# purvakulkarni15/PathTracerAP

Measured on NVIDIA B200. Metric: Mrays/s (all bounces), higher is better.
Workload: dtype f32

## Files before the change

### pathtracerap_b200/csrc/api.cu

```cuda
#include <dlfcn.h>

#include <algorithm>
#include <array>
#include <cmath>
#include <chrono>
#include <cstdarg>
#include <cstdio>
#include <cstdlib>
#include <cstring>
#include <atomic>
#include <string>
#include <thread>
#include <vector>

#include "bvh_build.h"
#include "host_math.h"
#include "kernels.cuh"

using namespace ptap;

namespace {

struct Arena {
    char* base = nullptr;
    size_t cap = 0, used = 0;
    cudaError_t reserve(size_t bytes)
    {
        used = 0;
        if (bytes <= cap) return cudaSuccess;
        if (base) cudaFree(base);
        base = nullptr; cap = 0;
        cudaError_t e = cudaMalloc(&base, bytes);
        if (e == cudaSuccess) cap = bytes;
        return e;
    }
    template <typename T> T* alloc(size_t count)
    {
        size_t bytes = (count * sizeof(T) + 255) & ~size_t(255);
        if (used + bytes > cap) return nullptr;
        T* p = reinterpret_cast<T*>(base + used);
        used += bytes;
        return p;
    }
    static size_t need(size_t count, size_t elem) { return (count * elem + 255) & ~size_t(255); }
    void release() { if (base) cudaFree(base); base = nullptr; cap = used = 0; }
};

}

struct ptap_ctx {
    int device = 0;
    int sms = 148;
    cudaStream_t stream = nullptr;
    cudaEvent_t ev0 = nullptr, ev1 = nullptr, tm0 = nullptr, tm1 = nullptr;
    std::vector<cudaEvent_t> prof_events;
    std::vector<int> prof_kind;
    size_t prof_used = 0;
    Arena scene_arena, frame_arena, scratch;
    SceneDev sc{};
    WaveDev wv{};
    int lanes = 1;
    int lanes_env = 0;
    WaveDev wvx[kMaxLanes]{};
    cudaStream_t streams[kMaxLanes] = {};
    cudaEvent_t e_fork = nullptr, e_cache = nullptr, e_join[kMaxLanes] = {}, e_gather[kMaxLanes] = {};
    std::vector<TriRec> h_tris;
    int ntris = 0;
    std::vector<PtapMesh> h_meshes;
    std::vector<PtapModel> h_models;
    std::vector<InstanceTrace> h_inst;
    InstanceTrace* d_inst = nullptr; TriRec* d_tris = nullptr; BvhNode* d_nodes = nullptr; size_t nodes_cap = 0; LeafTri* d_btris = nullptr; int* d_btid = nullptr;
    bool have_scene = false, have_grid = false, have_bvh = false, have_frame = false;
    int bvh_kind = -1;
    int accel = PTAP_ACCEL_GRID_COMPAT;
    uint32_t flags = 0;
    bool cache_valid = false;
    int grid_trace = 0, grid_shade = 0, grid_gen = 0;
    int trace_ctas = 0;
    PtapStats stats{};
    PtapCamera camera{{0.0f, 0.0f, 920.0f}, {-10.0f, -4.0f, 900.0f}, {20.0f, 16.0f}, 0, 0u};
    std::vector<cudaEvent_t> iter_events;
    int iter_events_used = 0;
    std::vector<float> iter_ms;
    int emu_replay_ctas = 6, emu_walk_ctas = 2;
    Arena emu_arena; int emu_lanes = 0;
    int2* d_tri_box = nullptr; size_t tri_box_cap = 0; bool emu_ok = false;
    std::vector<int> h_grid_first, h_model_grid;
    int2* gd_cells = nullptr; int* gd_refs = nullptr; size_t gd_ncells = 0, gd_nrefs = 0;
    void* nccl_comm = nullptr;
    cudaEvent_t e_peer = nullptr;
    unsigned long long* d_stamps = nullptr;
    int stamps_used = 0;
    bool render_pending = false;
    Arena query_arena;
    cudaEvent_t e_qin = nullptr, e_qout = nullptr;
    bool query_anyhit = true;
    std::string err;
};

namespace {

int fail(ptap_ctx* c, int code, const char* fmt, ...)
{
    char buf[512];
    va_list ap; va_start(ap, fmt); vsnprintf(buf, sizeof buf, fmt, ap); va_end(ap);
    if (c) c->err = buf;
    return code;
}

#define CK(call)                                                                                       \
    do {                                                                                               \
        cudaError_t e_ = (call);                                                                       \
        if (e_ != cudaSuccess) return fail(ctx, (int)e_, "%s: %s", #call, cudaGetErrorString(e_));   \
    } while (0)

template <typename F> void parallelFor(int n, F fn)
{
    const int workers = n < (1 << 16) ? 1 : (int)std::min(8u, std::max(1u, std::thread::hardware_concurrency()));
    if (workers <= 1) { fn(0, n); return; }
    std::vector<std::thread> pool;
    const int chunk = (n + workers - 1) / workers;
    for (int w = 1; w < workers; ++w) pool.emplace_back([=]() { fn(std::min(n, w * chunk), std::min(n, (w + 1) * chunk)); });
    fn(0, std::min(n, chunk));
    for (std::thread& t : pool) t.join();
}

float4 row(const float* m, int r) { return make_float4(m[0 + r], m[4 + r], m[8 + r], m[12 + r]); }

constexpr int kMaxStamps = 8192;

void launchTrace(ptap_ctx* c, FrameState* st, const float4* O, const float4* D, float4* hit, float2* uv, int4* counts, int round, int n_fixed,
                 const EmuBuf& emu, bool count_totals = false, cudaStream_t stream = nullptr, unsigned long long* stamp = nullptr)
{
    if (!stream) stream = c->stream;
    if (c->accel == PTAP_ACCEL_GRID_EMULATED) {
        launchTraceEmu(c->sc, O, D, hit, uv, counts, count_totals, st, round, n_fixed, c->grid_trace, c->sms * c->emu_replay_ctas, c->sms, stream, stamp, emu);
        launchTraceGrid(c->sc, O, D, hit, uv, nullptr, false, st, round, n_fixed, c->sms, stream, nullptr, emu.list2);
    }
    else if (c->accel != PTAP_ACCEL_GRID_COMPAT) launchTraceBvh(c->sc, O, D, hit, uv, counts, count_totals, st, round, n_fixed, c->grid_trace, stream, stamp);
    else launchTraceGrid(c->sc, O, D, hit, uv, counts, count_totals, st, round, n_fixed, c->grid_trace, stream, stamp);
}

size_t emuFullThreads(const ptap_ctx* c) { return (size_t)c->sms * kTraceBlock; }

size_t emuArenaNeed(const ptap_ctx* c, size_t n)
{
    return Arena::need(n, sizeof(int)) * 3 + Arena::need(n * kEmuHits, sizeof(int)) + Arena::need(n * kEmuHits, sizeof(float)) + Arena::need(n * 5, sizeof(uint4)) +
           Arena::need(emuFullThreads(c) * kBigHits, sizeof(uint4));
}

EmuBuf emuFromArena(const ptap_ctx* c, Arena& A, size_t n)
{
    EmuBuf e;
    e.n = A.alloc<int>(n); e.list = A.alloc<int>(n); e.list2 = A.alloc<int>(n); e.id = A.alloc<int>(n * kEmuHits); e.t = A.alloc<float>(n * kEmuHits); e.stride = (int)n;
    e.cont = A.alloc<uint4>(n * 5); e.cont_cap = (int)n;
    e.big = A.alloc<uint4>(emuFullThreads(c) * kBigHits);
    return e;
}

int ensureEmuBuffers(ptap_ctx* ctx)
{
    if (ctx->accel != PTAP_ACCEL_GRID_EMULATED) return PTAP_OK;
    const size_t N = (size_t)ctx->wv.N, per_lane = emuArenaNeed(ctx, N), need = per_lane * (size_t)ctx->lanes + 4096;
    bool moved = false;
    if (ctx->emu_arena.cap < need) { CK(ctx->emu_arena.reserve(need)); moved = true; }
    if (!moved && ctx->wv.emu.n && ctx->wv.emu.stride == (int)N && ctx->emu_lanes == ctx->lanes) return PTAP_OK;
    ctx->emu_arena.used = 0;
    ctx->wv.emu = emuFromArena(ctx, ctx->emu_arena, N);
    for (int l = 1; l < ctx->lanes; ++l) ctx->wvx[l].emu = emuFromArena(ctx, ctx->emu_arena, N);
    ctx->emu_lanes = ctx->lanes;
    return PTAP_OK;
}

void profMark(ptap_ctx* c, int kind)
{
    if (!(c->flags & PTAP_FLAG_PROFILE)) return;
    if (c->prof_used == c->prof_events.size()) {
        cudaEvent_t e; cudaEventCreate(&e); c->prof_events.push_back(e); c->prof_kind.push_back(0);
    }
    c->prof_kind[c->prof_used] = kind;
    cudaEventRecord(c->prof_events[c->prof_used++], c->stream);
}

void resetStats(ptap_ctx* c)
{
    const PtapStats old = c->stats;
    c->stats = PtapStats{};
    c->stats.scene_bytes = old.scene_bytes; c->stats.ms_build = old.ms_build; c->stats.bvh_nodes = old.bvh_nodes; c->stats.bvh_depth = old.bvh_depth;
    c->stats.lanes = c->lanes;
}

void applyCamera(const ptap_ctx* c, WaveDev& wv)
{
    wv.step_x = (float)((double)c->camera.span[0] / (double)wv.W);
    wv.step_y = (float)((double)c->camera.span[1] / (double)wv.H);
    for (int k = 0; k < 3; ++k) { wv.cam_o[k] = c->camera.origin[k]; wv.cam_p[k] = c->camera.plane_min[k]; }
    wv.jitter = c->camera.jitter; wv.jitter_seed = c->camera.jitter_seed;
}

int traceGridSize(ptap_ctx* c)
{
    int occ = c->accel == PTAP_ACCEL_GRID_EMULATED ? traceEmuOccupancy() : c->accel != PTAP_ACCEL_GRID_COMPAT ? traceBvhOccupancy() : traceGridOccupancy();
    if (c->trace_ctas > 0) occ = std::min(occ, c->trace_ctas);
    return c->sms * std::max(occ, 1);
}

int collect(ptap_ctx* ctx)
{
    if (!ctx->render_pending) return PTAP_OK;
    CK(cudaStreamSynchronize(ctx->stream));
    ctx->render_pending = false;
    CK(cudaEventElapsedTime(&ctx->stats.ms_render, ctx->ev0, ctx->ev1));
    FrameState fs;
    CK(cudaMemcpy(&fs, ctx->wv.st, sizeof fs, cudaMemcpyDeviceToHost));
    for (int l = 1; l < ctx->lanes; ++l) {
        if (!ctx->wvx[l].st) continue;
        FrameState f2;
        CK(cudaMemcpy(&f2, ctx->wvx[l].st, sizeof f2, cudaMemcpyDeviceToHost));
        const bool later = f2.iter_cur > fs.iter_cur && f2.paths > 0;
        f2.rays_traced += fs.rays_traced; f2.rays_walked += fs.rays_walked; f2.rays_reemulated += fs.rays_reemulated; f2.paths += fs.paths;
        f2.count_nodes += fs.count_nodes; f2.count_tris += fs.count_tris; f2.count_cells += fs.count_cells; f2.count_refs += fs.count_refs;
        if (later) fs = f2;
        else { fs.rays_traced = f2.rays_traced; fs.rays_walked = f2.rays_walked; fs.rays_reemulated = f2.rays_reemulated; fs.paths = f2.paths; fs.count_nodes = f2.count_nodes; fs.count_tris = f2.count_tris; fs.count_cells = f2.count_cells; fs.count_refs = f2.count_refs; }
    }
    ctx->stats.rays_traced = (int64_t)fs.rays_traced;
    ctx->stats.rays_walked = (int64_t)fs.rays_walked;
    ctx->stats.rays_reemulated = (int64_t)fs.rays_reemulated;
    ctx->stats.paths = (int64_t)fs.paths;
    for (int i = 0; i < 16; ++i) ctx->stats.active_per_round[i] = i <= kMaxDepth ? fs.n_active[i] : 0;
    const double rt = fs.rays_traced ? (double)fs.rays_traced : 1.0;
    ctx->stats.avg_nodes = (float)(fs.count_nodes / rt); ctx->stats.avg_tris = (float)(fs.count_tris / rt);
    ctx->stats.avg_cells = (float)(fs.count_cells / rt); ctx->stats.avg_refs = (float)(fs.count_refs / rt);
    ctx->stats.ms_generate = ctx->stats.ms_trace = ctx->stats.ms_shade = 0.f;
    for (size_t i = 0; i + 1 < ctx->prof_used; ++i) {
        float ms = 0.f;
        if (ctx->prof_kind[i] < 0) continue;
        cudaEventElapsedTime(&ms, ctx->prof_events[i], ctx->prof_events[i + 1]);
        if (ctx->prof_kind[i] == 0) ctx->stats.ms_generate += ms;
        else if (ctx->prof_kind[i] == 1) ctx->stats.ms_trace += ms;
        else ctx->stats.ms_shade += ms;
    }
    ctx->prof_used = 0;
    ctx->iter_ms.assign(ctx->iter_events_used, 0.f);
    for (int k = 0; k < ctx->iter_events_used; ++k) cudaEventElapsedTime(&ctx->iter_ms[k], ctx->ev0, ctx->iter_events[k]);
    ctx->iter_events_used = 0;
    ctx->stats.ms_trace_inflight = ctx->stats.ms_trace_sum = 0.f;
    if (ctx->stamps_used > 0 && ctx->d_stamps) {
        std::vector<unsigned long long> h((size_t)ctx->stamps_used * 2);
        CK(cudaMemcpy(h.data(), ctx->d_stamps, h.size() * sizeof(unsigned long long), cudaMemcpyDeviceToHost));
        std::vector<std::pair<unsigned long long, unsigned long long>> iv;
        double sum = 0.0;
        for (int k = 0; k < ctx->stamps_used; ++k)
            if (h[2 * k + 1] >= h[2 * k]) { iv.push_back({h[2 * k], h[2 * k + 1]}); sum += (double)(h[2 * k + 1] - h[2 * k]); }
        std::sort(iv.begin(), iv.end());
        double uni = 0.0; unsigned long long cur_b = 0, cur_e = 0; bool open = false;
        for (auto& x : iv) {
            if (!open) { cur_b = x.first; cur_e = x.second; open = true; }
            else if (x.first <= cur_e) cur_e = std::max(cur_e, x.second);
            else { uni += (double)(cur_e - cur_b); cur_b = x.first; cur_e = x.second; }
        }
        if (open) uni += (double)(cur_e - cur_b);
        ctx->stats.ms_trace_inflight = (float)(uni * 1e-6); ctx->stats.ms_trace_sum = (float)(sum * 1e-6);
        ctx->stamps_used = 0;
    }
    return PTAP_OK;
}

bool invert3(const double m[9], double out[9])
{
    const double c0 = m[4] * m[8] - m[5] * m[7], c1 = m[5] * m[6] - m[3] * m[8], c2 = m[3] * m[7] - m[4] * m[6];
    const double det = m[0] * c0 + m[1] * c1 + m[2] * c2;
    if (!(std::fabs(det) > 1e-300)) return false;
    const double id = 1.0 / det;
    out[0] = c0 * id; out[1] = (m[2] * m[7] - m[1] * m[8]) * id; out[2] = (m[1] * m[5] - m[2] * m[4]) * id;
    out[3] = c1 * id; out[4] = (m[0] * m[8] - m[2] * m[6]) * id; out[5] = (m[2] * m[3] - m[0] * m[5]) * id;
    out[6] = c2 * id; out[7] = (m[1] * m[6] - m[0] * m[7]) * id; out[8] = (m[0] * m[4] - m[1] * m[3]) * id;
    return true;
}

struct TlasItem { float lo[3], hi[3]; int inst; };

float boxArea(const float* lo, const float* hi)
{
    const float dx = hi[0] - lo[0], dy = hi[1] - lo[1], dz = hi[2] - lo[2];
    return 2.f * (dx * dy + dy * dz + dz * dx);
}

int buildTlas(std::vector<TlasItem>& items, int b, int e, std::vector<Bvh2Node>& nodes, float* lo, float* hi)
{
    for (int k = 0; k < 3; ++k) { lo[k] = 3e38f; hi[k] = -3e38f; }
    for (int i = b; i < e; ++i)
        for (int k = 0; k < 3; ++k) { lo[k] = std::min(lo[k], items[i].lo[k]); hi[k] = std::max(hi[k], items[i].hi[k]); }
    if (e - b == 1) return ~(0x20000000 | items[b].inst);
    int axis = 0; float best = -1.f;
    for (int k = 0; k < 3; ++k) {
        float cmin = 3e38f, cmax = -3e38f;
        for (int i = b; i < e; ++i) { const float c = items[i].lo[k] + items[i].hi[k]; cmin = std::min(cmin, c); cmax = std::max(cmax, c); }
        if (cmax - cmin > best) { best = cmax - cmin; axis = k; }
    }
    const int mid = (b + e) / 2;
    std::nth_element(items.begin() + b, items.begin() + mid, items.begin() + e,
                     [axis](const TlasItem& x, const TlasItem& y) { return x.lo[axis] + x.hi[axis] < y.lo[axis] + y.hi[axis]; });
    const int me = (int)nodes.size();
    nodes.emplace_back();
    float l0[3], h0[3], l1[3], h1[3];
    int c0 = buildTlas(items, b, mid, nodes, l0, h0);
    int c1 = buildTlas(items, mid, e, nodes, l1, h1);
    if (boxArea(l1, h1) < boxArea(l0, h0)) {
        std::swap(c0, c1);
        for (int k = 0; k < 3; ++k) { std::swap(l0[k], l1[k]); std::swap(h0[k], h1[k]); }
    }
    Bvh2Node& nd = nodes[me];
    nd.xy0 = make_float4(l0[0], h0[0], l0[1], h0[1]);
    nd.xy1 = make_float4(l1[0], h1[0], l1[1], h1[1]);
    nd.z01 = make_float4(l0[2], h0[2], l1[2], h1[2]);
    nd.link = make_int4(c0, c1, 0, 0);
    return me;
}

void dropBvh(ptap_ctx* ctx)
{
    ctx->have_bvh = false; ctx->bvh_kind = -1; ctx->sc.tlas_root = -1;
}

bool bvhMissing(const ptap_ctx* ctx) { return ctx->accel != PTAP_ACCEL_GRID_COMPAT && !ctx->have_bvh; }

int finishBvh(ptap_ctx* ctx, const BvhNode* roots, const int* mesh_root, int nnodes, int blas_depth, size_t* tlas_bytes)
{
    const int nm = (int)ctx->h_models.size();
    std::vector<TlasItem> items;
    double max_scale = 0.0, max_pad = 0.0, max_trans = 1.0;
    bool consistent = true;
    for (int i = 0; i < nm; ++i) {
        const PtapModel& m = ctx->h_models[i];
        const int root = mesh_root[m.mesh_index];
        ctx->h_inst[i].grid.z = __builtin_bit_cast(float, root);
        if (root < 0) continue;
        const float* W = m.world_to_model; const float* M = m.model_to_world;
        const double w3[9] = {W[0], W[4], W[8], W[1], W[5], W[9], W[2], W[6], W[10]};
        double wi[9];
        if (!invert3(w3, wi)) return fail(ctx, PTAP_E_INVALID, "model %d: world_to_model is singular", i);
        for (int r = 0; r < 3 && consistent; ++r)
            for (int c = 0; c < 4; ++c) {
                const double scale = c == 3 ? std::max(1.0, std::fabs((double)M[12 + r])) : 1.0;
                if (c == 3) max_trans = std::max(max_trans, scale);
                const double v = (double)M[0 + r] * W[4 * c + 0] + (double)M[4 + r] * W[4 * c + 1] + (double)M[8 + r] * W[4 * c + 2] + (c == 3 ? (double)M[12 + r] : 0.0);
                if (!(std::fabs(v - (r == c ? 1.0 : 0.0)) <= 2e-5 * scale)) { consistent = false; break; }
            }
        const BvhNode& r = roots[m.mesh_index];
        float mlo[3] = {3e38f, 3e38f, 3e38f}, mhi[3] = {-3e38f, -3e38f, -3e38f};
        for (int k = 0; k < 4; ++k) {
            if (!slotUsed(r, k)) continue;
            double lo[3], hi[3];
            decodeChild(r, k, lo, hi);
            for (int a = 0; a < 3; ++a) { mlo[a] = std::min(mlo[a], std::nextafter((float)lo[a], -3e38f)); mhi[a] = std::max(mhi[a], std::nextafter((float)hi[a], 3e38f)); }
        }
        TlasItem it; it.inst = i;
        for (int k = 0; k < 3; ++k) { it.lo[k] = 3e38f; it.hi[k] = -3e38f; }
        double ext = 0.0;
        for (int c = 0; c < 8; ++c) {
            const double p[3] = {((c & 1) ? mhi[0] : mlo[0]) - (double)W[12], ((c & 2) ? mhi[1] : mlo[1]) - (double)W[13], ((c & 4) ? mhi[2] : mlo[2]) - (double)W[14]};
            for (int rr = 0; rr < 3; ++rr) {
                const double w = wi[3 * rr] * p[0] + wi[3 * rr + 1] * p[1] + wi[3 * rr + 2] * p[2];
                it.lo[rr] = std::min(it.lo[rr], (float)w); it.hi[rr] = std::max(it.hi[rr], (float)w);
                ext = std::max(ext, std::fabs(w));
            }
        }
        const float pad = (float)(ext * 1e-4 + 1e-3);
        for (int k = 0; k < 3; ++k) { it.lo[k] -= pad; it.hi[k] += pad; }
        items.push_back(it);
        double fro = 0.0;
        for (double v : wi) fro += v * v;
        max_scale = std::max(max_scale, std::sqrt(fro));
        max_pad = std::max(max_pad, (double)pad);
    }
    std::vector<BvhNode> tlas;
    int tlas_root = -1, tlas_depth = 0;
    if (!items.empty()) {
        float lo[3], hi[3];
        std::vector<Bvh2Node> t2;
        const int link = buildTlas(items, 0, (int)items.size(), t2, lo, hi);
        if (link < 0) {
            Bvh2Node nd;
            nd.xy0 = make_float4(lo[0], hi[0], lo[1], hi[1]); nd.xy1 = nd.xy0;
            nd.z01 = make_float4(lo[2], hi[2], lo[2], hi[2]);
            nd.link = make_int4(link, link, 0, 0);
            t2.push_back(nd);
        }
        tlas_root = collapseBvh2(t2.data(), link < 0 ? (int)t2.size() - 1 : link, tlas, nnodes, 1, tlas_depth);
    }
    if (3 * (blas_depth + tlas_depth) + 8 > kBvhStack) return fail(ctx, PTAP_E_INVALID, "BVH too deep for the traversal stack (%d + %d levels, %d entries)", blas_depth, tlas_depth, kBvhStack);
    if (nnodes + tlas.size() > ctx->nodes_cap) return fail(ctx, PTAP_E_NOMEM, "BVH node storage exhausted");
    CK(cudaMemcpyAsync(ctx->d_inst, ctx->h_inst.data(), nm * sizeof(InstanceTrace), cudaMemcpyHostToDevice, ctx->stream));
    if (!tlas.empty()) CK(cudaMemcpyAsync(ctx->d_nodes + nnodes, tlas.data(), tlas.size() * sizeof(BvhNode), cudaMemcpyHostToDevice, ctx->stream));
    CK(cudaStreamSynchronize(ctx->stream));
    if (tlas_bytes) *tlas_bytes = nm * sizeof(InstanceTrace) + tlas.size() * sizeof(BvhNode);
    ctx->sc.tlas_root = tlas_root;
    ctx->sc.tmin_world = -(float)((kEpsilon + 2e-4) * max_scale * 1.001 + max_pad + 1e-3);
    ctx->sc.prune = consistent ? 1.0003f : INFINITY;
    ctx->sc.tie = consistent ? 1.5e-4f : INFINITY;
    ctx->sc.c_pad = (float)(4e-5 * max_trans + 1e-3);
    ctx->have_bvh = true;
    return PTAP_OK;
}

int uploadBvh(ptap_ctx* ctx, const BvhNode* nodes, int nnodes, const int* tri_id, const int* mesh_root, int known_depth, size_t* bytes)
{
    const int nt = ctx->ntris, nm = (int)ctx->h_models.size();
    dropBvh(ctx);
    if ((size_t)nnodes > ctx->nodes_cap) return fail(ctx, PTAP_E_NOMEM, "BVH has more nodes than reserved (2 per triangle)");
    {
        std::atomic<int> bad_node{-1}, bad_leaf{-1}, bad_entry{-1};
        parallelFor(nnodes, [&](int b, int e) {
            for (int i = b; i < e; ++i)
                for (int k = 0; k < 4; ++k) {
                    const int l = nodes[i].link[k];
                    if (l >= nnodes) bad_node = i;
                    if (l < 0) { const int code = ~l, first = code >> 3, cnt = (code & 7) + 1; if (code >= 0x20000000 || first < 0 || first + cnt > nt) bad_leaf = i; }
                }
        });
        parallelFor(nt, [&](int b, int e) { for (int k = b; k < e; ++k) if (tri_id[k] < 0 || tri_id[k] >= nt) bad_entry = k; });
        if (bad_node >= 0) return fail(ctx, PTAP_E_INVALID, "BVH node %d: child index out of range", bad_node.load());
        if (bad_leaf >= 0) return fail(ctx, PTAP_E_INVALID, "BVH node %d: leaf range out of bounds", bad_leaf.load());
        if (bad_entry >= 0) return fail(ctx, PTAP_E_INVALID, "BVH leaf order entry %d out of range", bad_entry.load());
    }
    for (size_t m = 0; m < ctx->h_meshes.size(); ++m)
        if (mesh_root[m] >= nnodes) return fail(ctx, PTAP_E_INVALID, "mesh %d: BVH root out of range", (int)m);
    int blas_depth = 0;
    (void)known_depth;
    {
        std::vector<int> level(nnodes, 0);
        bool ordered = true;
        for (size_t m = 0; m < ctx->h_meshes.size(); ++m) {
            if (mesh_root[m] < 0) continue;
            if (level[mesh_root[m]]) return fail(ctx, PTAP_E_INVALID, "BVH node %d is the root of two meshes", mesh_root[m]);
            level[mesh_root[m]] = 1;
        }
        for (int i = 0; i < nnodes && ordered; ++i) {
            if (!level[i]) continue;
            blas_depth = std::max(blas_depth, level[i]);
            for (int k = 0; k < 4; ++k) {
                const int l = nodes[i].link[k];
                if (l < 0 || !slotUsed(nodes[i], k)) continue;
                if (l <= i) { ordered = false; break; }
                if (level[l]) return fail(ctx, PTAP_E_INVALID, "BVH node %d is reachable twice", l);
                level[l] = level[i] + 1;
            }
        }
        if (!ordered) {
            blas_depth = 0;
            std::vector<std::pair<int, int>> todo;
            std::vector<char> seen(nnodes, 0);
            for (size_t m = 0; m < ctx->h_meshes.size(); ++m) if (mesh_root[m] >= 0) todo.push_back({mesh_root[m], 1});
            while (!todo.empty()) {
                const auto [node, d] = todo.back(); todo.pop_back();
                if (seen[node]) return fail(ctx, PTAP_E_INVALID, "BVH node %d is reachable twice", node);
                seen[node] = 1;
                blas_depth = std::max(blas_depth, d);
                for (int k = 0; k < 4; ++k)
                    if (nodes[node].link[k] >= 0 && slotUsed(nodes[node], k)) todo.push_back({nodes[node].link[k], d + 1});
            }
        }
    }
    std::vector<BvhNode> roots(ctx->h_meshes.size());
    for (size_t m = 0; m < roots.size(); ++m)
        if (mesh_root[m] >= 0) roots[m] = nodes[mesh_root[m]];
    CK(cudaMemcpyAsync(ctx->d_nodes, nodes, (size_t)nnodes * sizeof(BvhNode), cudaMemcpyHostToDevice, ctx->stream));
    CK(cudaMemcpyAsync(ctx->d_btid, tri_id, (size_t)nt * sizeof(int), cudaMemcpyHostToDevice, ctx->stream));
    launchGatherTris(ctx->d_tris, ctx->d_btid, nt, ctx->d_btris, ctx->stream);
    size_t tb = 0;
    const int rc = finishBvh(ctx, roots.data(), mesh_root, nnodes, blas_depth, &tb);
    if (rc) return rc;
    if (bytes) *bytes = tb + (size_t)nnodes * sizeof(BvhNode) + (size_t)nt * sizeof(int);
    ctx->bvh_kind = PTAP_ACCEL_BVH;
    return PTAP_OK;
}

int buildBvhOnDevice(ptap_ctx* ctx)
{
    const int nt = ctx->ntris, nmesh = (int)ctx->h_meshes.size();
    dropBvh(ctx);
    int max_tris = 0;
    for (const PtapMesh& m : ctx->h_meshes) max_tris = std::max(max_tris, m.t_end - m.t_start);
    const size_t need = deviceBvhScratchBytes(max_tris);
    if (need > ctx->scratch.cap) CK(ctx->scratch.reserve(need)); else ctx->scratch.used = 0;
    std::vector<int> mesh_root(nmesh, -1);
    int nnodes = 0, leaf_base = 0, blas_depth = 0;
    for (int mi = 0; mi < nmesh; ++mi) {
        const PtapMesh& m = ctx->h_meshes[mi];
        const int n = m.t_end - m.t_start;
        if (n <= 0 || m.t_start < 0 || m.t_end > nt) continue;
        if ((size_t)nnodes + (size_t)n > ctx->nodes_cap || leaf_base + n > nt) return fail(ctx, PTAP_E_NOMEM, "device BVH build: node / leaf storage exhausted");
        int made = 0, depth = 0;
        std::string why;
        const int e = buildMeshBvhDevice(ctx->d_tris, m.t_start, m.t_end, m.bb_min, m.bb_max, nnodes, ctx->d_nodes + nnodes, leaf_base, ctx->d_btris, ctx->d_btid,
                                         ctx->scratch.base, ctx->scratch.cap, ctx->stream, &made, &depth, &why);
        if (e != 0) return fail(ctx, e, "device BVH build of mesh %d (%d triangles): %s", mi, n, why.empty() ? cudaGetErrorString((cudaError_t)e) : why.c_str());
        mesh_root[mi] = nnodes;
        nnodes += made; leaf_base += n; blas_depth = std::max(blas_depth, depth);
    }
    std::vector<BvhNode> roots(nmesh);
    for (int mi = 0; mi < nmesh; ++mi)
        if (mesh_root[mi] >= 0) CK(cudaMemcpyAsync(&roots[mi], ctx->d_nodes + mesh_root[mi], sizeof(BvhNode), cudaMemcpyDeviceToHost, ctx->stream));
    CK(cudaStreamSynchronize(ctx->stream));
    const int rc = finishBvh(ctx, roots.data(), mesh_root.data(), nnodes, blas_depth, nullptr);
    if (rc) return rc;
    ctx->bvh_kind = PTAP_ACCEL_BVH_DEVICE;
    ctx->stats.bvh_nodes = nnodes; ctx->stats.bvh_depth = blas_depth;
    return PTAP_OK;
}

}

extern "C" {

int ptap_create(int device, size_t arena_bytes, ptap_ctx** out)
{
    if (!out) return PTAP_E_INVALID;
    *out = nullptr;
    int ndev = 0;
    if (cudaGetDeviceCount(&ndev) != cudaSuccess || ndev == 0 || device < 0 || device >= ndev) return PTAP_E_NO_DEVICE;
    cudaDeviceProp prop;
    if (cudaGetDeviceProperties(&prop, device) != cudaSuccess) return PTAP_E_NO_DEVICE;
    if (prop.major < 10) return PTAP_E_NO_DEVICE;
    ptap_ctx* ctx = new ptap_ctx();
    ctx->device = device;
    ctx->sms = prop.multiProcessorCount;
    if (cudaSetDevice(device) != cudaSuccess || cudaStreamCreateWithFlags(&ctx->stream, cudaStreamNonBlocking) != cudaSuccess) {
        delete ctx; return PTAP_E_NO_DEVICE;
    }
    cudaEventCreate(&ctx->ev0); cudaEventCreate(&ctx->ev1);
    auto envInt = [](const char* name, int dflt) { const char* v = getenv(name); return v && *v ? atoi(v) : dflt; };
    ctx->sc.vote_tri = std::min(32, std::max(1, envInt("PTAP_VOTE_TRI", kVoteTri)));
    ctx->sc.vote_inst = std::min(32, std::max(1, envInt("PTAP_VOTE_INST", kVoteInst)));
    ctx->sc.vote_refill = std::min(32, std::max(1, envInt("PTAP_VOTE_REFILL", kVoteRefill)));
    ctx->sc.batch = std::max(1, envInt("PTAP_BATCH", kTraceBatch));
    ctx->sc.vote_grid = std::min(32, std::max(1, envInt("PTAP_VOTE_GRID", kVoteGrid)));
    ctx->sc.shade_sort = envInt("PTAP_SHADE_SORT", 0) != 0;
    ctx->lanes_env = std::min(kMaxLanes, std::max(0, envInt("PTAP_LANES", 0)));
    ctx->lanes = ctx->lanes_env ? ctx->lanes_env : kDefaultLanes;
    ctx->streams[0] = ctx->stream;
    const int max_lanes = ctx->lanes_env ? ctx->lanes_env : kMaxLanes;
    if (max_lanes > 1) {
        bool ok = cudaEventCreateWithFlags(&ctx->e_fork, cudaEventDisableTiming) == cudaSuccess && cudaEventCreateWithFlags(&ctx->e_cache, cudaEventDisableTiming) == cudaSuccess;
        for (int l = 0; l < max_lanes; ++l) {
            if (l > 0) ok = ok && cudaStreamCreateWithFlags(&ctx->streams[l], cudaStreamNonBlocking) == cudaSuccess;
            ok = ok && cudaEventCreateWithFlags(&ctx->e_join[l], cudaEventDisableTiming) == cudaSuccess && cudaEventCreateWithFlags(&ctx->e_gather[l], cudaEventDisableTiming) == cudaSuccess;
        }
        if (!ok) { ptap_destroy(ctx); return PTAP_E_NOMEM; }
    }
    ctx->trace_ctas = std::max(0, envInt("PTAP_TRACE_CTAS", 0));
    ctx->emu_replay_ctas = std::max(1, envInt("PTAP_EMU_REPLAY_CTAS", 6));
    ctx->emu_walk_ctas = std::max(1, envInt("PTAP_EMU_WALK_CTAS", 2));
    ctx->sc.emu_refill = std::min(32, std::max(1, envInt("PTAP_EMU_REFILL", 8)));
    ctx->query_anyhit = envInt("PTAP_QUERY_ANYHIT", 1) != 0;
    if (cudaEventCreateWithFlags(&ctx->e_qin, cudaEventDisableTiming) != cudaSuccess || cudaEventCreateWithFlags(&ctx->e_qout, cudaEventDisableTiming) != cudaSuccess) {
        ptap_destroy(ctx); return PTAP_E_NOMEM;
    }
    if (arena_bytes) {
        if (ctx->scene_arena.reserve(arena_bytes / 4) != cudaSuccess || ctx->frame_arena.reserve(arena_bytes - arena_bytes / 4) != cudaSuccess) {
            ptap_destroy(ctx); return PTAP_E_NOMEM;
        }
    }
    *out = ctx;
    return PTAP_OK;
}

void ptap_destroy(ptap_ctx* ctx)
{
    if (!ctx) return;
    cudaSetDevice(ctx->device);
    if (ctx->stream) cudaStreamSynchronize(ctx->stream);
    for (int l = 1; l < kMaxLanes; ++l) if (ctx->streams[l]) { cudaStreamSynchronize(ctx->streams[l]); cudaStreamDestroy(ctx->streams[l]); }
    for (cudaEvent_t e : {ctx->e_fork, ctx->e_cache}) if (e) cudaEventDestroy(e);
    for (int l = 0; l < kMaxLanes; ++l) { if (ctx->e_join[l]) cudaEventDestroy(ctx->e_join[l]); if (ctx->e_gather[l]) cudaEventDestroy(ctx->e_gather[l]); }
    ctx->scene_arena.release(); ctx->frame_arena.release(); ctx->scratch.release(); ctx->emu_arena.release(); ctx->query_arena.release();
    for (cudaEvent_t e : {ctx->e_qin, ctx->e_qout}) if (e) cudaEventDestroy(e);
    if (ctx->gd_cells) cudaFree(ctx->gd_cells);
    if (ctx->d_tri_box) cudaFree(ctx->d_tri_box);
    if (ctx->gd_refs) cudaFree(ctx->gd_refs);
    for (cudaEvent_t e : ctx->prof_events) cudaEventDestroy(e);
    for (cudaEvent_t e : ctx->iter_events) cudaEventDestroy(e);
    if (ctx->e_peer) cudaEventDestroy(ctx->e_peer);
    if (ctx->nccl_comm) ptap_nccl_finalize(ctx);
    if (ctx->ev0) cudaEventDestroy(ctx->ev0);
    if (ctx->tm0) { cudaEventDestroy(ctx->tm0); cudaEventDestroy(ctx->tm1); }
    if (ctx->ev1) cudaEventDestroy(ctx->ev1);
    if (ctx->stream) cudaStreamDestroy(ctx->stream);
    delete ctx;
}

const char* ptap_last_error(const ptap_ctx* ctx) { return ctx ? ctx->err.c_str() : "no context"; }
void* ptap_stream(ptap_ctx* ctx) { return ctx ? (void*)ctx->stream : nullptr; }

int ptap_upload_scene(ptap_ctx* ctx, const PtapSceneView* v)
{
    if (!ctx || !v || !v->models || !v->meshes || !v->vertices || !v->triangles || v->nmodels <= 0) return fail(ctx, PTAP_E_INVALID, "upload_scene: missing arrays");
    CK(cudaSetDevice(ctx->device));
    if (ctx->render_pending) { int rc = collect(ctx); if (rc) return rc; }
    const bool timing = getenv("PTAP_UPLOAD_TIMING") != nullptr;
    const auto t_begin = std::chrono::steady_clock::now();
    auto t_last = t_begin;
    auto lap = [&](const char* what) {
        if (!timing) return;
        const auto now = std::chrono::steady_clock::now();
        fprintf(stderr, "ptap_upload_scene: %-28s %8.3f ms\n", what, std::chrono::duration<double, std::milli>(now - t_last).count());
        t_last = now;
    };
    const int nm = v->nmodels, nt = v->ntriangles;
    const bool grid = v->grids && v->voxels && v->refs && v->ngrids > 0;
    ctx->have_scene = false; ctx->have_grid = false; ctx->have_bvh = false; ctx->bvh_kind = -1; ctx->cache_valid = false; ctx->emu_ok = false;
    ctx->sc.tlas_root = -1; ctx->sc.nmodels = 0;
    for (int i = 0; i < nm; ++i) {
        const PtapModel& m = v->models[i];
        if (m.mesh_index < 0 || m.mesh_index >= v->nmeshes) return fail(ctx, PTAP_E_INVALID, "model %d: mesh_index %d out of range", i, m.mesh_index);
        if (grid && (m.grid_index < 0 || m.grid_index >= v->ngrids)) return fail(ctx, PTAP_E_INVALID, "model %d: grid_index %d out of range", i, m.grid_index);
    }
    const bool prepacked = v->tri_recs && v->n_tri_recs == nt;
    if (!prepacked)
        for (int t = 0; t < nt; ++t)
            for (int k = 0; k < 3; ++k)
                if (v->triangles[t].v[k] < 0 || v->triangles[t].v[k] >= v->nvertices) return fail(ctx, PTAP_E_INVALID, "triangle %d: vertex index out of range", t);

    std::vector<InstanceTrace> inst(nm);
    std::vector<InstanceShade> shade(nm);
    for (int i = 0; i < nm; ++i) {
        const PtapModel& m = v->models[i];
        InstanceTrace& it = inst[i];
        for (int r = 0; r < 3; ++r) { it.w2m[r] = row(m.world_to_model, r); it.m2w[r] = row(m.model_to_world, r); }
        it.bb_min = make_float4(0, 0, 0, 1); it.bb_max = make_float4(0, 0, 0, 1); it.grid = make_float4(1, 0, 0, 0);
        if (grid) {
            const PtapGrid& g = v->grids[m.grid_index];
            int owner = g.entity_index;
            if (owner < 0 || owner >= nm) return fail(ctx, PTAP_E_INVALID, "grid %d: entity_index %d out of range", m.grid_index, owner);
            const PtapMesh& mesh = v->meshes[v->models[owner].mesh_index];
            it.bb_min = make_float4(mesh.bb_min[0], mesh.bb_min[1], mesh.bb_min[2], g.width[0]);
            it.bb_max = make_float4(mesh.bb_max[0], mesh.bb_max[1], mesh.bb_max[2], g.width[1]);
            it.grid.x = g.width[2];
            it.grid.y = __builtin_bit_cast(float, (int)g.v_start);
        }
        float nmx[9];
        hm::normal_matrix(m.model_to_world, nmx);
        shade[i].nm0 = make_float4(nmx[0], nmx[1], nmx[2], m.mat.color[0]);
        shade[i].nm1 = make_float4(nmx[3], nmx[4], nmx[5], m.mat.color[1]);
        shade[i].nm2 = make_float4(nmx[6], nmx[7], nmx[8], m.mat.color[2]);
        shade[i].mat = make_int4(m.mat.type, 0, 0, 0);
    }
    const TriRec* recs = static_cast<const TriRec*>(v->tri_recs);
    if (!prepacked) {
        ctx->h_tris.resize(nt);
        makeTriRecs(v->vertices, v->triangles, nt, ctx->h_tris.data());
        recs = ctx->h_tris.data();
    } else ctx->h_tris.clear();
    ctx->ntris = nt;
    ctx->h_meshes.assign(v->meshes, v->meshes + v->nmeshes);
    ctx->h_models.assign(v->models, v->models + nm);
    ctx->h_grid_first.clear(); ctx->h_model_grid.clear();
    if (grid) {
        for (int g = 0; g < v->ngrids; ++g) ctx->h_grid_first.push_back(v->grids[g].v_start);
        for (int i = 0; i < nm; ++i) ctx->h_model_grid.push_back(v->models[i].grid_index);
    }

    std::vector<int2> cells;
    if (grid) {
        cells.resize(v->nvoxels);
        for (int i = 0; i < v->nvoxels; ++i) {
            const bool tri = v->voxels[i].entity_type == 2;
            cells[i] = tri ? make_int2(v->voxels[i].start, v->voxels[i].end) : make_int2(0, 0);
            if (tri && (v->voxels[i].start < 0 || v->voxels[i].end > v->nrefs)) return fail(ctx, PTAP_E_INVALID, "voxel %d: ref range out of bounds", i);
        }
        for (int i = 0; i < v->nrefs; ++i)
            if (v->refs[i] < 0 || v->refs[i] >= nt) return fail(ctx, PTAP_E_INVALID, "ref %d: triangle index out of range", i);
        if (v->grid_dim[0] <= 0 || v->grid_dim[1] <= 0 || v->grid_dim[2] <= 0) return fail(ctx, PTAP_E_INVALID, "grid_dim must be positive");
        const long long ncell = (long long)v->grid_dim[0] * v->grid_dim[1] * v->grid_dim[2];
        for (int g = 0; g < v->ngrids; ++g)
            if (v->grids[g].v_start < 0 || v->grids[g].v_start + ncell > v->nvoxels) return fail(ctx, PTAP_E_INVALID, "grid %d: voxel range out of bounds", g);
    }

    lap("validate + repack (host)");
    const size_t nodes_cap = (size_t)std::max(nt, 1) * 2 + (size_t)nm * 2 + 2;
    size_t need = Arena::need(nm, sizeof(InstanceTrace)) + Arena::need(nm, sizeof(InstanceShade)) +
                  Arena::need(nt, sizeof(TriRec)) + Arena::need(nt, sizeof(LeafTri)) + Arena::need(nt, sizeof(float4)) + Arena::need(nt, sizeof(int)) + Arena::need(nodes_cap, sizeof(BvhNode)) +
                  (grid ? Arena::need(v->nvoxels, sizeof(int2)) + Arena::need(v->nrefs, sizeof(int)) : 0) + 4096;
    if (need > ctx->scene_arena.cap) CK(ctx->scene_arena.reserve(need)); else ctx->scene_arena.used = 0;
    Arena& A = ctx->scene_arena;
    InstanceTrace* d_inst = A.alloc<InstanceTrace>(nm);
    InstanceShade* d_shade = A.alloc<InstanceShade>(nm);
    TriRec* d_tris = A.alloc<TriRec>(nt);
    LeafTri* d_btris = A.alloc<LeafTri>(nt);
    float4* d_normals = A.alloc<float4>(nt);
    int* d_btid = A.alloc<int>(nt);
    BvhNode* d_nodes = A.alloc<BvhNode>(nodes_cap);
    int2* d_cells = grid ? A.alloc<int2>(v->nvoxels) : nullptr;
    int* d_refs = grid ? A.alloc<int>(v->nrefs) : nullptr;
    if (!d_inst || !d_shade || !d_tris || !d_normals || !d_btris || !d_btid || !d_nodes || (grid && (!d_cells || !d_refs))) return fail(ctx, PTAP_E_NOMEM, "scene arena exhausted");
    CK(cudaMemcpyAsync(d_inst, inst.data(), nm * sizeof(InstanceTrace), cudaMemcpyHostToDevice, ctx->stream));
    CK(cudaMemcpyAsync(d_shade, shade.data(), nm * sizeof(InstanceShade), cudaMemcpyHostToDevice, ctx->stream));
    CK(cudaMemcpyAsync(d_tris, recs, (size_t)nt * sizeof(TriRec), cudaMemcpyHostToDevice, ctx->stream));
    launchExtractNormals(d_tris, nt, d_normals, ctx->stream);
    ctx->d_tris = d_tris;
    if (grid) {
        CK(cudaMemcpyAsync(d_cells, cells.data(), cells.size() * sizeof(int2), cudaMemcpyHostToDevice, ctx->stream));
        CK(cudaMemcpyAsync(d_refs, v->refs, v->nrefs * sizeof(int), cudaMemcpyHostToDevice, ctx->stream));
    }
    size_t bytes = nm * (sizeof(InstanceTrace) + sizeof(InstanceShade)) + (size_t)nt * sizeof(TriRec) +
                   (grid ? cells.size() * sizeof(int2) + (size_t)v->nrefs * sizeof(int) : 0);
    ctx->h_inst = inst;
    ctx->d_inst = d_inst; ctx->d_nodes = d_nodes; ctx->nodes_cap = nodes_cap; ctx->d_btris = d_btris; ctx->d_btid = d_btid;
    ctx->have_bvh = false; ctx->bvh_kind = -1;
    lap("enqueue scene copies");
    if (v->bvh_nodes && v->n_bvh_nodes > 0 && v->bvh_tri_id && v->bvh_mesh_root) {
        if (v->n_bvh_tris != nt || v->n_bvh_roots != v->nmeshes) return fail(ctx, PTAP_E_INVALID, "upload_scene: prebuilt BVH does not match the triangle / mesh counts");
        size_t bb = 0;
        int rc = uploadBvh(ctx, reinterpret_cast<const BvhNode*>(v->bvh_nodes), v->n_bvh_nodes, v->bvh_tri_id, v->bvh_mesh_root, v->bvh_depth, &bb);
        if (rc) return rc;
        bytes += bb;
    }
    lap("BVH checks + TLAS (host)");
    CK(cudaStreamSynchronize(ctx->stream));
    lap("wait for the device");
    ctx->stats.scene_bytes = (int64_t)bytes;
    ctx->sc.inst = d_inst; ctx->sc.shade = d_shade; ctx->sc.tris = d_tris; ctx->sc.normals = d_normals;
    ctx->sc.cells = d_cells; ctx->sc.refs = d_refs; ctx->sc.nodes = d_nodes; ctx->sc.bvh_tris = d_btris; ctx->sc.bvh_tri_id = d_btid;
    ctx->sc.nmodels = nm; ctx->sc.gx = v->grid_dim[0]; ctx->sc.gy = v->grid_dim[1]; ctx->sc.gz = v->grid_dim[2];
    ctx->have_scene = true; ctx->have_grid = grid; ctx->cache_valid = false;
    ctx->accel = grid ? PTAP_ACCEL_GRID_COMPAT : PTAP_ACCEL_BVH;
    ctx->grid_trace = 0;
    return PTAP_OK;
}

int ptap_build_accel(ptap_ctx* ctx, int kind)
{
    if (!ctx || !ctx->have_scene) return fail(ctx, PTAP_E_STATE, "build_accel: no scene uploaded");
    CK(cudaSetDevice(ctx->device));
    if (ctx->render_pending) { int rc = collect(ctx); if (rc) return rc; }
    if (kind == PTAP_ACCEL_GRID_COMPAT) {
        if (!ctx->have_grid) return fail(ctx, PTAP_E_STATE, "build_accel: the uploaded scene carries no grids (call ptap_scene_build_grids first)");
    } else if (kind == PTAP_ACCEL_BVH) {
        if (!ctx->have_bvh || ctx->bvh_kind != PTAP_ACCEL_BVH) {
            BvhBuildResult res;
            if ((int)ctx->h_tris.size() != ctx->ntris) {
                ctx->h_tris.resize(ctx->ntris);
                CK(cudaMemcpyAsync(ctx->h_tris.data(), ctx->d_tris, (size_t)ctx->ntris * sizeof(TriRec), cudaMemcpyDeviceToHost, ctx->stream));
                CK(cudaStreamSynchronize(ctx->stream));
            }
            buildSceneBvh(ctx->h_tris.data(), (int)ctx->h_tris.size(), ctx->h_meshes.data(), (int)ctx->h_meshes.size(), res);
            int rc = uploadBvh(ctx, res.nodes.data(), (int)res.nodes.size(), res.tri_id.data(), res.mesh_root.data(), res.max_depth + 1, nullptr);
            if (rc) return rc;
            CK(cudaStreamSynchronize(ctx->stream));
        }
    } else if (kind == PTAP_ACCEL_BVH_DEVICE) {
        if (ctx->bvh_kind != PTAP_ACCEL_BVH_DEVICE) {
            cudaEvent_t b0, b1;
            CK(cudaEventCreate(&b0)); CK(cudaEventCreate(&b1));
            CK(cudaEventRecord(b0, ctx->stream));
            const int rc = buildBvhOnDevice(ctx);
            if (rc) { cudaEventDestroy(b0); cudaEventDestroy(b1); return rc; }
            CK(cudaEventRecord(b1, ctx->stream)); CK(cudaEventSynchronize(b1));
            cudaEventElapsedTime(&ctx->stats.ms_build, b0, b1);
            cudaEventDestroy(b0); cudaEventDestroy(b1);
        }
    } else if (kind == PTAP_ACCEL_GRID_EMULATED) {
        if (!ctx->have_grid) return fail(ctx, PTAP_E_STATE, "build_accel: the uploaded scene carries no grids (call ptap_scene_build_grids first)");
        if (!ctx->have_bvh) { const int rc = buildBvhOnDevice(ctx); if (rc) return rc; }
        if (!ctx->emu_ok) {
            const int nt = ctx->ntris, ng = (int)ctx->h_grid_first.size();
            if ((size_t)nt > ctx->tri_box_cap) {
                if (ctx->d_tri_box) { cudaFree(ctx->d_tri_box); ctx->d_tri_box = nullptr; ctx->tri_box_cap = 0; }
                CK(cudaMalloc(&ctx->d_tri_box, (size_t)std::max(nt, 1) * sizeof(int2)));
                ctx->tri_box_cap = (size_t)nt;
            }
            std::vector<int> range(2 * (size_t)std::max(ng, 1), 0);
            int ok = 0;
            const int e = gridTriBoxes(ctx->sc.cells, ctx->sc.refs, ng, ctx->h_grid_first.data(), ctx->sc.gx, ctx->sc.gy, ctx->sc.gz, nt, ctx->d_tri_box, range.data(), &ok, ctx->stream);
            if (e != 0) return fail(ctx, e, "build_accel: voxel boxes: %s", cudaGetErrorString((cudaError_t)e));
            if (!ok) return fail(ctx, PTAP_E_UNSUPPORTED, "build_accel: the voxel lists are not box-shaped ascending registrations of one grid per triangle; use PTAP_ACCEL_GRID_COMPAT");
            for (size_t i = 0; i < ctx->h_models.size(); ++i) {
                const int g = ctx->h_model_grid[i];
                const PtapMesh& mesh = ctx->h_meshes[ctx->h_models[i].mesh_index];
                if (range[2 * g] <= range[2 * g + 1] && (range[2 * g] < mesh.t_start || range[2 * g + 1] >= mesh.t_end))
                    return fail(ctx, PTAP_E_UNSUPPORTED, "build_accel: grid %d lists triangles outside the mesh of model %d; use PTAP_ACCEL_GRID_COMPAT", g, (int)i);
            }
            ctx->sc.tri_box = ctx->d_tri_box;
            ctx->emu_ok = true;
        }
    } else return fail(ctx, PTAP_E_INVALID, "build_accel: unknown kind %d", kind);
    ctx->accel = kind;
    ctx->cache_valid = false;
    ctx->grid_trace = traceGridSize(ctx);
    return PTAP_OK;
}

int ptap_set_render_params(ptap_ctx* ctx, int32_t W, int32_t H, int32_t depth, uint32_t flags)
{
    if (!ctx || W <= 0 || H <= 0 || depth <= 0 || depth > kMaxDepth) return fail(ctx, PTAP_E_INVALID, "set_render_params: W,H > 0 and 1 <= depth <= %d required", kMaxDepth);
    if ((long long)W * H > (1ll << 30)) return fail(ctx, PTAP_E_INVALID, "set_render_params: too many pixels");
    CK(cudaSetDevice(ctx->device));
    if (ctx->render_pending) { int rc = collect(ctx); if (rc) return rc; }
    const int N = W * H;
    ctx->lanes = ctx->lanes_env ? ctx->lanes_env : (N <= (1 << 20) ? kSmallFrameLanes : kDefaultLanes);
    const int ntiles = (N + kShadeTile - 1) / kShadeTile, nscan = (N + kScanSlots - 1) / kScanSlots;
    size_t need = Arena::need(N, sizeof(float4)) * 8 + Arena::need(N, sizeof(float2)) + Arena::need((size_t)N * 3, sizeof(float)) +
                  Arena::need((size_t)nscan * kMaxDepth, sizeof(unsigned long long)) + Arena::need(ntiles, sizeof(int)) * 2 +
                  Arena::need((size_t)nscan * kScanSlots, 1) + Arena::need(1, sizeof(FrameState)) + Arena::need(2 * kMaxStamps, sizeof(unsigned long long)) + 4096;
    if (ctx->lanes > 1)
        need += (size_t)(ctx->lanes - 1) * (Arena::need(N, sizeof(float4)) * 7 + Arena::need((size_t)nscan * kMaxDepth, sizeof(unsigned long long)) +
                                            Arena::need(ntiles, sizeof(int)) * 2 + Arena::need((size_t)nscan * kScanSlots, 1) + Arena::need(1, sizeof(FrameState)) + 4096) +
                (size_t)ctx->lanes * Arena::need((size_t)N * 3, sizeof(float));
    if (need > ctx->frame_arena.cap) CK(ctx->frame_arena.reserve(need)); else ctx->frame_arena.used = 0;
    Arena& A = ctx->frame_arena;
    WaveDev& wv = ctx->wv;
    for (int k = 0; k < 2; ++k) { wv.O[k] = A.alloc<float4>(N); wv.D[k] = A.alloc<float4>(N); wv.C[k] = A.alloc<float4>(N); }
    wv.hit = A.alloc<float4>(N); wv.hit_cache = A.alloc<float4>(N); wv.uv = A.alloc<float2>(N);
    wv.film = A.alloc<float>((size_t)N * 3);
    wv.tile_status = A.alloc<unsigned long long>((size_t)nscan * kMaxDepth);
    wv.tile_offset = A.alloc<int>(ntiles);
    wv.tile_ballot = A.alloc<unsigned>(ntiles);
    wv.perm = A.alloc<unsigned char>((size_t)nscan * kScanSlots);
    wv.st = A.alloc<FrameState>(1);
    wv.emu = EmuBuf{};
    ctx->d_stamps = A.alloc<unsigned long long>(2 * kMaxStamps); ctx->stamps_used = 0;
    if (!ctx->d_stamps || !wv.st || !wv.tile_status || !wv.tile_offset || !wv.tile_ballot || !wv.perm || !wv.film) return fail(ctx, PTAP_E_NOMEM, "frame arena exhausted");
    wv.W = W; wv.H = H; wv.N = N; wv.depth = depth; wv.ntiles = ntiles; wv.nscan = nscan;
    applyCamera(ctx, wv);
    wv.iter_stride = 1; wv.contrib = nullptr;
    if (ctx->lanes > 1) wv.contrib = A.alloc<float>((size_t)N * 3);
    for (int l = 1; l < ctx->lanes; ++l) {
        WaveDev& w2 = ctx->wvx[l];
        w2 = wv;
        for (int k = 0; k < 2; ++k) { w2.O[k] = A.alloc<float4>(N); w2.D[k] = A.alloc<float4>(N); w2.C[k] = A.alloc<float4>(N); }
        w2.hit = A.alloc<float4>(N);
        w2.tile_status = A.alloc<unsigned long long>((size_t)nscan * kMaxDepth);
        w2.tile_offset = A.alloc<int>(ntiles); w2.tile_ballot = A.alloc<unsigned>(ntiles);
        w2.perm = A.alloc<unsigned char>((size_t)nscan * kScanSlots);
        w2.st = A.alloc<FrameState>(1);
        w2.contrib = A.alloc<float>((size_t)N * 3);
        if (!w2.st || !w2.contrib || !wv.contrib || !w2.perm || !w2.hit) return fail(ctx, PTAP_E_NOMEM, "frame arena exhausted (lane %d)", l);
        CK(cudaMemsetAsync(w2.st, 0, sizeof(FrameState), ctx->stream));
    }
    CK(cudaMemsetAsync(wv.film, 0, (size_t)N * 3 * sizeof(float), ctx->stream));
    CK(cudaMemsetAsync(wv.st, 0, sizeof(FrameState), ctx->stream));
    CK(cudaStreamSynchronize(ctx->stream));
    ctx->flags = flags; ctx->cache_valid = false; ctx->have_frame = true;
    ctx->grid_shade = ctx->sms * std::max(shadeOccupancy(), 1);
    ctx->grid_gen = ctx->sms * 8;
    if (!ctx->grid_trace) ctx->grid_trace = traceGridSize(ctx);
    resetStats(ctx);
    return PTAP_OK;
}

int ptap_set_camera(ptap_ctx* ctx, const PtapCamera* cam)
{
    if (!ctx) return PTAP_E_INVALID;
    CK(cudaSetDevice(ctx->device));
    if (ctx->render_pending) { int rc = collect(ctx); if (rc) return rc; }
    const PtapCamera ref{{0.0f, 0.0f, 920.0f}, {-10.0f, -4.0f, 900.0f}, {20.0f, 16.0f}, 0, 0u};
    const PtapCamera c = cam ? *cam : ref;
    if (!(c.span[0] > 0.0f) || !(c.span[1] > 0.0f)) return fail(ctx, PTAP_E_INVALID, "set_camera: the image plane needs a positive extent");
    ctx->camera = c;
    ctx->cache_valid = false;
    if (ctx->have_frame) {
        applyCamera(ctx, ctx->wv);
        for (int l = 1; l < kMaxLanes; ++l) if (ctx->wvx[l].st) { WaveDev& w = ctx->wvx[l]; w.step_x = ctx->wv.step_x; w.step_y = ctx->wv.step_y; for (int k = 0; k < 3; ++k) { w.cam_o[k] = ctx->wv.cam_o[k]; w.cam_p[k] = ctx->wv.cam_p[k]; } w.jitter = ctx->wv.jitter; w.jitter_seed = ctx->wv.jitter_seed; }
    }
    return PTAP_OK;
}

int ptap_render(ptap_ctx* ctx, int32_t iter_begin, int32_t iter_end)
{
    if (!ctx || !ctx->have_scene || !ctx->have_frame) return fail(ctx, PTAP_E_STATE, "render: scene and render parameters required");
    if ((ctx->accel == PTAP_ACCEL_GRID_COMPAT || ctx->accel == PTAP_ACCEL_GRID_EMULATED) && !ctx->have_grid) return fail(ctx, PTAP_E_STATE, "render: no grid in the uploaded scene; build the BVH");
    if (bvhMissing(ctx)) return fail(ctx, PTAP_E_STATE, "render: no BVH on the device (build_accel failed or was not called)");
    if (iter_end < iter_begin) return fail(ctx, PTAP_E_INVALID, "render: empty iteration range");
    CK(cudaSetDevice(ctx->device));
    if (ctx->render_pending) { int rc = collect(ctx); if (rc) return rc; }
    { const int rc = ensureEmuBuffers(ctx); if (rc) return rc; }
    const bool cache = (ctx->flags & PTAP_FLAG_FIRST_HIT_CACHE) && !ctx->camera.jitter;
    const int L = (ctx->flags & (PTAP_FLAG_PROFILE | PTAP_FLAG_COUNT)) ? 1 : std::max(1, std::min(ctx->lanes, iter_end - iter_begin));
    WaveDev lane[kMaxLanes];
    lane[0] = ctx->wv;
    for (int l = 1; l < L; ++l) lane[l] = ctx->wvx[l];
    for (int l = 0; l < L; ++l) { lane[l].iter_stride = L; if (L == 1) lane[l].contrib = nullptr; }
    const bool stamping = (ctx->flags & PTAP_FLAG_STAMP) != 0;
    if (stamping) {
        CK(cudaMemset2DAsync(ctx->d_stamps, 16, 0xff, 8, kMaxStamps, ctx->stream));
        CK(cudaMemset2DAsync(ctx->d_stamps + 1, 16, 0x00, 8, kMaxStamps, ctx->stream));
    }
    ctx->stamps_used = 0; ctx->iter_events_used = 0;
    CK(cudaEventRecord(ctx->ev0, ctx->stream));
    if (L > 1) CK(cudaEventRecord(ctx->e_fork, ctx->stream));
    for (int l = 0; l < L; ++l) {
        if (l > 0) CK(cudaStreamWaitEvent(ctx->streams[l], ctx->e_fork, 0));
        launchSetIter(lane[l].st, iter_begin + l, ctx->streams[l]);
    }
    int64_t launches = L, trace_launches = 0;
    int cache_lane = -1;
    unsigned cache_waited = 0;
    for (int it = iter_begin; it < iter_end; ++it) {
        const int l = (it - iter_begin) % L;
        const WaveDev& wv = lane[l];
        cudaStream_t S = ctx->streams[l];
        profMark(ctx, 0);
        launchGenerate(wv, it, ctx->grid_gen, S); ++launches;
        int in = 0;
        for (int round = 0; round < wv.depth; ++round) {
            float4* hitbuf = (round == 0 && cache) ? wv.hit_cache : wv.hit;
            if (!(round == 0 && cache && ctx->cache_valid)) {
                profMark(ctx, 1);
                unsigned long long* stamp = stamping && ctx->stamps_used < kMaxStamps ? ctx->d_stamps + 2 * (size_t)ctx->stamps_used++ : nullptr;
                launchTrace(ctx, wv.st, wv.O[in], wv.D[in], hitbuf, nullptr, nullptr, round, -1, wv.emu, (ctx->flags & PTAP_FLAG_COUNT) != 0, S, stamp); launches += ctx->accel == PTAP_ACCEL_GRID_EMULATED ? 5 : 1; ++trace_launches;
                if (L > 1 && round == 0 && cache) { CK(cudaEventRecord(ctx->e_cache, S)); cache_lane = l; cache_waited = 1u << l; }
            } else if (L > 1 && cache_lane >= 0 && !(cache_waited >> l & 1u)) {
                CK(cudaStreamWaitEvent(S, ctx->e_cache, 0)); cache_waited |= 1u << l;
            }
            profMark(ctx, 2);
            launchScan(ctx->sc, wv, round, hitbuf, wv.depth - round, -1, S); ++launches;
            launchShade(ctx->sc, wv, round, in, hitbuf, wv.depth - round, -1, 0, nullptr, ctx->grid_shade, S); ++launches;
            in ^= 1;
        }
        if (L > 1) {
            if (it > iter_begin) CK(cudaStreamWaitEvent(S, ctx->e_gather[(l + L - 1) % L], 0));
            launchFilmAdd(wv.film, wv.contrib, (size_t)wv.N * 3, S); ++launches;
            CK(cudaEventRecord(ctx->e_gather[l], S));
        }
        if (cache) ctx->cache_valid = true;
        if (ctx->flags & PTAP_FLAG_ITER_TIMES) {
            if (ctx->iter_events_used == (int)ctx->iter_events.size()) { cudaEvent_t e; CK(cudaEventCreate(&e)); ctx->iter_events.push_back(e); }
            CK(cudaEventRecord(ctx->iter_events[ctx->iter_events_used++], S));
        }
    }
    for (int l = 1; l < L; ++l) {
        CK(cudaEventRecord(ctx->e_join[l], ctx->streams[l]));
        CK(cudaStreamWaitEvent(ctx->stream, ctx->e_join[l], 0));
    }
    profMark(ctx, -1);
    CK(cudaEventRecord(ctx->ev1, ctx->stream));
    CK(cudaGetLastError());
    ctx->stats.kernel_launches += launches;
    ctx->stats.trace_launches = trace_launches;
    ctx->render_pending = true;
    return PTAP_OK;
}

int ptap_sync(ptap_ctx* ctx)
{
    if (!ctx) return PTAP_E_INVALID;
    CK(cudaSetDevice(ctx->device));
    int rc = collect(ctx); if (rc) return rc;
    CK(cudaStreamSynchronize(ctx->stream));
    return PTAP_OK;
}

int ptap_frame_begin(ptap_ctx* ctx)
{
    if (!ctx || !ctx->have_frame) return fail(ctx, PTAP_E_STATE, "frame_begin: no render parameters");
    CK(cudaSetDevice(ctx->device));
    if (ctx->render_pending) { int rc = collect(ctx); if (rc) return rc; }
    CK(cudaMemsetAsync(ctx->wv.film, 0, (size_t)ctx->wv.N * 3 * sizeof(float), ctx->stream));
    CK(cudaMemsetAsync(ctx->wv.st, 0, sizeof(FrameState), ctx->stream));
    for (int l = 1; l < ctx->lanes; ++l) if (ctx->wvx[l].st) CK(cudaMemsetAsync(ctx->wvx[l].st, 0, sizeof(FrameState), ctx->stream));
    ctx->cache_valid = false;
    resetStats(ctx);
    return PTAP_OK;
}

int ptap_timer_start(ptap_ctx* ctx)
{
    if (!ctx) return PTAP_E_INVALID;
    CK(cudaSetDevice(ctx->device));
    if (!ctx->tm0) { CK(cudaEventCreate(&ctx->tm0)); CK(cudaEventCreate(&ctx->tm1)); }
    CK(cudaEventRecord(ctx->tm0, ctx->stream));
    return PTAP_OK;
}

int ptap_timer_stop(ptap_ctx* ctx, float* ms)
{
    if (!ctx || !ms || !ctx->tm0) return PTAP_E_INVALID;
    CK(cudaSetDevice(ctx->device));
    CK(cudaEventRecord(ctx->tm1, ctx->stream));
    CK(cudaEventSynchronize(ctx->tm1));
    CK(cudaEventElapsedTime(ms, ctx->tm0, ctx->tm1));
    return PTAP_OK;
}

int ptap_film_reset(ptap_ctx* ctx)
{
    if (!ctx || !ctx->have_frame) return fail(ctx, PTAP_E_STATE, "film_reset: no render parameters");
    CK(cudaSetDevice(ctx->device));
    CK(cudaMemsetAsync(ctx->wv.film, 0, (size_t)ctx->wv.N * 3 * sizeof(float), ctx->stream));
    return PTAP_OK;
}

int ptap_read_film(ptap_ctx* ctx, float* rgb)
{
    if (!ctx || !ctx->have_frame || !rgb) return fail(ctx, PTAP_E_STATE, "read_film: no render parameters");
    CK(cudaSetDevice(ctx->device));
    CK(cudaMemcpyAsync(rgb, ctx->wv.film, (size_t)ctx->wv.N * 3 * sizeof(float), cudaMemcpyDeviceToHost, ctx->stream));
    return ptap_sync(ctx);
}

int ptap_film_device_ptr(ptap_ctx* ctx, void** dev_ptr, size_t* nfloats)
{
    if (!ctx || !ctx->have_frame || !dev_ptr) return fail(ctx, PTAP_E_STATE, "film_device_ptr: no render parameters");
    *dev_ptr = ctx->wv.film;
    if (nfloats) *nfloats = (size_t)ctx->wv.N * 3;
    return PTAP_OK;
}

int ptap_film_add(ptap_ctx* ctx, const float* rgb)
{
    if (!ctx || !ctx->have_frame || !rgb) return fail(ctx, PTAP_E_STATE, "film_add: no render parameters");
    CK(cudaSetDevice(ctx->device));
    const size_t n = (size_t)ctx->wv.N * 3;
    if (Arena::need(n, sizeof(float)) > ctx->scratch.cap) CK(ctx->scratch.reserve(Arena::need(n, sizeof(float)))); else ctx->scratch.used = 0;
    float* tmp = ctx->scratch.alloc<float>(n);
    CK(cudaMemcpyAsync(tmp, rgb, n * sizeof(float), cudaMemcpyHostToDevice, ctx->stream));
    launchFilmAdd(ctx->wv.film, tmp, n, ctx->stream);
    CK(cudaStreamSynchronize(ctx->stream));
    return PTAP_OK;
}

int ptap_get_stats(ptap_ctx* ctx, PtapStats* out)
{
    if (!ctx || !out) return PTAP_E_INVALID;
    CK(cudaSetDevice(ctx->device));
    int rc = collect(ctx); if (rc) return rc;
// ... 575 lines not shown
```

### pathtracerap_b200/csrc/bvh_device.cu

```cuda
#include <algorithm>
#include <cmath>
#include <cstdlib>
#include <string>
#include <utility>
#include <vector>

#include <cub/device/device_radix_sort.cuh>
#include <cub/device/device_scan.cuh>

#include "kernels.cuh"

namespace ptap {

namespace {

constexpr float kBandEpsF = 0.0056f;
#ifndef PTAP_LBVH_CLUSTER
#define PTAP_LBVH_CLUSTER 1
#endif
constexpr int kCluster = PTAP_LBVH_CLUSTER;

__device__ __forceinline__ unsigned expandBits(unsigned v)
{
    v = (v * 0x00010001u) & 0xFF0000FFu;
    v = (v * 0x00000101u) & 0x0F00F00Fu;
    v = (v * 0x00000011u) & 0xC30C30C3u;
    v = (v * 0x00000005u) & 0x49249249u;
    return v;
}

struct Box6 { float lo[3], hi[3]; };

__device__ __forceinline__ Box6 fatBox(const TriRec& r, float slack)
{
    Box6 b;
    const float uv[3][2] = {{-kBandEpsF, -kBandEpsF}, {1.0f + 2.0f * kBandEpsF, -kBandEpsF}, {-kBandEpsF, 1.0f + 2.0f * kBandEpsF}};
    const float v0[3] = {r.v0.x, r.v0.y, r.v0.z}, e1[3] = {r.e1.x, r.e1.y, r.e1.z}, e2[3] = {r.e2.x, r.e2.y, r.e2.z};
#pragma unroll
    for (int k = 0; k < 3; ++k) {
        float lo = 3e38f, hi = -3e38f;
#pragma unroll
        for (int c = 0; c < 3; ++c) {
            const float p = v0[k] + uv[c][0] * e1[k] + uv[c][1] * e2[k];
            lo = fminf(lo, p); hi = fmaxf(hi, p);
        }
        const float pad = slack + 2e-6f * fmaxf(fabsf(lo), fabsf(hi));
        b.lo[k] = lo - pad; b.hi[k] = hi + pad;
    }
    return b;
}

__global__ void k_lbvh_keys(const TriRec* __restrict__ tris, int t0, int n, float3 mlo, float3 minv, unsigned* __restrict__ keys, int* __restrict__ ids)
{
    const int i = blockIdx.x * blockDim.x + threadIdx.x;
    if (i >= n) return;
    const TriRec r = tris[t0 + i];
    const float cx = r.v0.x + (r.e1.x + r.e2.x) * (1.0f / 3.0f), cy = r.v0.y + (r.e1.y + r.e2.y) * (1.0f / 3.0f), cz = r.v0.z + (r.e1.z + r.e2.z) * (1.0f / 3.0f);
    const unsigned qx = (unsigned)fminf(fmaxf((cx - mlo.x) * minv.x, 0.0f), 1023.0f);
    const unsigned qy = (unsigned)fminf(fmaxf((cy - mlo.y) * minv.y, 0.0f), 1023.0f);
    const unsigned qz = (unsigned)fminf(fmaxf((cz - mlo.z) * minv.z, 0.0f), 1023.0f);
    keys[i] = (expandBits(qx) << 2) | (expandBits(qy) << 1) | expandBits(qz);
    ids[i] = t0 + i;
}

__global__ void k_lbvh_leaves(const TriRec* __restrict__ tris, const unsigned* __restrict__ keys, const int* __restrict__ ids, int n, int nleaves,
                              float slack, int leaf_base, LeafTri* __restrict__ btris, int* __restrict__ btid, Box6* __restrict__ leaf_box,
                              unsigned long long* __restrict__ leaf_key)
{
    const int c = blockIdx.x * blockDim.x + threadIdx.x;
    if (c >= nleaves) return;
    Box6 box;
#pragma unroll
    for (int k = 0; k < 3; ++k) { box.lo[k] = 3e38f; box.hi[k] = -3e38f; }
    const int first = kCluster * c, last = min(first + kCluster, n);
    for (int s = first; s < last; ++s) {
        const int id = ids[s];
        const TriRec r = tris[id];
        const Box6 b = fatBox(r, slack);
#pragma unroll
        for (int k = 0; k < 3; ++k) { box.lo[k] = fminf(box.lo[k], b.lo[k]); box.hi[k] = fmaxf(box.hi[k], b.hi[k]); }
        float4* o = reinterpret_cast<float4*>(&btris[leaf_base + s]);
        o[0] = make_float4(r.v0.x, r.v0.y, r.v0.z, r.e1.x);
        o[1] = make_float4(r.e1.y, r.e1.z, r.e2.x, r.e2.y);
        o[2] = make_float4(r.e2.z, __int_as_float(id), 0.0f, 0.0f);
        o[3] = make_float4(0.0f, 0.0f, 0.0f, 0.0f);
        btid[leaf_base + s] = id;
    }
    leaf_box[c] = box;
    leaf_key[c] = ((unsigned long long)keys[first] << 32) | (unsigned)c;
}

__device__ __forceinline__ int delta(const unsigned long long* __restrict__ k, int n, int i, int j)
{
    return (j < 0 || j >= n) ? -1 : __clzll(k[i] ^ k[j]);
}

__global__ void k_lbvh_topology(const unsigned long long* __restrict__ key, int nleaves, int2* __restrict__ child, int* __restrict__ parent_internal,
                                int* __restrict__ parent_leaf)
{
    const int i = blockIdx.x * blockDim.x + threadIdx.x;
    if (i >= nleaves - 1) return;
    const int d = delta(key, nleaves, i, i + 1) - delta(key, nleaves, i, i - 1) >= 0 ? 1 : -1;
    const int dmin = delta(key, nleaves, i, i - d);
    int lmax = 2;
    while (delta(key, nleaves, i, i + lmax * d) > dmin) lmax <<= 1;
    int l = 0;
    for (int t = lmax >> 1; t >= 1; t >>= 1)
        if (delta(key, nleaves, i, i + (l + t) * d) > dmin) l += t;
    const int j = i + l * d;
    const int dnode = delta(key, nleaves, i, j);
    int s = 0;
    for (int t = (l + 1) >> 1;; t = (t + 1) >> 1) {
        if (delta(key, nleaves, i, i + (s + t) * d) > dnode) s += t;
        if (t <= 1) break;
    }
    const int gamma = i + s * d + min(d, 0);
    const int lo = min(i, j), hi = max(i, j);
    const int left = lo == gamma ? ~gamma : gamma, right = hi == gamma + 1 ? ~(gamma + 1) : gamma + 1;
    child[i] = make_int2(left, right);
    if (left >= 0) parent_internal[left] = i; else parent_leaf[~left] = i;
    if (right >= 0) parent_internal[right] = i; else parent_leaf[~right] = i;
    if (i == 0) parent_internal[0] = -1;
}

__device__ __forceinline__ Box6 loadBoxL2(const Box6* p)
{
    Box6 b;
    const float* f = reinterpret_cast<const float*>(p);
#pragma unroll
    for (int k = 0; k < 3; ++k) { b.lo[k] = __ldcg(f + k); b.hi[k] = __ldcg(f + 3 + k); }
    return b;
}

__global__ void k_lbvh_refit(const int2* __restrict__ child, const int* __restrict__ parent_internal, const int* __restrict__ parent_leaf,
                             const Box6* __restrict__ leaf_box, int nleaves, Box6* __restrict__ node_box, int* __restrict__ arrived)
{
    const int c = blockIdx.x * blockDim.x + threadIdx.x;
    if (c >= nleaves) return;
    int node = parent_leaf[c];
    while (node >= 0) {
        if (atomicAdd(&arrived[node], 1) == 0) return;
        __threadfence();
        const int2 ch = child[node];
        const Box6 a = ch.x >= 0 ? loadBoxL2(&node_box[ch.x]) : leaf_box[~ch.x], b = ch.y >= 0 ? loadBoxL2(&node_box[ch.y]) : leaf_box[~ch.y];
        Box6 u;
#pragma unroll
        for (int k = 0; k < 3; ++k) { u.lo[k] = fminf(a.lo[k], b.lo[k]); u.hi[k] = fmaxf(a.hi[k], b.hi[k]); }
        node_box[node] = u;
        __threadfence();
        node = parent_internal[node];
    }
}

__device__ __forceinline__ int leafLink(int c, int n, int leaf_base)
{
    const int first = kCluster * c, count = min(kCluster, n - first);
    return ~(((leaf_base + first) << 3) | (count - 1));
}

__device__ void encodeNodeDevice(BvhNode& nd, const Box6* boxes, int ne)
{
    float lo[3] = {3e38f, 3e38f, 3e38f}, mag = 0.0f;
    for (int c = 0; c < ne; ++c)
        for (int k = 0; k < 3; ++k) {
            lo[k] = fminf(lo[k], boxes[c].lo[k]);
            mag = fmaxf(mag, fmaxf(fabsf(boxes[c].lo[k]), fabsf(boxes[c].hi[k])));
        }
    const float margin = __fmul_ru(mag, 9.5367431640625e-7f) + 1e-30f;
    float p[3];
    for (int k = 0; k < 3; ++k) p[k] = nextafterf(__fsub_rd(lo[k], margin), -3e38f);
    nd.px = p[0]; nd.py = p[1]; nd.pz = p[2]; nd.pad = 0;
    for (int c = 0; c < 4; ++c)
        for (int k = 0; k < 3; ++k) {
            if (c < ne) {
                nd.planes[k][0][c] = nextafterf(__fsub_rd(__fsub_rd(boxes[c].lo[k], margin), p[k]), -3e38f);
                nd.planes[k][1][c] = nextafterf(__fsub_ru(__fadd_ru(boxes[c].hi[k], margin), p[k]), 3e38f);
            } else { nd.planes[k][0][c] = 1e15f; nd.planes[k][1][c] = -1e15f; }
        }
}

__global__ void k_lbvh_collapse(const int2* __restrict__ child, const Box6* __restrict__ node_box, const Box6* __restrict__ leaf_box, int n, int leaf_base,
                                const int2* __restrict__ frontier, int nfrontier, int2* __restrict__ next, int* __restrict__ counters ,
                                int node_base, BvhNode* __restrict__ out)
{
    const int f = blockIdx.x * blockDim.x + threadIdx.x;
    if (f >= nfrontier) return;
    const int2 item = frontier[f];
    int ent[4]; Box6 ebox[4]; int ne = 2;
    { const int2 ch = child[item.x]; ent[0] = ch.x; ent[1] = ch.y; }
    for (int k = 0; k < 2; ++k) ebox[k] = ent[k] >= 0 ? node_box[ent[k]] : leaf_box[~ent[k]];
    while (ne < 4) {
        int best = -1; float best_area = -1.0f;
        for (int k = 0; k < ne; ++k) {
            if (ent[k] < 0) continue;
            const float dx = ebox[k].hi[0] - ebox[k].lo[0], dy = ebox[k].hi[1] - ebox[k].lo[1], dz = ebox[k].hi[2] - ebox[k].lo[2];
            const float a = dx * dy + dy * dz + dz * dx;
            if (a > best_area) { best_area = a; best = k; }
        }
        if (best < 0) break;
        const int2 g = child[ent[best]];
        ent[best] = g.x; ebox[best] = g.x >= 0 ? node_box[g.x] : leaf_box[~g.x];
        ent[ne] = g.y; ebox[ne] = g.y >= 0 ? node_box[g.y] : leaf_box[~g.y];
        ++ne;
    }
    BvhNode nd;
    Box6 boxes[4];
    for (int k = 0; k < 4; ++k) {
        if (k < ne) {
            const int e = ent[k];
            boxes[k] = ebox[k];
            if (e >= 0) {
                const int idx = atomicAdd(&counters[0], 1);
                next[atomicAdd(&counters[1], 1)] = make_int2(e, idx);
                nd.link[k] = node_base + idx;
            } else nd.link[k] = leafLink(~e, n, leaf_base);
        } else nd.link[k] = nd.link[0];
    }
    encodeNodeDevice(nd, boxes, ne);
    out[item.y] = nd;
}

__global__ void k_lbvh_single(const Box6* __restrict__ leaf_box, int n, int leaf_base, BvhNode* __restrict__ out)
{
    BvhNode nd;
    const Box6 b = leaf_box[0];
    for (int k = 0; k < 4; ++k) nd.link[k] = leafLink(0, n, leaf_base);
    encodeNodeDevice(nd, &b, 1);
    out[0] = nd;
}


#ifndef PTAP_PLOC_RADIUS
#define PTAP_PLOC_RADIUS 16
#endif
constexpr int kPlocRadius = PTAP_PLOC_RADIUS;
#ifndef PTAP_PLOC_TOP
#define PTAP_PLOC_TOP 4096
#endif
constexpr int kPlocTop = PTAP_PLOC_TOP;

__device__ __forceinline__ float unionArea(const Box6& a, const Box6& b)
{
    const float dx = fmaxf(a.hi[0], b.hi[0]) - fminf(a.lo[0], b.lo[0]), dy = fmaxf(a.hi[1], b.hi[1]) - fminf(a.lo[1], b.lo[1]), dz = fmaxf(a.hi[2], b.hi[2]) - fminf(a.lo[2], b.lo[2]);
    return dx * dy + dy * dz + dz * dx;
}

__global__ void k_ploc_init(const Box6* __restrict__ leaf_box, int n, Box6* __restrict__ cbox, int* __restrict__ cnode)
{
    const int i = blockIdx.x * blockDim.x + threadIdx.x;
    if (i < n) { cbox[i] = leaf_box[i]; cnode[i] = ~i; }
}

__device__ __forceinline__ unsigned long long plocTieKey(int i, int j)
{
    return ((unsigned long long)((i >> 1) != (j >> 1)) << 63) | ((unsigned long long)abs(i - j) << 32) | (unsigned)min(i, j);
}

__global__ void k_ploc_nearest(const Box6* __restrict__ cbox, int n, int* __restrict__ nearest)
{
    const int i = blockIdx.x * blockDim.x + threadIdx.x;
    if (i >= n) return;
    const Box6 me = cbox[i];
    float best = 3e38f; int bj = -1; unsigned long long bkey = ~0ull;
    const int j0 = max(0, i - kPlocRadius), j1 = min(n - 1, i + kPlocRadius);
    for (int j = j0; j <= j1; ++j) {
        if (j == i) continue;
        const float a = unionArea(me, cbox[j]);
        const unsigned long long key = plocTieKey(i, j);
        if (a < best || (a == best && key < bkey)) { best = a; bj = j; bkey = key; }
    }
    nearest[i] = bj;
}

__global__ void k_ploc_merge(Box6* __restrict__ cbox, int* __restrict__ cnode, const int* __restrict__ nearest, int n, int2* __restrict__ child,
                             Box6* __restrict__ node_box, int* __restrict__ counter, int* __restrict__ keep)
{
    const int i = blockIdx.x * blockDim.x + threadIdx.x;
    if (i >= n) return;
    const int j = nearest[i];
    if (j >= 0 && nearest[j] == i) {
        if (i < j) {
            const Box6 a = cbox[i], b = cbox[j];
            Box6 u;
#pragma unroll
            for (int k = 0; k < 3; ++k) { u.lo[k] = fminf(a.lo[k], b.lo[k]); u.hi[k] = fmaxf(a.hi[k], b.hi[k]); }
            const int id = atomicAdd(counter, 1);
            child[id] = make_int2(cnode[i], cnode[j]);
            node_box[id] = u;
            cbox[i] = u; cnode[i] = id;
            keep[i] = 1;
        } else keep[i] = 0;
    } else keep[i] = 1;
}

__global__ void k_ploc_compact(const Box6* __restrict__ cbox, const int* __restrict__ cnode, const int* __restrict__ keep, const int* __restrict__ pos, int n,
                               Box6* __restrict__ obox, int* __restrict__ onode)
{
    const int i = blockIdx.x * blockDim.x + threadIdx.x;
    if (i < n && keep[i]) { obox[pos[i]] = cbox[i]; onode[pos[i]] = cnode[i]; }
}

struct TopItem { Box6 box; float c[3]; int link; };

int buildTopSah(std::vector<TopItem>& it, int begin, int end, int base, std::vector<int2>& out_child, std::vector<Box6>& out_box, Box6& bounds)
{
    auto grow = [](Box6& a, const Box6& b) { for (int k = 0; k < 3; ++k) { a.lo[k] = std::min(a.lo[k], b.lo[k]); a.hi[k] = std::max(a.hi[k], b.hi[k]); } };
    auto area = [](const Box6& b) { const float dx = b.hi[0] - b.lo[0], dy = b.hi[1] - b.lo[1], dz = b.hi[2] - b.lo[2]; return dx < 0 ? 0.0f : dx * dy + dy * dz + dz * dx; };
    auto empty = []() { Box6 b; for (int k = 0; k < 3; ++k) { b.lo[k] = 3e38f; b.hi[k] = -3e38f; } return b; };
    bounds = empty();
    float clo[3] = {3e38f, 3e38f, 3e38f}, chi[3] = {-3e38f, -3e38f, -3e38f};
    for (int i = begin; i < end; ++i) { grow(bounds, it[i].box); for (int k = 0; k < 3; ++k) { clo[k] = std::min(clo[k], it[i].c[k]); chi[k] = std::max(chi[k], it[i].c[k]); } }
    if (end - begin == 1) return it[begin].link;
    constexpr int kBins = 16;
    int best_axis = -1, best_bin = -1; float best_cost = 3e38f;
    for (int axis = 0; axis < 3; ++axis) {
        const float ext = chi[axis] - clo[axis];
        if (!(ext > 0.0f)) continue;
        Box6 bb[kBins]; int cnt[kBins];
        for (int b = 0; b < kBins; ++b) { bb[b] = empty(); cnt[b] = 0; }
        const float scale = kBins / ext;
        for (int i = begin; i < end; ++i) { const int b = std::min(kBins - 1, std::max(0, (int)((it[i].c[axis] - clo[axis]) * scale))); grow(bb[b], it[i].box); cnt[b]++; }
        float right_area[kBins]; int right_cnt[kBins];
        Box6 acc = empty(); int c = 0;
        for (int b = kBins - 1; b > 0; --b) { grow(acc, bb[b]); c += cnt[b]; right_area[b] = area(acc); right_cnt[b] = c; }
        acc = empty(); c = 0;
        for (int b = 0; b < kBins - 1; ++b) {
            grow(acc, bb[b]); c += cnt[b];
            if (c == 0 || right_cnt[b + 1] == 0) continue;
            const float cost = area(acc) * c + right_area[b + 1] * right_cnt[b + 1];
            if (cost < best_cost) { best_cost = cost; best_axis = axis; best_bin = b; }
        }
    }
    int mid = begin + (end - begin) / 2;
    if (best_axis >= 0) {
        const float lo = clo[best_axis], scale = kBins / (chi[best_axis] - clo[best_axis]);
        auto m = std::partition(it.begin() + begin, it.begin() + end, [&](const TopItem& t) { return std::min(kBins - 1, std::max(0, (int)((t.c[best_axis] - lo) * scale))) <= best_bin; });
        const int k = (int)(m - it.begin());
        if (k > begin && k < end) mid = k;
    }
    const int me = (int)out_child.size();
    out_child.push_back(make_int2(0, 0)); out_box.push_back(bounds);
    Box6 b0, b1;
    const int l0 = buildTopSah(it, begin, mid, base, out_child, out_box, b0);
    const int l1 = buildTopSah(it, mid, end, base, out_child, out_box, b1);
    out_child[me] = make_int2(l0, l1);
    return base + me;
}

template <typename T> T* carve(char*& p, size_t count)
{
    T* r = reinterpret_cast<T*>(p);
    p += (count * sizeof(T) + 255) & ~size_t(255);
    return r;
}

}

size_t deviceBvhScratchBytes(int ntris)
{
    const size_t n = (size_t)std::max(ntris, 1), L = (n + kCluster - 1) / kCluster;
    size_t cub_bytes = 0;
    cub::DeviceRadixSort::SortPairs(nullptr, cub_bytes, (const unsigned*)nullptr, (unsigned*)nullptr, (const int*)nullptr, (int*)nullptr, (int)n, 0, 30);
    size_t scan_bytes = 0;
    cub::DeviceScan::ExclusiveSum(nullptr, scan_bytes, (const int*)nullptr, (int*)nullptr, (int)n);
    cub_bytes = std::max(cub_bytes, scan_bytes);
    return 4 * ((n * 4 + 255) & ~size_t(255)) + cub_bytes + 256 + 4 * ((L * sizeof(Box6) + 255) & ~size_t(255)) + ((L * 8 + 255) & ~size_t(255)) * 4 +
           ((L * 4 + 255) & ~size_t(255)) * 3 + 4096;
}

int buildMeshBvhDevice(const TriRec* d_tris, int t0, int t1, const float* bb_min, const float* bb_max, int node_base, BvhNode* out_nodes, int leaf_base,
                       LeafTri* btris, int* btid, char* scratch, size_t scratch_bytes, cudaStream_t stream, int* nnodes, int* depth, std::string* why)
{
    const int n = t1 - t0, L = (n + kCluster - 1) / kCluster;
    *nnodes = 0; *depth = 0;
    if (n <= 0) return cudaSuccess;
    if (deviceBvhScratchBytes(n) > scratch_bytes) return cudaErrorMemoryAllocation;
    char* p = scratch;
    unsigned* keys = carve<unsigned>(p, n); unsigned* keys2 = carve<unsigned>(p, n);
    int* ids = carve<int>(p, n); int* ids2 = carve<int>(p, n);
    size_t cub_bytes = 0;
    cub::DeviceRadixSort::SortPairs(nullptr, cub_bytes, (const unsigned*)keys, keys2, (const int*)ids, ids2, n, 0, 30);
    { size_t scan_bytes = 0; cub::DeviceScan::ExclusiveSum(nullptr, scan_bytes, (const int*)nullptr, (int*)nullptr, n); cub_bytes = std::max(cub_bytes, scan_bytes); }
    void* cub_tmp = carve<char>(p, cub_bytes + 1);
    Box6* leaf_box = carve<Box6>(p, L); Box6* node_box = carve<Box6>(p, L);
    Box6* cbox_a = carve<Box6>(p, L); Box6* cbox_b = carve<Box6>(p, L);
    unsigned long long* leaf_key = carve<unsigned long long>(p, L);
    int2* child = carve<int2>(p, L); int2* fr_a = carve<int2>(p, L); int2* fr_b = carve<int2>(p, L);
    int* parent_internal = carve<int>(p, L); int* parent_leaf = carve<int>(p, L); int* arrived = carve<int>(p, L);
    int* counters = carve<int>(p, 64);

    double ext = 0.0;
    float3 mlo, minv;
    {
        const float lo[3] = {bb_min[0], bb_min[1], bb_min[2]}, hi[3] = {bb_max[0], bb_max[1], bb_max[2]};
        for (int k = 0; k < 3; ++k) ext = std::max(ext, (double)std::max(std::fabs(lo[k]), std::fabs(hi[k])));
        mlo = make_float3(lo[0], lo[1], lo[2]);
        auto inv = [](float a, float b) { return b > a ? 1023.999f / (b - a) : 0.0f; };
        minv = make_float3(inv(lo[0], hi[0]), inv(lo[1], hi[1]), inv(lo[2], hi[2]));
    }
    const float slack = (float)(ext * 4e-6 + 1e-6);
    const int B = 256;
    k_lbvh_keys<<<(n + B - 1) / B, B, 0, stream>>>(d_tris, t0, n, mlo, minv, keys, ids);
    cudaError_t e = cub::DeviceRadixSort::SortPairs(cub_tmp, cub_bytes, (const unsigned*)keys, keys2, (const int*)ids, ids2, n, 0, 30, stream);
    if (e != cudaSuccess) return e;
    k_lbvh_leaves<<<(L + B - 1) / B, B, 0, stream>>>(d_tris, keys2, ids2, n, L, slack, leaf_base, btris, btid, leaf_box, leaf_key);
    if (L == 1) {
        k_lbvh_single<<<1, 1, 0, stream>>>(leaf_box, n, leaf_base, out_nodes);
        *nnodes = 1; *depth = 1;
        return cudaGetLastError();
    }
    int root_node = 0;
    const char* which = getenv("PTAP_DEVICE_BUILDER");
    if (which && std::string(which) == "lbvh") {
        k_lbvh_topology<<<(L - 1 + B - 1) / B, B, 0, stream>>>(leaf_key, L, child, parent_internal, parent_leaf);
        e = cudaMemsetAsync(arrived, 0, (size_t)L * sizeof(int), stream);
        if (e != cudaSuccess) return e;
        k_lbvh_refit<<<(L + B - 1) / B, B, 0, stream>>>(child, parent_internal, parent_leaf, leaf_box, L, node_box, arrived);
    } else {
        Box6 *cb = cbox_a, *cb2 = cbox_b;
        int *cn = parent_internal, *cn2 = parent_leaf, *nearest = arrived, *keep = reinterpret_cast<int*>(keys), *pos = ids;
        e = cudaMemsetAsync(counters + 8, 0, sizeof(int), stream);
        if (e != cudaSuccess) return e;
        k_ploc_init<<<(L + B - 1) / B, B, 0, stream>>>(leaf_box, L, cb, cn);
        int m = L, rounds = 0;
        const char* top_env = getenv("PTAP_PLOC_TOP");
        const int top = top_env ? atoi(top_env) : kPlocTop;
        while (m > 1 && !(top > 1 && m <= top)) {
            const int g = (m + B - 1) / B;
            k_ploc_nearest<<<g, B, 0, stream>>>(cb, m, nearest);
            k_ploc_merge<<<g, B, 0, stream>>>(cb, cn, nearest, m, child, node_box, counters + 8, keep);
            e = cub::DeviceScan::ExclusiveSum(cub_tmp, cub_bytes, keep, pos, m, stream);
            if (e != cudaSuccess) return e;
            k_ploc_compact<<<g, B, 0, stream>>>(cb, cn, keep, pos, m, cb2, cn2);
            int last[2];
            e = cudaMemcpyAsync(&last[0], pos + m - 1, sizeof(int), cudaMemcpyDeviceToHost, stream);
            if (e == cudaSuccess) e = cudaMemcpyAsync(&last[1], keep + m - 1, sizeof(int), cudaMemcpyDeviceToHost, stream);
            if (e == cudaSuccess) e = cudaStreamSynchronize(stream);
            if (e != cudaSuccess) return e;
            const int m2 = last[0] + last[1];
            if (m2 >= m || ++rounds > 4096) {
                if (why) *why = "PLOC merging stalled at " + std::to_string(m2) + " of " + std::to_string(L) + " clusters after " + std::to_string(rounds) + " rounds";
                return cudaErrorUnknown;
            }
            m = m2;
            std::swap(cb, cb2); std::swap(cn, cn2);
        }
        if (m > 1) {
            std::vector<Box6> hb(m); std::vector<int> hl(m);
            int made = 0;
            e = cudaMemcpyAsync(hb.data(), cb, (size_t)m * sizeof(Box6), cudaMemcpyDeviceToHost, stream);
            if (e == cudaSuccess) e = cudaMemcpyAsync(hl.data(), cn, (size_t)m * sizeof(int), cudaMemcpyDeviceToHost, stream);
            if (e == cudaSuccess) e = cudaMemcpyAsync(&made, counters + 8, sizeof(int), cudaMemcpyDeviceToHost, stream);
            if (e == cudaSuccess) e = cudaStreamSynchronize(stream);
            if (e != cudaSuccess) return e;
            if (made + m - 1 > L) return cudaErrorUnknown;
            std::vector<TopItem> items(m);
            for (int k = 0; k < m; ++k) { items[k].box = hb[k]; items[k].link = hl[k]; for (int a = 0; a < 3; ++a) items[k].c[a] = 0.5f * (hb[k].lo[a] + hb[k].hi[a]); }
            std::vector<int2> tc; std::vector<Box6> tb;
            tc.reserve(m); tb.reserve(m);
            Box6 bounds;
            root_node = buildTopSah(items, 0, m, made, tc, tb, bounds);
            e = cudaMemcpyAsync(child + made, tc.data(), tc.size() * sizeof(int2), cudaMemcpyHostToDevice, stream);
            if (e == cudaSuccess) e = cudaMemcpyAsync(node_box + made, tb.data(), tb.size() * sizeof(Box6), cudaMemcpyHostToDevice, stream);
            if (e == cudaSuccess) e = cudaStreamSynchronize(stream);
            if (e != cudaSuccess) return e;
        } else {
            e = cudaMemcpyAsync(&root_node, cn, sizeof(int), cudaMemcpyDeviceToHost, stream);
            if (e == cudaSuccess) e = cudaStreamSynchronize(stream);
            if (e != cudaSuccess) return e;
        }
        if (root_node < 0) return cudaErrorUnknown;
    }
    const int2 root = make_int2(root_node, 0);
    const int init[2] = {1, 0};
    e = cudaMemcpyAsync(fr_a, &root, sizeof root, cudaMemcpyHostToDevice, stream);
    if (e == cudaSuccess) e = cudaMemcpyAsync(counters, init, sizeof init, cudaMemcpyHostToDevice, stream);
    if (e != cudaSuccess) return e;
    int nfrontier = 1, levels = 0;
    int2 *cur = fr_a, *nxt = fr_b;
    while (nfrontier > 0) {
        ++levels;
        k_lbvh_collapse<<<(nfrontier + B - 1) / B, B, 0, stream>>>(child, node_box, leaf_box, n, leaf_base, cur, nfrontier, nxt, counters, node_base, out_nodes);
        int host_counters[2];
        e = cudaMemcpyAsync(host_counters, counters, sizeof host_counters, cudaMemcpyDeviceToHost, stream);
        if (e == cudaSuccess) e = cudaStreamSynchronize(stream);
        if (e != cudaSuccess) return e;
        nfrontier = host_counters[1];
        *nnodes = host_counters[0];
        const int zero = 0;
        e = cudaMemcpyAsync(counters + 1, &zero, sizeof zero, cudaMemcpyHostToDevice, stream);
        if (e != cudaSuccess) return e;
        std::swap(cur, nxt);
        if (levels > 200) { if (why) *why = "the 4-wide collapse exceeded 200 levels"; return cudaErrorUnknown; }
    }
    *depth = levels;
    return cudaGetLastError();
}

}
```

### pathtracerap_b200/csrc/bvh_traverse.cuh

```cuda
#pragma once
#include "kernels.cuh"

namespace ptap {
namespace bvh {

constexpr unsigned kFull = 0xffffffffu;
constexpr int kDone = (int)0x80000000u;
constexpr unsigned kEnterBit = 0x20000000u, kExitBit = 0x40000000u, kIndexMask = 0x1fffffffu;
__device__ __forceinline__ float2 fma2(float2 a, float2 b, float2 c)
{
    unsigned long long ra = *reinterpret_cast<unsigned long long*>(&a), rb = *reinterpret_cast<unsigned long long*>(&b), rc = *reinterpret_cast<unsigned long long*>(&c), rd;
    asm("fma.rn.f32x2 %0, %1, %2, %3;" : "=l"(rd) : "l"(ra), "l"(rb), "l"(rc));
    return *reinterpret_cast<float2*>(&rd);
}

__device__ __forceinline__ uint4 ldg4u(const void* p)
{
    uint4 r;
    asm("ld.global.nc.v4.u32 {%0,%1,%2,%3}, [%4];" : "=r"(r.x), "=r"(r.y), "=r"(r.z), "=r"(r.w) : "l"(p));
    return r;
}

__device__ __forceinline__ int childKey(float nx, float ny, float nz, float fx, float fy, float fz, float tmin, float tmax)
{
    const float tn = fmaxf(fmaxf(fmaxf(nx, ny), nz), tmin);
    const float tf = fminf(fminf(fminf(fx, fy), fz), tmax);
    const bool h = tn <= tf + __fmaf_rn(fabsf(tf), 2e-6f, 1e-6f);
    return h ? __float_as_int(fmaxf(tn, 0.0f)) : 0x7f800000;
}

__device__ __forceinline__ unsigned nearOffsets(const V3& d)
{
    const unsigned sx = __float_as_uint(d.x) >> 31, sy = __float_as_uint(d.y) >> 31, sz = __float_as_uint(d.z) >> 31;
    return (32u + (sx << 4)) | ((64u + (sy << 4)) << 8) | ((96u + (sz << 4)) << 16);
}

__device__ __forceinline__ float safeInv(float d)
{
    const float ooeps = 1e-30f;
    return __fdividef(1.0f, fabsf(d) > ooeps ? d : copysignf(ooeps, d));
}

__device__ __forceinline__ float worldBound(float g_dist, float prune, float cb)
{
    return g_dist < kFloatMax ? g_dist * prune + cb + 1e-3f : 3.0e38f;
}

__device__ __forceinline__ void nodeChildren(const char* __restrict__ np, const V3& ro, const V3& rinv, unsigned near_off, float tmin, float tmax, int key[4], int lnk[4])
{
    const F8 hd = ldg8(np);
    const unsigned nox = near_off & 0xffu, noy = (near_off >> 8) & 0xffu, noz = near_off >> 16;
    const uint4 NX = ldg4u(np + nox), FX = ldg4u(np + (nox ^ 16u));
    const uint4 NY = ldg4u(np + noy), FY = ldg4u(np + (noy ^ 16u));
    const uint4 NZ = ldg4u(np + noz), FZ = ldg4u(np + (noz ^ 16u));
    const float cx = (hd.v[0] - ro.x) * rinv.x, cy = (hd.v[1] - ro.y) * rinv.y, cz = (hd.v[2] - ro.z) * rinv.z;
    const float2 ix = make_float2(rinv.x, rinv.x), iy = make_float2(rinv.y, rinv.y), iz = make_float2(rinv.z, rinv.z);
    const float2 ccx = make_float2(cx, cx), ccy = make_float2(cy, cy), ccz = make_float2(cz, cz);
    const float2 nxa = fma2(make_float2(__uint_as_float(NX.x), __uint_as_float(NX.y)), ix, ccx), nxb = fma2(make_float2(__uint_as_float(NX.z), __uint_as_float(NX.w)), ix, ccx);
    const float2 nya = fma2(make_float2(__uint_as_float(NY.x), __uint_as_float(NY.y)), iy, ccy), nyb = fma2(make_float2(__uint_as_float(NY.z), __uint_as_float(NY.w)), iy, ccy);
    const float2 nza = fma2(make_float2(__uint_as_float(NZ.x), __uint_as_float(NZ.y)), iz, ccz), nzb = fma2(make_float2(__uint_as_float(NZ.z), __uint_as_float(NZ.w)), iz, ccz);
    const float2 fxa = fma2(make_float2(__uint_as_float(FX.x), __uint_as_float(FX.y)), ix, ccx), fxb = fma2(make_float2(__uint_as_float(FX.z), __uint_as_float(FX.w)), ix, ccx);
    const float2 fya = fma2(make_float2(__uint_as_float(FY.x), __uint_as_float(FY.y)), iy, ccy), fyb = fma2(make_float2(__uint_as_float(FY.z), __uint_as_float(FY.w)), iy, ccy);
    const float2 fza = fma2(make_float2(__uint_as_float(FZ.x), __uint_as_float(FZ.y)), iz, ccz), fzb = fma2(make_float2(__uint_as_float(FZ.z), __uint_as_float(FZ.w)), iz, ccz);
    key[0] = childKey(nxa.x, nya.x, nza.x, fxa.x, fya.x, fza.x, tmin, tmax);
    key[1] = childKey(nxa.y, nya.y, nza.y, fxa.y, fya.y, fza.y, tmin, tmax);
    key[2] = childKey(nxb.x, nyb.x, nzb.x, fxb.x, fyb.x, fzb.x, tmin, tmax);
    key[3] = childKey(nxb.y, nyb.y, nzb.y, fxb.y, fyb.y, fzb.y, tmin, tmax);
#pragma unroll
    for (int c = 0; c < 4; ++c) lnk[c] = __float_as_int(hd.v[4 + c]);
#define PTAP_CSWAP(a, b) { const bool sw = key[b] < key[a]; const int ka = sw ? key[b] : key[a], kb = sw ? key[a] : key[b]; \
                           const int la = sw ? lnk[b] : lnk[a], lb = sw ? lnk[a] : lnk[b]; key[a] = ka; key[b] = kb; lnk[a] = la; lnk[b] = lb; }
    PTAP_CSWAP(0, 1) PTAP_CSWAP(2, 3) PTAP_CSWAP(0, 2) PTAP_CSWAP(1, 3) PTAP_CSWAP(1, 2)
#undef PTAP_CSWAP
}

}
}
```

### pathtracerap_b200/csrc/device_types.h

```cpp
#pragma once
#include <cuda_runtime.h>
#include <stdint.h>

namespace ptap {

constexpr float kEpsilon = 0.005f;
constexpr float kFloatMax = 9999999.0f;
constexpr float kFloatMin = -9999990.0f;
constexpr int kAnyOccluded = -2;
constexpr int kMaxDepth = 16;
constexpr int kBigHits = 108;
constexpr int kEmuHits = 8;
constexpr int kBvhStack = 160;

struct InstanceTrace {
    float4 w2m[3];
    float4 m2w[3];
    float4 bb_min;
    float4 bb_max;
    float4 grid;
};

struct InstanceShade {
    float4 nm0;
    float4 nm1;
    float4 nm2;
    int4 mat;
};

struct TriRec {
    float4 v0;
    float4 e1;
    float4 e2;
};

struct __align__(32) LeafTri {
    float v0[3], e1[3], e2[3];
    int id;
    int pad[6];
};

struct Bvh2Node {
    float4 xy0;
    float4 xy1;
    float4 z01;
    int4 link;
};

struct __align__(32) BvhNode {
    float px, py, pz;
    int pad;
    int link[4];
    float planes[3][2][4];
};
static_assert(sizeof(BvhNode) == 128, "BvhNode must be one 128-byte line");

struct FrameState {
    int n_active[kMaxDepth + 2];
    unsigned int ticket[kMaxDepth + 2];
    unsigned int fetch[kMaxDepth + 2];
    unsigned int n_replay[kMaxDepth + 2];
    unsigned int fetch_replay[kMaxDepth + 2];
    unsigned int n_walk[kMaxDepth + 2];
    unsigned int fetch_walk[kMaxDepth + 2];
    unsigned int fetch_emu[kMaxDepth + 2];
    unsigned int n_cont[kMaxDepth + 2];
    int iter_cur, iter_next;
    int cache_valid;
    int pad;
    unsigned long long rays_traced;
    unsigned long long rays_walked;
    unsigned long long rays_reemulated;
    unsigned long long paths;
    unsigned long long count_nodes, count_tris, count_cells, count_refs;
};

struct SceneDev {
    const InstanceTrace* inst;
    const InstanceShade* shade;
    const TriRec* tris;
    const float4* normals;
    const int2* cells;
    const int* refs;
    const int2* tri_box;
    const BvhNode* nodes;
    const LeafTri* bvh_tris;
    const int* bvh_tri_id;
    int nmodels;
    int gx, gy, gz;
    int tlas_root;
    float tmin_world;
    int batch;
    int shade_sort;
    int vote_grid;
    int emu_refill;
    int vote_tri, vote_inst, vote_refill;
    float c_pad;
    float tie;
    float prune;
};

struct EmuBuf {
    int* n;
    int* id;
    float* t;
    int* list;
    int* list2;
    uint4* cont;
    uint4* big;
    int stride;
    int cont_cap;
};

struct WaveDev {
    float4* O[2];
    float4* D[2];
    float4* C[2];
    float4* hit;
    float4* hit_cache;
    float2* uv;
    EmuBuf emu;
    float* film;
    float* contrib;
    unsigned long long* tile_status;
    int* tile_offset;
    unsigned* tile_ballot;
    unsigned char* perm;
    FrameState* st;
    int W, H, N, depth, ntiles, nscan;
    float step_x, step_y;
    float cam_o[3], cam_p[3];
    int jitter; unsigned jitter_seed;
    int iter_stride;
};

}
```

### pathtracerap_b200/csrc/kernels.cuh

```cuda
#pragma once
#include <string>

#include "device_types.h"
#include "exact_math.cuh"
#include "../../include/ptap.h"

namespace ptap {

#ifndef PTAP_TRACE_BLOCK
#define PTAP_TRACE_BLOCK 128
#endif
constexpr int kTraceBlock = PTAP_TRACE_BLOCK;
constexpr int kShadeBlock = 256;
constexpr int kShadeTile = 32;
constexpr int kScanBlock = 256, kScanSlots = 2048, kScanTiles = kScanSlots / kShadeTile;
constexpr int kGenBlock = 256;
constexpr int kMaxLanes = 8, kDefaultLanes = 4, kSmallFrameLanes = 8;
constexpr int kTraceBatch = 32;
constexpr int kVoteTri = 8, kVoteInst = 6, kVoteRefill = 8;
constexpr int kVoteGrid = 5;

__device__ __forceinline__ unsigned long long globalTimerNs()
{
    unsigned long long t;
    asm volatile("mov.u64 %0, %%globaltimer;" : "=l"(t));
    return t;
}

__device__ __forceinline__ float exactHitDistance(const SceneDev& sc, V3 bo, V3 bd, int im, float t)
{
    const InstanceTrace* __restrict__ inst = &sc.inst[im];
    const float4 w0 = ldg4(&inst->w2m[0]), w1 = ldg4(&inst->w2m[1]), w2 = ldg4(&inst->w2m[2]);
    const V3 ro = xmat4(w0, w1, w2, bo, 1.0f);
    const V3 rd = xnormalize(xmat4(w0, w1, w2, bd, 0.0f));
    const V3 nd = xnormalize(rd);
    const V3 pm = xadd(ro, xscale(nd, t));
    const V3 pw = xmat4(ldg4(&inst->m2w[0]), ldg4(&inst->m2w[1]), ldg4(&inst->m2w[2]), pm, 1.0f);
    return xlength(xsub(pw, bo));
}

void launchTraceGrid(const SceneDev& sc, const float4* O, const float4* D, float4* hit, float2* uv, int4* counts, bool count_totals,
                     FrameState* st, int round, int n_fixed, int grid, cudaStream_t stream, unsigned long long* stamp = nullptr, const int* list = nullptr);
void launchTraceEmu(const SceneDev& sc, const float4* O, const float4* D, float4* hit, float2* uv, int4* counts, bool count_totals,
                    FrameState* st, int round, int n_fixed, int grid, int grid_replay, int grid_full, cudaStream_t stream, unsigned long long* stamp, const EmuBuf& emu);
int traceEmuOccupancy();
int gridTriBoxes(const int2* cells, const int* refs, int ngrids, const int* grid_first_cell, int gx, int gy, int gz, int ntris, int2* tri_box,
                 int* grid_tri_range_host, int* ok, cudaStream_t stream);
int traceGridOccupancy();
void launchTraceBvh(const SceneDev& sc, const float4* O, const float4* D, float4* hit, float2* uv, int4* counts, bool count_totals,
                    FrameState* st, int round, int n_fixed, int grid, cudaStream_t stream, unsigned long long* stamp = nullptr);
int traceBvhOccupancy();
void launchTraceBvhAny(const SceneDev& sc, const float4* O, const float4* D, float4* hit, FrameState* st, int n, int grid, cudaStream_t stream);

size_t deviceBvhScratchBytes(int ntris);
int buildMeshBvhDevice(const TriRec* d_tris, int t0, int t1, const float* bb_min, const float* bb_max, int node_base, BvhNode* out_nodes, int leaf_base,
                       LeafTri* btris, int* btid, char* scratch, size_t scratch_bytes, cudaStream_t stream, int* nnodes, int* depth,
                       std::string* why);

int gridDeviceCount(const float* d_pos, int t0, int n, const float bb_min[3], const float width[3], const int gd[3], int* d_count, int* d_offset,
                    void* d_tmp, size_t tmp_bytes, cudaStream_t stream, long long* npairs);
int gridDeviceFill(const float* d_pos, int t0, int n, const float bb_min[3], const float width[3], const int gd[3], const int* d_offset, int npairs,
                   int* d_keys, int* d_vals, int* d_keys2, void* d_tmp, size_t tmp_bytes, int ref_base, int* d_refs, int2* d_cells, cudaStream_t stream);
size_t gridDeviceTempBytes(int ntris, long long npairs);

void launchGenerate(const WaveDev& wv, int iter , int grid, cudaStream_t stream);
void launchScan(const SceneDev& sc, const WaveDev& wv, int round, const float4* hit, int remaining, int n_fixed, cudaStream_t stream);
void launchShade(const SceneDev& sc, const WaveDev& wv, int round, int in_buf, const float4* hit, int remaining, int n_fixed,
                 int iter_fixed, int* slot_pos, int grid, cudaStream_t stream);
int shadeOccupancy();
void launchResolveHits(const SceneDev& sc, const float4* O, const float4* D, const float4* hit, const float2* uv, int n, PtapHit* out, cudaStream_t stream);
void launchResolveOccluded(const SceneDev& sc, const float4* O, const float4* D, const float4* hit, int n, uint8_t* occluded, cudaStream_t stream);
void launchSetIter(FrameState* st, int iter, cudaStream_t stream);
void launchFilmAdd(float* film, const float* add, size_t n, cudaStream_t stream);
void launchResolveBmp(const float* film, size_t nvalues, float div, unsigned char* out, cudaStream_t stream);
void launchResolveBox(const float* film, int W, int H, int sx, int sy, float* out, cudaStream_t stream);
void launchExtractNormals(const TriRec* tris, int n, float4* normals, cudaStream_t stream);
void launchGatherTris(const TriRec* tris, const int* tri_id, int n, LeafTri* out, cudaStream_t stream);

}
```

### pathtracerap_b200/csrc/trace_bvh.cu

```cuda
#include "bvh_traverse.cuh"

namespace ptap {

using namespace bvh;

namespace {

#ifndef PTAP_TRACE_MIN_CTAS
#define PTAP_TRACE_MIN_CTAS 8
#endif
#ifndef PTAP_NODE_LDG256
#define PTAP_NODE_LDG256 0
#endif
#ifndef PTAP_COLD_SMEM
#define PTAP_COLD_SMEM 0
#endif
#ifndef PTAP_SMEM_STACK
#define PTAP_SMEM_STACK 12
#endif
constexpr int kSmemStack = PTAP_SMEM_STACK;
#ifndef PTAP_NODE_STEPS
#define PTAP_NODE_STEPS 1
#endif
constexpr int kNodeSteps = PTAP_NODE_STEPS;

template <bool UV, bool COUNT>
__device__ __forceinline__ void leafTriangle(const SceneDev& sc, const V3& o, const V3& d, float& tmax, int& best_tri, float& best_u, float& best_v,
                                             int k, int4& cnt)
{
    const F8 ta = ldg8(&sc.bvh_tris[k]), tb = ldg8(reinterpret_cast<const char*>(&sc.bvh_tris[k]) + 32);
    if (COUNT) cnt.z++;
    const V3 v0 = v3(ta.v[0], ta.v[1], ta.v[2]), v0v1 = v3(ta.v[3], ta.v[4], ta.v[5]), v0v2 = v3(ta.v[6], ta.v[7], tb.v[0]);
    const V3 pvec = xcross(d, v0v2);
    const float det = xdot(v0v1, pvec);
    const float invDet = xdiv(1.0f, det);
    const V3 tvec = xsub(o, v0);
    const float u = xmul(xdot(tvec, pvec), invDet);
    const V3 qvec = xcross(tvec, v0v1);
    const float v = xmul(xdot(d, qvec), invDet);
    const float t = xmul(xdot(v0v2, qvec), invDet);
    const bool reject = (xabs(xsub(det, 0.0f)) < kEpsilon) | (u < (0.0f - kEpsilon)) | (u > (1.0f + kEpsilon)) |
                        (v < (0.0f - kEpsilon)) | (xadd(u, v) > (1.0f + kEpsilon)) | (t < (0.0f - kEpsilon)) | (t > tmax);
    if (reject || !(t <= tmax)) return;
    const int id = __float_as_int(tb.v[1]);
    if (t < tmax || (best_tri >= 0 && id < best_tri)) { tmax = t; best_tri = id; if (UV) { best_u = u; best_v = v; } }
}

}

template <bool UV, bool COUNT, bool ANY = false>
__global__ void __launch_bounds__(kTraceBlock, PTAP_TRACE_MIN_CTAS)
k_trace_bvh(SceneDev sc, const float4* __restrict__ O, const float4* __restrict__ D, float4* __restrict__ hit,
            float2* __restrict__ uv, int4* __restrict__ counts, FrameState* st, int round, int n_fixed, unsigned long long* __restrict__ stamp)
{
    const int n = n_fixed >= 0 ? n_fixed : st->n_active[round];
    if (blockIdx.x == 0 && threadIdx.x == 0 && n_fixed < 0) st->rays_traced += (unsigned long long)n;
    if (stamp && threadIdx.x == 0) atomicMin(stamp, globalTimerNs());
    unsigned int* cursor = &st->fetch[round];
    const int lane = threadIdx.x & 31;
    unsigned long long tot_x = 0, tot_z = 0;
    int4 cnt = make_int4(0, 0, 0, 0);

    if (sc.tlas_root < 0) {
        for (int k = blockIdx.x * blockDim.x + threadIdx.x; k < n; k += gridDim.x * blockDim.x) {
            hit[k] = make_float4(kFloatMax, __int_as_float(-1), __int_as_float(-1), 0.0f);
            if (UV && uv) uv[k] = make_float2(0.0f, 0.0f);
            if (COUNT && counts) counts[k] = cnt;
        }
        return;
    }

    int sp = 0;
    __shared__ int s_stack[kSmemStack > 0 ? kSmemStack * kTraceBlock : 1];
    int l_stack[kBvhStack > kSmemStack ? kBvhStack - kSmemStack : 1];
    auto push = [&](int v) {
        if (kSmemStack > 0 && sp < kSmemStack) s_stack[sp * kTraceBlock + threadIdx.x] = v; else l_stack[sp - kSmemStack] = v;
        ++sp;
    };
    auto pop = [&]() {
        --sp;
        return (kSmemStack > 0 && sp < kSmemStack) ? s_stack[sp * kTraceBlock + threadIdx.x] : l_stack[sp - kSmemStack];
    };
    int node = kDone, i = -1;
#if PTAP_COLD_SMEM
    __shared__ float s_cold[16 * kTraceBlock];
    float* const cold = s_cold + threadIdx.x;
#define CF(k) cold[(k) * kTraceBlock]
#else
    float cold_regs[16];
#define CF(k) cold_regs[k]
#endif
#define C_BO v3(CF(0), CF(1), CF(2))
#define C_BD v3(CF(3), CF(4), CF(5))
#define C_WINV v3(CF(6), CF(7), CF(8))
#define C_WNEAR CF(9)
#define g_dist CF(10)
#define g_t CF(11)
#define g_model_f CF(12)
#define g_tri_f CF(13)
#define g_u CF(14)
#define g_v CF(15)
    unsigned near_off = 0u;
    V3 ro = v3(0, 0, 0), rd = v3(0, 0, 1), rinv = v3(0, 0, 0);
    float tmin = 0.0f, tmax = 0.0f;
    int best_tri = -1; float best_u = 0.0f, best_v = 0.0f;
    int w_next = 0, w_end = 0;
    bool exhausted = false;
    const int vote_tri = sc.vote_tri, vote_inst = sc.vote_inst, vote_refill = sc.vote_refill;
    float any_len = 0.0f, any_cb = 0.0f, any_scale = 0.0f;

    for (;;) {
#pragma unroll
        for (int rep = 0; rep < kNodeSteps; ++rep) {
            if (node >= 0) {
                const char* __restrict__ np = reinterpret_cast<const char*>(&sc.nodes[node]);
                const F8 hd = ldg8(np);
#if PTAP_NODE_LDG256
                const F8 px8 = ldg8(np + 32), py8 = ldg8(np + 64), pz8 = ldg8(np + 96);
                if (COUNT) cnt.x++;
                const float cx = (hd.v[0] - ro.x) * rinv.x, cy = (hd.v[1] - ro.y) * rinv.y, cz = (hd.v[2] - ro.z) * rinv.z;
                const float2 ix = make_float2(rinv.x, rinv.x), iy = make_float2(rinv.y, rinv.y), iz = make_float2(rinv.z, rinv.z);
                const float2 ccx = make_float2(cx, cx), ccy = make_float2(cy, cy), ccz = make_float2(cz, cz);
                const float2 lxa = fma2(make_float2(px8.v[0], px8.v[1]), ix, ccx), lxb = fma2(make_float2(px8.v[2], px8.v[3]), ix, ccx), hxa = fma2(make_float2(px8.v[4], px8.v[5]), ix, ccx), hxb = fma2(make_float2(px8.v[6], px8.v[7]), ix, ccx);
                const float2 lya = fma2(make_float2(py8.v[0], py8.v[1]), iy, ccy), lyb = fma2(make_float2(py8.v[2], py8.v[3]), iy, ccy), hya = fma2(make_float2(py8.v[4], py8.v[5]), iy, ccy), hyb = fma2(make_float2(py8.v[6], py8.v[7]), iy, ccy);
                const float2 lza = fma2(make_float2(pz8.v[0], pz8.v[1]), iz, ccz), lzb = fma2(make_float2(pz8.v[2], pz8.v[3]), iz, ccz), hza = fma2(make_float2(pz8.v[4], pz8.v[5]), iz, ccz), hzb = fma2(make_float2(pz8.v[6], pz8.v[7]), iz, ccz);
#define PTAP_MM(l, h, c) fminf(l.c, h.c), fmaxf(l.c, h.c)
                const float2 nxa = make_float2(fminf(lxa.x, hxa.x), fminf(lxa.y, hxa.y)), fxa = make_float2(fmaxf(lxa.x, hxa.x), fmaxf(lxa.y, hxa.y));
                const float2 nxb = make_float2(fminf(lxb.x, hxb.x), fminf(lxb.y, hxb.y)), fxb = make_float2(fmaxf(lxb.x, hxb.x), fmaxf(lxb.y, hxb.y));
                const float2 nya = make_float2(fminf(lya.x, hya.x), fminf(lya.y, hya.y)), fya = make_float2(fmaxf(lya.x, hya.x), fmaxf(lya.y, hya.y));
                const float2 nyb = make_float2(fminf(lyb.x, hyb.x), fminf(lyb.y, hyb.y)), fyb = make_float2(fmaxf(lyb.x, hyb.x), fmaxf(lyb.y, hyb.y));
                const float2 nza = make_float2(fminf(lza.x, hza.x), fminf(lza.y, hza.y)), fza = make_float2(fmaxf(lza.x, hza.x), fmaxf(lza.y, hza.y));
                const float2 nzb = make_float2(fminf(lzb.x, hzb.x), fminf(lzb.y, hzb.y)), fzb = make_float2(fmaxf(lzb.x, hzb.x), fmaxf(lzb.y, hzb.y));
#undef PTAP_MM
#else
                const unsigned nox = near_off & 0xffu, noy = (near_off >> 8) & 0xffu, noz = near_off >> 16;
                const uint4 NX = ldg4u(np + nox), FX = ldg4u(np + (nox ^ 16u));
                const uint4 NY = ldg4u(np + noy), FY = ldg4u(np + (noy ^ 16u));
                const uint4 NZ = ldg4u(np + noz), FZ = ldg4u(np + (noz ^ 16u));
                if (COUNT) cnt.x++;
                const float cx = (hd.v[0] - ro.x) * rinv.x, cy = (hd.v[1] - ro.y) * rinv.y, cz = (hd.v[2] - ro.z) * rinv.z;
                const float2 ix = make_float2(rinv.x, rinv.x), iy = make_float2(rinv.y, rinv.y), iz = make_float2(rinv.z, rinv.z);
                const float2 ccx = make_float2(cx, cx), ccy = make_float2(cy, cy), ccz = make_float2(cz, cz);
                const float2 nxa = fma2(make_float2(__uint_as_float(NX.x), __uint_as_float(NX.y)), ix, ccx), nxb = fma2(make_float2(__uint_as_float(NX.z), __uint_as_float(NX.w)), ix, ccx);
                const float2 nya = fma2(make_float2(__uint_as_float(NY.x), __uint_as_float(NY.y)), iy, ccy), nyb = fma2(make_float2(__uint_as_float(NY.z), __uint_as_float(NY.w)), iy, ccy);
                const float2 nza = fma2(make_float2(__uint_as_float(NZ.x), __uint_as_float(NZ.y)), iz, ccz), nzb = fma2(make_float2(__uint_as_float(NZ.z), __uint_as_float(NZ.w)), iz, ccz);
                const float2 fxa = fma2(make_float2(__uint_as_float(FX.x), __uint_as_float(FX.y)), ix, ccx), fxb = fma2(make_float2(__uint_as_float(FX.z), __uint_as_float(FX.w)), ix, ccx);
                const float2 fya = fma2(make_float2(__uint_as_float(FY.x), __uint_as_float(FY.y)), iy, ccy), fyb = fma2(make_float2(__uint_as_float(FY.z), __uint_as_float(FY.w)), iy, ccy);
                const float2 fza = fma2(make_float2(__uint_as_float(FZ.x), __uint_as_float(FZ.y)), iz, ccz), fzb = fma2(make_float2(__uint_as_float(FZ.z), __uint_as_float(FZ.w)), iz, ccz);
#endif
                int key[4], lnk[4];
                key[0] = childKey(nxa.x, nya.x, nza.x, fxa.x, fya.x, fza.x, tmin, tmax);
                key[1] = childKey(nxa.y, nya.y, nza.y, fxa.y, fya.y, fza.y, tmin, tmax);
                key[2] = childKey(nxb.x, nyb.x, nzb.x, fxb.x, fyb.x, fzb.x, tmin, tmax);
                key[3] = childKey(nxb.y, nyb.y, nzb.y, fxb.y, fyb.y, fzb.y, tmin, tmax);
#pragma unroll
                for (int c = 0; c < 4; ++c) lnk[c] = __float_as_int(hd.v[4 + c]);
                if (!ANY) {
#define PTAP_CSWAP(a, b) { const bool sw = key[b] < key[a]; const int ka = sw ? key[b] : key[a], kb = sw ? key[a] : key[b]; \
                           const int la = sw ? lnk[b] : lnk[a], lb = sw ? lnk[a] : lnk[b]; key[a] = ka; key[b] = kb; lnk[a] = la; lnk[b] = lb; }
                    PTAP_CSWAP(0, 1) PTAP_CSWAP(2, 3) PTAP_CSWAP(0, 2) PTAP_CSWAP(1, 3) PTAP_CSWAP(1, 2)
#undef PTAP_CSWAP
                }
                if (key[3] != 0x7f800000) push(lnk[3]);
                if (key[2] != 0x7f800000) push(lnk[2]);
                if (key[1] != 0x7f800000) push(lnk[1]);
                if (key[0] != 0x7f800000) node = lnk[0]; else node = pop();
            }
        }
        const unsigned code = ~(unsigned)node;
        const unsigned state = min(code >> 29, 4u);
        const bool live = state != 3u || i >= 0 || !exhausted;
        const unsigned sum = __reduce_add_sync(kFull, live ? 1u << (6u * state) : 0u);
        if (sum == 0u) break;
        const int n_tri = sum & 63u, n_enter = (sum >> 6) & 63u, n_exit = (sum >> 12) & 63u, n_done = (sum >> 18) & 63u, n_inner = (sum >> 24) & 63u;
        const bool s_tri = state == 0u, s_enter = state == 1u, s_exit = state == 2u, s_done = state == 3u;

        if (s_tri && n_tri >= min(vote_tri, n_inner)) {
            leafTriangle<UV, COUNT>(sc, ro, rd, tmax, best_tri, best_u, best_v, (int)(code >> 3), cnt);
            if constexpr (ANY) {
                bool occluded = false;
                if (best_tri >= 0) {
                    const float m = fmaxf(fabsf(tmax), kEpsilon) * any_scale;
                    occluded = m + (m * sc.tie + any_cb) < any_len;
                }
                if (occluded) { sp = 0; node = kDone; g_model_f = __int_as_float(kAnyOccluded); }
                else if (code & 7u) node = (int)~(code + 7u); else node = pop();
            } else {
                if (code & 7u) node = (int)~(code + 7u); else node = pop();
            }
        }
        if (s_enter && n_enter >= min(vote_inst, n_inner)) {
            const int im = (int)(code & kIndexMask);
            const InstanceTrace* __restrict__ inst = &sc.inst[im];
            const float4 w0 = ldg4(&inst->w2m[0]), w1 = ldg4(&inst->w2m[1]), w2 = ldg4(&inst->w2m[2]);
            const V3 bo = C_BO, bd = C_BD;
            ro = xmat4(w0, w1, w2, bo, 1.0f);
            const V3 dm = xmat4(w0, w1, w2, bd, 0.0f);
            const float mlen = xsqrt(xdot(dm, dm));
            rd = xscale(dm, xdiv(1.0f, mlen));
            rinv = v3(safeInv(rd.x), safeInv(rd.y), safeInv(rd.z));
            near_off = nearOffsets(rd);
            const float wil = rsqrtf(bd.x * bd.x + bd.y * bd.y + bd.z * bd.z);
            tmin = -(kEpsilon + 1e-4f);
            tmax = kFloatMax; best_tri = -1;
            if (g_dist < kFloatMax) {
                const float tb = (g_dist * sc.prune + sc.c_pad + 1e-4f * (fabsf(bo.x) + fabsf(bo.y) + fabsf(bo.z))) * (mlen * wil) * 1.0001f;
                if (tb < kFloatMax) tmax = tb;
            }
            if constexpr (ANY) any_scale = __fdividef(1.0f, mlen * wil);
            push(__float_as_int(__fdividef(1.0f, mlen * wil)));
            push((int)~(kExitBit | (unsigned)im));
            node = __float_as_int(__ldg(&inst->grid.z));
        }
        if (s_exit && n_exit >= min(vote_inst, n_inner)) {
            const int im = (int)(code & kIndexMask);
            const float ascale = __int_as_float(pop());
            const V3 bo = C_BO, bd = C_BD;
            const int g_model = __float_as_int(g_model_f);
            const float cb = sc.c_pad + 1e-4f * (fabsf(bo.x) + fabsf(bo.y) + fabsf(bo.z));
            if (best_tri >= 0) {
                const float a = fabsf(tmax * ascale);
                const float a_lo = a - (fabsf(a) * sc.tie + cb), a_hi = a + (fabsf(a) * sc.tie + cb);
                const float g_lo = g_dist - (g_dist * sc.tie + cb), g_hi = g_dist + (g_dist * sc.tie + cb);
                bool take;
                float nd = a;
                if (a_hi < g_lo && a_hi < 0.99f * kFloatMax) take = true;
                else if ((ANY || g_model >= 0) && a_lo > g_hi) take = false;
                else {
                    const float dn = exactHitDistance(sc, bo, bd, im, tmax);
                    const float dg = g_model >= 0 ? exactHitDistance(sc, bo, bd, g_model, g_t) : ANY ? g_dist : kFloatMax;
                    take = dg > dn || (dg == dn && g_model >= 0 && im < g_model);
                    nd = dn;
                    if (!take && g_model >= 0) g_dist = dg;
                }
                if (take) {
                    g_dist = nd; g_model_f = __int_as_float(im); g_tri_f = __int_as_float(best_tri); g_t = tmax;
                    if (UV) { g_u = best_u; g_v = best_v; }
                }
            }
            ro = bo; rinv = C_WINV; near_off = __float_as_uint(C_WNEAR);
            tmin = sc.tmin_world; tmax = worldBound(g_dist, sc.prune, cb);
            node = pop();
        }
        if (n_done > 0 && n_done >= min(vote_refill, n_inner)) {
            const unsigned m_done = __ballot_sync(kFull, s_done && live);
            if (s_done && i >= 0) {
                const bool found = g_dist < kFloatMax;
                if constexpr (ANY) {
                    const bool cand = __float_as_int(g_model_f) >= 0;
                    hit[i] = make_float4(cand ? -1.0f : kFloatMax, cand ? g_tri_f : __int_as_float(-1), g_model_f, g_t);
                } else {
                    hit[i] = make_float4(found ? -1.0f : kFloatMax, found ? g_tri_f : __int_as_float(-1), found ? g_model_f : __int_as_float(-1), g_t);
                }
                if (UV && uv) uv[i] = make_float2(g_u, g_v);
                if (COUNT) { if (counts) counts[i] = cnt; tot_x += cnt.x; tot_z += cnt.z; }
                i = -1;
            }
            if (w_next >= w_end && !exhausted) {
                unsigned b = 0;
                if (lane == 0) b = atomicAdd(cursor, (unsigned)sc.batch);
                b = __shfl_sync(kFull, b, 0);
                if (b >= (unsigned)n) { exhausted = true; w_next = w_end = n; }
                else { w_next = (int)b; w_end = min((int)b + sc.batch, n); }
            }
            const int avail = w_end - w_next;
            const int rank = __popc(m_done & ((1u << lane) - 1u));
            if (s_done && live && rank < avail) {
                i = w_next + rank;
                const float4 o4 = O[i], d4 = D[i];
                const V3 bo = v3(o4), bd = v3(d4);
                const float il = rsqrtf(bd.x * bd.x + bd.y * bd.y + bd.z * bd.z);
                const V3 winv = v3(safeInv(bd.x * il), safeInv(bd.y * il), safeInv(bd.z * il));
                const unsigned wnear_off = nearOffsets(bd);
                CF(0) = bo.x; CF(1) = bo.y; CF(2) = bo.z; CF(3) = bd.x; CF(4) = bd.y; CF(5) = bd.z;
                CF(6) = winv.x; CF(7) = winv.y; CF(8) = winv.z; C_WNEAR = __uint_as_float(wnear_off);
                ro = bo; rinv = winv; near_off = wnear_off;
                tmin = sc.tmin_world; tmax = 3.0e38f;
                g_dist = kFloatMax; g_model_f = __int_as_float(-1); g_tri_f = __int_as_float(-1); g_t = 0.0f; g_u = 0.0f; g_v = 0.0f;
                best_tri = -1;
                if (COUNT) cnt = make_int4(0, 0, 0, 0);
                sp = 0; push(kDone);
                node = sc.tlas_root;
                if constexpr (ANY) {
                    any_len = d4.w > kFloatMax ? kFloatMax : d4.w;
                    any_cb = sc.c_pad + 1e-4f * (fabsf(bo.x) + fabsf(bo.y) + fabsf(bo.z));
                    if (any_len < kFloatMax) { g_dist = any_len; tmax = worldBound(any_len, sc.prune, any_cb); }
                    if (!(any_len > 0.0f)) node = pop();
                }
            }
            w_next += min(__popc(m_done), avail);
        }
    }
    if (stamp && (threadIdx.x & 31) == 0) atomicMax(stamp + 1, globalTimerNs());
    if (COUNT) {
#pragma unroll
        for (int d = 16; d > 0; d >>= 1) { tot_x += __shfl_xor_sync(kFull, tot_x, d); tot_z += __shfl_xor_sync(kFull, tot_z, d); }
        if (lane == 0) { atomicAdd(&st->count_nodes, tot_x); atomicAdd(&st->count_tris, tot_z); }
    }
}

#undef CF
#undef C_BO
#undef C_BD
#undef C_WINV
#undef C_WNEAR
#undef g_dist
#undef g_t
#undef g_model_f
#undef g_tri_f
#undef g_u
#undef g_v

void launchTraceBvhAny(const SceneDev& sc, const float4* O, const float4* D, float4* hit, FrameState* st, int n, int grid, cudaStream_t stream)
{
    k_trace_bvh<false, false, true><<<grid, kTraceBlock, 0, stream>>>(sc, O, D, hit, nullptr, nullptr, st, 0, n, nullptr);
}

void launchTraceBvh(const SceneDev& sc, const float4* O, const float4* D, float4* hit, float2* uv, int4* counts, bool count_totals,
                     FrameState* st, int round, int n_fixed, int grid, cudaStream_t stream, unsigned long long* stamp)
{
    if (counts || count_totals) k_trace_bvh<true, true><<<grid, kTraceBlock, 0, stream>>>(sc, O, D, hit, uv, counts, st, round, n_fixed, stamp);
    else if (uv) k_trace_bvh<true, false><<<grid, kTraceBlock, 0, stream>>>(sc, O, D, hit, uv, counts, st, round, n_fixed, stamp);
    else k_trace_bvh<false, false><<<grid, kTraceBlock, 0, stream>>>(sc, O, D, hit, uv, counts, st, round, n_fixed, stamp);
}

int traceBvhOccupancy()
{
    int nb = 0;
    cudaOccupancyMaxActiveBlocksPerMultiprocessor(&nb, k_trace_bvh<false, false>, kTraceBlock, 0);
    return nb;
}

}
```

### pathtracerap_b200/csrc/trace_emu.cu

```cuda
#include "bvh_traverse.cuh"

namespace ptap {

using namespace bvh;

namespace {

#ifndef PTAP_EMU_MIN_CTAS
#define PTAP_EMU_MIN_CTAS 7
#endif
#ifndef PTAP_EMU_FULL_BATCH
#define PTAP_EMU_FULL_BATCH 8
#endif
constexpr int kFullBatch = PTAP_EMU_FULL_BATCH;
constexpr int kFullHits = 20;
constexpr int kEmuStack = 12;
constexpr int kReplayBlock = 128, kReplayBatch = 32;
constexpr int kSetupBlock = 128;
#ifndef PTAP_EMU_SETUP_STEPS
#define PTAP_EMU_SETUP_STEPS 2
#endif
#ifndef PTAP_EMU_BURST
#define PTAP_EMU_BURST 8
#endif
constexpr int kBurst = PTAP_EMU_BURST;
#ifndef PTAP_EMU_SETUP_BURST
#define PTAP_EMU_SETUP_BURST PTAP_EMU_BURST
#endif
constexpr int kSetupBurst = PTAP_EMU_SETUP_BURST;
constexpr int kSetupSteps = PTAP_EMU_SETUP_STEPS;
constexpr unsigned kGuard = 0x20080200u;

}

template <bool COUNT>
__global__ void __launch_bounds__(kTraceBlock, PTAP_EMU_MIN_CTAS)
k_trace_emu(SceneDev sc, const float4* __restrict__ O, const float4* __restrict__ D, float4* __restrict__ hit,
            int4* __restrict__ counts, FrameState* st, int round, int n_fixed, unsigned long long* __restrict__ stamp, EmuBuf emu)
{
    const int n = n_fixed >= 0 ? n_fixed : st->n_active[round];
    if (blockIdx.x == 0 && threadIdx.x == 0 && n_fixed < 0) st->rays_traced += (unsigned long long)n;
    if (stamp && threadIdx.x == 0) atomicMin(stamp, globalTimerNs());
    unsigned int* cursor = &st->fetch[round];
    const int lane = threadIdx.x & 31;
    unsigned long long tot_x = 0, tot_z = 0;
    int4 cnt = make_int4(0, 0, 0, 0);

    if (sc.tlas_root < 0) {
        for (int k = blockIdx.x * blockDim.x + threadIdx.x; k < n; k += gridDim.x * blockDim.x) {
            hit[k] = make_float4(kFloatMax, __int_as_float(-1), __int_as_float(-1), 0.0f);
            emu.n[k] = 0;
            if (COUNT && counts) counts[k] = cnt;
        }
        return;
    }

    int sp = 0;
    __shared__ int s_stack[kEmuStack * kTraceBlock];
    int l_stack[kBvhStack - kEmuStack];
    auto push = [&](int v) { if (sp < kEmuStack) s_stack[sp * kTraceBlock + threadIdx.x] = v; else l_stack[sp - kEmuStack] = v; ++sp; };
    auto pop = [&]() { --sp; return sp < kEmuStack ? s_stack[sp * kTraceBlock + threadIdx.x] : l_stack[sp - kEmuStack]; };
    __shared__ int s_id[2 * kEmuHits * kTraceBlock];
    __shared__ float s_t[2 * kEmuHits * kTraceBlock];
    int cur = 0, nh = 0, nh_best = 0;
    int n_amb = 0; bool best_amb = false;
    float c_t = kFloatMax; int c_tri = -1;

    int node = kDone, i = -1;
    V3 bo = v3(0, 0, 0), bd = v3(0, 0, 0);
    V3 winv = v3(0, 0, 0);
    unsigned near_off = 0u, wnear_off = 0u;
    V3 ro = v3(0, 0, 0), rd = v3(0, 0, 1), rinv = v3(0, 0, 0);
    float tmin = 0.0f, tmax = 0.0f;
    float g_dist = kFloatMax, g_t = 0.0f;
    int g_model = -1, g_tri = -1;
    int w_next = 0, w_end = 0;
    bool exhausted = false;
    const int vote_tri = sc.vote_tri, vote_inst = sc.vote_inst, vote_refill = sc.vote_refill;

    for (;;) {
        if (node >= 0) {
            int key[4], lnk[4];
            nodeChildren(reinterpret_cast<const char*>(&sc.nodes[node]), ro, rinv, near_off, tmin, tmax, key, lnk);
            if (COUNT) cnt.x++;
            if (key[3] != 0x7f800000) push(lnk[3]);
            if (key[2] != 0x7f800000) push(lnk[2]);
            if (key[1] != 0x7f800000) push(lnk[1]);
            if (key[0] != 0x7f800000) node = lnk[0]; else node = pop();
        }
        const unsigned code = ~(unsigned)node;
        const unsigned state = min(code >> 29, 4u);
        const bool live = state != 3u || i >= 0 || !exhausted;
        const unsigned sum = __reduce_add_sync(kFull, live ? 1u << (6u * state) : 0u);
        if (sum == 0u) break;
        const int n_tri = sum & 63u, n_enter = (sum >> 6) & 63u, n_exit = (sum >> 12) & 63u, n_done = (sum >> 18) & 63u, n_inner = (sum >> 24) & 63u;
        const bool s_tri = state == 0u, s_enter = state == 1u, s_exit = state == 2u, s_done = state == 3u;

        if (s_tri && n_tri >= min(vote_tri, n_inner)) {
            const int k = (int)(code >> 3);
            const F8 ta = ldg8(&sc.bvh_tris[k]), tb = ldg8(reinterpret_cast<const char*>(&sc.bvh_tris[k]) + 32);
            if (COUNT) cnt.z++;
            const V3 v0 = v3(ta.v[0], ta.v[1], ta.v[2]), v0v1 = v3(ta.v[3], ta.v[4], ta.v[5]), v0v2 = v3(ta.v[6], ta.v[7], tb.v[0]);
            const V3 pvec = xcross(rd, v0v2);
            const float det = xdot(v0v1, pvec);
            const float invDet = xdiv(1.0f, det);
            const V3 tvec = xsub(ro, v0);
            const float u = xmul(xdot(tvec, pvec), invDet);
            const V3 qvec = xcross(tvec, v0v1);
            const float v = xmul(xdot(rd, qvec), invDet);
            const float t = xmul(xdot(v0v2, qvec), invDet);
            const bool reject = (xabs(xsub(det, 0.0f)) < kEpsilon) | (u < (0.0f - kEpsilon)) | (u > (1.0f + kEpsilon)) |
                                (v < (0.0f - kEpsilon)) | (xadd(u, v) > (1.0f + kEpsilon)) | (t < (0.0f - kEpsilon));
            if (!reject) {
                const int id = __float_as_int(tb.v[1]);
                if (nh < kEmuHits) {
                    const int slot = ((cur * kEmuHits + nh) * kTraceBlock) + threadIdx.x;
                    s_id[slot] = id; s_t[slot] = t;
                }
                ++nh;
                if (t < c_t || (t == c_t && c_tri >= 0 && id < c_tri)) { c_t = t; c_tri = id; }
            }
            if (code & 7u) node = (int)~(code + 7u); else node = pop();
        }
        if (s_enter && n_enter >= min(vote_inst, n_inner)) {
            const int im = (int)(code & kIndexMask);
            const InstanceTrace* __restrict__ inst = &sc.inst[im];
            const float4 w0 = ldg4(&inst->w2m[0]), w1 = ldg4(&inst->w2m[1]), w2 = ldg4(&inst->w2m[2]);
            ro = xmat4(w0, w1, w2, bo, 1.0f);
            const V3 dm = xmat4(w0, w1, w2, bd, 0.0f);
            const float mlen = xsqrt(xdot(dm, dm));
            rd = xscale(dm, xdiv(1.0f, mlen));
            rinv = v3(safeInv(rd.x), safeInv(rd.y), safeInv(rd.z));
            near_off = nearOffsets(rd);
            const float wil = rsqrtf(bd.x * bd.x + bd.y * bd.y + bd.z * bd.z);
            tmin = -(kEpsilon + 1e-4f);
            tmax = 3.0e38f;
            nh = 0; c_t = kFloatMax; c_tri = -1;
            push(__float_as_int(__fdividef(1.0f, mlen * wil)));
            push((int)~(kExitBit | (unsigned)im));
            node = __float_as_int(__ldg(&inst->grid.z));
        }
        if (s_exit && n_exit >= min(vote_inst, n_inner)) {
            const int im = (int)(code & kIndexMask);
            const float ascale = __int_as_float(pop());
            const float cb = sc.c_pad + 1e-4f * (fabsf(bo.x) + fabsf(bo.y) + fabsf(bo.z));
            const bool amb = c_tri >= 0 && c_t < 0.0f && nh >= 2;
            if (amb) ++n_amb;
            if (c_tri >= 0) {
                const float a = fabsf(c_t * ascale);
                const float a_lo = a - (fabsf(a) * sc.tie + cb), a_hi = a + (fabsf(a) * sc.tie + cb);
                const float g_lo = g_dist - (g_dist * sc.tie + cb), g_hi = g_dist + (g_dist * sc.tie + cb);
                bool take;
                float nd = a;
                if (a_hi < g_lo && a_hi < 0.99f * kFloatMax) take = true;
                else if (g_model >= 0 && a_lo > g_hi) take = false;
                else {
                    const float dn = exactHitDistance(sc, bo, bd, im, c_t);
                    const float dg = g_model >= 0 ? exactHitDistance(sc, bo, bd, g_model, g_t) : kFloatMax;
                    take = dg > dn || (dg == dn && g_model >= 0 && im < g_model);
                    nd = dn;
                    if (!take && g_model >= 0) g_dist = dg;
                }
                if (take) {
                    g_dist = nd; g_model = im; g_tri = c_tri; g_t = c_t;
                    nh_best = nh; cur ^= 1;
                    best_amb = amb;
                }
            }
            nh = 0; c_t = kFloatMax; c_tri = -1;
            ro = bo; rinv = winv; near_off = wnear_off;
            tmin = sc.tmin_world; tmax = worldBound(g_dist, sc.prune, cb);
            node = pop();
        }
        if (n_done > 0 && n_done >= min(vote_refill, n_inner)) {
            const unsigned m_done = __ballot_sync(kFull, s_done && live);
            if (s_done && i >= 0) {
                const bool found = g_model >= 0;
                hit[i] = make_float4(found ? -1.0f : kFloatMax, __int_as_float(found ? g_tri : -1), __int_as_float(found ? g_model : -1), g_t);
                emu.n[i] = !found ? 0 : n_amb > (best_amb ? 1 : 0) ? kEmuHits + 1 : nh_best;
                if (found && nh_best > 1) {
                    const int kept = min(nh_best, kEmuHits), base = (cur ^ 1) * kEmuHits;
                    for (int j = 0; j < kept; ++j) {
                        const int slot = (base + j) * kTraceBlock + threadIdx.x;
                        emu.id[(size_t)j * emu.stride + i] = s_id[slot]; emu.t[(size_t)j * emu.stride + i] = s_t[slot];
                    }
                }
                if (COUNT) { if (counts) counts[i] = cnt; tot_x += cnt.x; tot_z += cnt.z; }
                i = -1;
            }
            if (w_next >= w_end && !exhausted) {
                unsigned b = 0;
                if (lane == 0) b = atomicAdd(cursor, (unsigned)sc.batch);
                b = __shfl_sync(kFull, b, 0);
                if (b >= (unsigned)n) { exhausted = true; w_next = w_end = n; }
                else { w_next = (int)b; w_end = min((int)b + sc.batch, n); }
            }
            const int avail = w_end - w_next;
            const int rank = __popc(m_done & ((1u << lane) - 1u));
            if (s_done && live && rank < avail) {
                i = w_next + rank;
                const float4 o4 = O[i], d4 = D[i];
                bo = v3(o4); bd = v3(d4);
                const float il = rsqrtf(bd.x * bd.x + bd.y * bd.y + bd.z * bd.z);
                winv = v3(safeInv(bd.x * il), safeInv(bd.y * il), safeInv(bd.z * il));
                wnear_off = nearOffsets(bd);
                ro = bo; rinv = winv; near_off = wnear_off;
                tmin = sc.tmin_world; tmax = 3.0e38f;
                g_dist = kFloatMax; g_model = -1; g_tri = -1; g_t = 0.0f;
                nh = 0; nh_best = 0; c_t = kFloatMax; c_tri = -1; n_amb = 0; best_amb = false;
                if (COUNT) cnt = make_int4(0, 0, 0, 0);
                sp = 0; push(kDone);
                node = sc.tlas_root;
            }
            w_next += min(__popc(m_done), avail);
        }
    }
    if (stamp && (threadIdx.x & 31) == 0) atomicMax(stamp + 1, globalTimerNs());
    if (COUNT) {
#pragma unroll
        for (int d = 16; d > 0; d >>= 1) { tot_x += __shfl_xor_sync(kFull, tot_x, d); tot_z += __shfl_xor_sync(kFull, tot_z, d); }
        if (lane == 0) { atomicAdd(&st->count_nodes, tot_x); atomicAdd(&st->count_tris, tot_z); }
    }
}

namespace {

struct Replay {
    int i, nh, ix, iy, iz, cx, cy, cz, k, best_k, w_tri, steps;
    unsigned ulo, uhi, gpos, seen;
    float tmx, tmy, tmz, dx, dy, dz, w_t, t_star;
    bool inter, passed;
};

template <int BURST = kBurst>
__device__ __forceinline__ bool replayStep(Replay& r, int GX, int GY, int GZ, const unsigned* s_lo, const unsigned* s_hi, const float* s_ts, const int* s_ids, int stride)
{
    ++r.steps;
    const unsigned gneg = kGuard ^ r.gpos;
    const unsigned v = (unsigned)r.ix | ((unsigned)r.iy << 10) | ((unsigned)r.iz << 20);
    bool any = false, finished = false;
    const unsigned u1 = (v | kGuard) - r.ulo, u2 = (r.uhi | kGuard) - v;
    if ((u1 & u2 & kGuard) == kGuard) {
#pragma unroll 1
        for (int j = 0; j < r.nh; ++j) {
            const int slot = j * stride + threadIdx.x;
            const unsigned d1 = (v | kGuard) - s_lo[slot], d2 = (s_hi[slot] | kGuard) - v;
            if ((d1 & d2 & kGuard) == kGuard) {
                any = true;
                if (!((r.seen >> j) & 1u)) {
                    r.seen |= 1u << j;
                    const float tj = s_ts[slot]; const int idj = s_ids[slot];
                    if (r.w_t > tj || (r.w_t == tj && r.best_k == r.k && idj < r.w_tri)) { r.w_t = tj; r.w_tri = idj; r.best_k = r.k; }
                }
            }
        }
    } else if ((~u2 & r.gpos) | (~u1 & gneg)) r.passed = true;
    if (r.w_t == r.t_star) finished = true;
    else {
        if (any) { r.cx = r.ix; r.cy = r.iy; r.cz = r.iz; r.inter = true; }
        if (r.inter && (abs(r.cx - r.ix) > 2 || abs(r.cy - r.iy) > 2 || abs(r.cz - r.iz) > 2)) finished = true;
        else if (r.passed) finished = true;
        else {
            const bool px = r.gpos & (1u << 9), py = r.gpos & (1u << 19), pz = r.gpos & (1u << 29);
            const bool sx = r.tmx < r.tmy && r.tmx < r.tmz, sy = !sx && r.tmy < r.tmz;
            r.ix += sx ? (px ? 1 : -1) : 0; r.iy += sy ? (py ? 1 : -1) : 0; r.iz += (sx || sy) ? 0 : (pz ? 1 : -1);
            const float tsel = sx ? r.tmx : sy ? r.tmy : r.tmz;
            const int isel = sx ? r.ix : sy ? r.iy : r.iz, lim = sx ? (px ? GX : -1) : sy ? (py ? GY : -1) : (pz ? GZ : -1);
            if (isel == lim || tsel >= kFloatMax) finished = true;
            else { r.tmx = sx ? xadd(r.tmx, r.dx) : r.tmx; r.tmy = sy ? xadd(r.tmy, r.dy) : r.tmy; r.tmz = (sx || sy) ? r.tmz : xadd(r.tmz, r.dz); }
        }
    }
    ++r.k;
#pragma unroll 1
    for (int b = 0; b < BURST && !finished; ++b) {
        const unsigned w = (unsigned)r.ix | ((unsigned)r.iy << 10) | ((unsigned)r.iz << 20);
        const unsigned q1 = (w | kGuard) - r.ulo, q2 = (r.uhi | kGuard) - w;
        if ((q1 & q2 & kGuard) == kGuard) break;
        ++r.steps;
        if ((~q2 & r.gpos) | (~q1 & gneg)) finished = true;
        else if (r.inter && (abs(r.cx - r.ix) > 2 || abs(r.cy - r.iy) > 2 || abs(r.cz - r.iz) > 2)) finished = true;
        else {
            const bool px = r.gpos & (1u << 9), py = r.gpos & (1u << 19), pz = r.gpos & (1u << 29);
            const bool sx = r.tmx < r.tmy && r.tmx < r.tmz, sy = !sx && r.tmy < r.tmz;
            r.ix += sx ? (px ? 1 : -1) : 0; r.iy += sy ? (py ? 1 : -1) : 0; r.iz += (sx || sy) ? 0 : (pz ? 1 : -1);
            const float tsel = sx ? r.tmx : sy ? r.tmy : r.tmz;
            const int isel = sx ? r.ix : sy ? r.iy : r.iz, lim = sx ? (px ? GX : -1) : sy ? (py ? GY : -1) : (pz ? GZ : -1);
            if (isel == lim || tsel >= kFloatMax) finished = true;
            else { r.tmx = sx ? xadd(r.tmx, r.dx) : r.tmx; r.tmy = sy ? xadd(r.tmy, r.dy) : r.tmy; r.tmz = (sx || sy) ? r.tmz : xadd(r.tmz, r.dz); }
        }
        ++r.k;
    }
    return finished;
}

__device__ __forceinline__ bool replayEnter(const InstanceTrace* __restrict__ inst, const V3& ro, const V3& rd, int GX, int GY, int GZ, Replay& r)
{
    const float4 bbmin_wx = ldg4(&inst->bb_min), bbmax_wy = ldg4(&inst->bb_max), gridrec = ldg4(&inst->grid);
    const V3 mn = v3(bbmin_wx), mx = v3(bbmax_wy);
    const V3 inv = v3(xdiv(1.0f, rd.x), xdiv(1.0f, rd.y), xdiv(1.0f, rd.z));
    const float t1 = rd.x == 0.0f ? kFloatMin : xmul(xsub(mn.x, ro.x), inv.x);
    const float t2 = rd.x == 0.0f ? kFloatMax : xmul(xsub(mx.x, ro.x), inv.x);
    const float t3 = rd.y == 0.0f ? kFloatMin : xmul(xsub(mn.y, ro.y), inv.y);
    const float t4 = rd.y == 0.0f ? kFloatMax : xmul(xsub(mx.y, ro.y), inv.y);
    const float t5 = rd.z == 0.0f ? kFloatMin : xmul(xsub(mn.z, ro.z), inv.z);
    const float t6 = rd.z == 0.0f ? kFloatMax : xmul(xsub(mx.z, ro.z), inv.z);
    const float sl_min = max_std(max_std(min_std(t1, t2), min_std(t3, t4)), min_std(t5, t6));
    const float sl_max = min_std(min_std(max_std(t1, t2), max_std(t3, t4)), max_std(t5, t6));
    const V3 p = xadd(ro, xscale(rd, sl_min));
    if ((sl_max < 0 || sl_min > sl_max) || (xsub(p.x, mn.x) < -kEpsilon || xsub(p.y, mn.y) < -kEpsilon || xsub(p.z, mn.z) < -kEpsilon)) return false;
    const float wx = bbmin_wx.w, wy = bbmax_wy.w, wz = gridrec.x;
    r.ix = f2i_x86(xdiv(xabs(xadd(xsub(p.x, mn.x), kEpsilon)), wx));
    r.iy = f2i_x86(xdiv(xabs(xadd(xsub(p.y, mn.y), kEpsilon)), wy));
    r.iz = f2i_x86(xdiv(xabs(xadd(xsub(p.z, mn.z), kEpsilon)), wz));
    r.ix = min(max(r.ix, 0), GX - 1); r.iy = min(max(r.iy, 0), GY - 1); r.iz = min(max(r.iz, 0), GZ - 1);
    r.tmx = kFloatMax; r.tmy = kFloatMax; r.tmz = kFloatMax; r.dx = kFloatMax; r.dy = kFloatMax; r.dz = kFloatMax;
    if (rd.x != 0) { const int nx = rd.x > 0.0f ? r.ix + 1 : r.ix; r.dx = xabs(xmul(wx, inv.x)); r.tmx = xmul(xsub(xadd(mn.x, xmul((float)nx, wx)), p.x), inv.x); }
    if (rd.y != 0) { const int ny = rd.y > 0.0f ? r.iy + 1 : r.iy; r.dy = xabs(xmul(wy, inv.y)); r.tmy = xmul(xsub(xadd(mn.y, xmul((float)ny, wy)), p.y), inv.y); }
    if (rd.z != 0) { const int nz = rd.z > 0.0f ? r.iz + 1 : r.iz; r.dz = xabs(xmul(wz, inv.z)); r.tmz = xmul(xsub(xadd(mn.z, xmul((float)nz, wz)), p.z), inv.z); }
    r.gpos = (rd.x > 0.0f ? 1u << 9 : 0u) | (rd.y > 0.0f ? 1u << 19 : 0u) | (rd.z > 0.0f ? 1u << 29 : 0u);
    r.seen = 0u; r.passed = false; r.cx = 0; r.cy = 0; r.cz = 0; r.best_k = -1; r.k = 0; r.inter = false;
    return true;
}

__device__ __forceinline__ void replayLoadHits(const SceneDev& sc, const EmuBuf& emu, int i, int nh, int first_id, float t_star, unsigned& ulo, unsigned& uhi,
                                               unsigned* s_lo, unsigned* s_hi, float* s_ts, int* s_ids, int stride)
{
    ulo = 0x1ffu | (0x1ffu << 10) | (0x1ffu << 20); uhi = 0u;
#pragma unroll 1
    for (int j = 0; j < nh; ++j) {
        const int slot = j * stride + threadIdx.x;
        const int idj = nh == 1 ? first_id : emu.id[(size_t)j * emu.stride + i];
        s_ids[slot] = idj; s_ts[slot] = nh == 1 ? t_star : emu.t[(size_t)j * emu.stride + i];
        const int2 bx = __ldg(&sc.tri_box[idj]);
        const unsigned lj = (unsigned)bx.x, hj = (unsigned)bx.y;
        s_lo[slot] = lj; s_hi[slot] = hj;
        if ((((hj | kGuard) - lj) & kGuard) == kGuard) {
            ulo = min(ulo & 0x1ffu, lj & 0x1ffu) | min(ulo & (0x1ffu << 10), lj & (0x1ffu << 10)) | min(ulo & (0x1ffu << 20), lj & (0x1ffu << 20));
            uhi = max(uhi & 0x1ffu, hj & 0x1ffu) | max(uhi & (0x1ffu << 10), hj & (0x1ffu << 10)) | max(uhi & (0x1ffu << 20), hj & (0x1ffu << 20));
        }
    }
}

template <bool UV>
__device__ __forceinline__ void replayFinish(const SceneDev& sc, const Replay& r, const float4& h, const float4* __restrict__ O, const float4* __restrict__ D,
                                             float4* __restrict__ hit, float2* __restrict__ uv, FrameState* st, int round, const EmuBuf& emu)
{
    if (r.w_tri >= 0 && r.w_t == r.t_star) {
        if (r.w_tri != __float_as_int(h.y)) hit[r.i] = make_float4(h.x, __int_as_float(r.w_tri), h.z, h.w);
        if (UV && uv) {
            const InstanceTrace* __restrict__ inst = &sc.inst[__float_as_int(h.z)];
            const float4 w0 = ldg4(&inst->w2m[0]), w1 = ldg4(&inst->w2m[1]), w2 = ldg4(&inst->w2m[2]);
            const V3 ro = xmat4(w0, w1, w2, v3(O[r.i]), 1.0f), rd = xnormalize(xmat4(w0, w1, w2, v3(D[r.i]), 0.0f));
            const float4 a = ldg4(&sc.tris[r.w_tri].v0), b = ldg4(&sc.tris[r.w_tri].e1), c = ldg4(&sc.tris[r.w_tri].e2);
            const V3 pvec = xcross(rd, v3(c));
            const float invDet = xdiv(1.0f, xdot(v3(b), pvec));
            const V3 tvec = xsub(ro, v3(a));
            uv[r.i] = make_float2(xmul(xdot(tvec, pvec), invDet), xmul(xdot(rd, xcross(tvec, v3(b))), invDet));
        }
    } else emu.list[atomicAdd(&st->n_replay[round], 1u)] = r.i;
}

}

template <bool UV, bool COUNT>
__global__ void __launch_bounds__(kSetupBlock)
k_emu_setup(SceneDev sc, const float4* __restrict__ O, const float4* __restrict__ D, float4* __restrict__ hit, float2* __restrict__ uv,
            int4* __restrict__ counts, FrameState* st, int round, int n_fixed, EmuBuf emu)
{
    const int n = n_fixed >= 0 ? n_fixed : st->n_active[round];
    const int GX = sc.gx, GY = sc.gy, GZ = sc.gz;
    __shared__ int s_ids[kEmuHits * kSetupBlock];
    __shared__ float s_ts[kEmuHits * kSetupBlock];
    __shared__ unsigned s_lo[kEmuHits * kSetupBlock], s_hi[kEmuHits * kSetupBlock];
    unsigned long long steps_total = 0;
    for (int i = blockIdx.x * blockDim.x + threadIdx.x; i < n; i += gridDim.x * blockDim.x) {
        const float4 h = hit[i];
        const int im = __float_as_int(h.z);
        if (im < 0) { if (UV && uv) uv[i] = make_float2(0.0f, 0.0f); continue; }
        Replay r;
        r.i = i; r.nh = emu.n[i]; r.t_star = h.w; r.w_tri = -1; r.w_t = kFloatMax; r.steps = 0;
        bool walking = false;
        if (r.nh <= kEmuHits) {
            const V3 bo = v3(O[i]), bd = v3(D[i]);
            const InstanceTrace* __restrict__ inst = &sc.inst[im];
            const float4 w0 = ldg4(&inst->w2m[0]), w1 = ldg4(&inst->w2m[1]), w2 = ldg4(&inst->w2m[2]);
            const V3 ro = xmat4(w0, w1, w2, bo, 1.0f);
            const V3 rd = xnormalize(xmat4(w0, w1, w2, bd, 0.0f));
            if (replayEnter(inst, ro, rd, GX, GY, GZ, r)) {
                replayLoadHits(sc, emu, i, r.nh, __float_as_int(h.y), r.t_star, r.ulo, r.uhi, s_lo, s_hi, s_ts, s_ids, kSetupBlock);
                walking = true;
#pragma unroll 1
                for (int s = 0; s < kSetupSteps && walking; ++s) walking = !replayStep<kSetupBurst>(r, GX, GY, GZ, s_lo, s_hi, s_ts, s_ids, kSetupBlock);
            }
        }
        if (walking) {
            const unsigned q = atomicAdd(&st->n_cont[round], 1u);
            if (q < (unsigned)emu.cont_cap) {
                uint4* rec = emu.cont + (size_t)q * 5;
                rec[0] = make_uint4((unsigned)i, (unsigned)r.ix | ((unsigned)r.iy << 10) | ((unsigned)r.iz << 20), r.gpos | (r.inter ? 1u : 0u) | ((unsigned)r.nh << 1), r.seen);
                rec[1] = make_uint4(__float_as_uint(r.tmx), __float_as_uint(r.tmy), __float_as_uint(r.tmz), __float_as_uint(r.t_star));
                rec[2] = make_uint4(__float_as_uint(r.dx), __float_as_uint(r.dy), __float_as_uint(r.dz), __float_as_uint(r.w_t));
                rec[3] = make_uint4((unsigned)r.w_tri, (unsigned)r.best_k, (unsigned)r.k, (unsigned)r.cx | ((unsigned)r.cy << 10) | ((unsigned)r.cz << 20));
                rec[4] = make_uint4(r.ulo, r.uhi, (unsigned)r.steps, 0u);
                continue;
            }
            r.w_tri = -1;
        }
        if (COUNT) { if (counts) counts[i].y = r.steps; steps_total += r.steps; }
        replayFinish<UV>(sc, r, h, O, D, hit, uv, st, round, emu);
    }
    if (COUNT) {
#pragma unroll
        for (int d = 16; d > 0; d >>= 1) steps_total += __shfl_xor_sync(0xffffffffu, steps_total, d);
        if ((threadIdx.x & 31) == 0) atomicAdd(&st->count_cells, steps_total);
    }
}

template <bool UV, bool COUNT>
__global__ void __launch_bounds__(kReplayBlock)
k_emu_tail(SceneDev sc, const float4* __restrict__ O, const float4* __restrict__ D, float4* __restrict__ hit, float2* __restrict__ uv,
           int4* __restrict__ counts, FrameState* st, int round, EmuBuf emu)
{
    constexpr unsigned kFullMask = 0xffffffffu;
    const int n = (int)min(st->n_cont[round], (unsigned)emu.cont_cap);
    unsigned int* cursor = &st->fetch_emu[round];
    const int lane = threadIdx.x & 31;
    const int GX = sc.gx, GY = sc.gy, GZ = sc.gz;
    __shared__ int s_ids[kEmuHits * kReplayBlock];
    __shared__ float s_ts[kEmuHits * kReplayBlock];
    __shared__ unsigned s_lo[kEmuHits * kReplayBlock], s_hi[kEmuHits * kReplayBlock];
    unsigned long long steps_total = 0;
    enum : int { R_IDLE = 0, R_STEP = 1, R_DONE = 2 };
    int state = R_IDLE;
    Replay r; r.i = -1; r.nh = 0; r.steps = 0;
    int w_next = 0, w_end = 0;
    bool exhausted = false;

    for (;;) {
        if (state == R_STEP && replayStep(r, GX, GY, GZ, s_lo, s_hi, s_ts, s_ids, kReplayBlock)) state = R_DONE;
        const unsigned m_step = __ballot_sync(kFullMask, state == R_STEP);
        if (m_step != 0u && 32 - __popc(m_step) < sc.emu_refill) continue;
        if (state == R_DONE) {
            if (COUNT) { if (counts) counts[r.i].y = r.steps; steps_total += r.steps; }
            replayFinish<UV>(sc, r, hit[r.i], O, D, hit, uv, st, round, emu);
            state = R_IDLE; r.i = -1;
        }
        if (w_next >= w_end && !exhausted) {
            unsigned b = 0;
            if (lane == 0) b = atomicAdd(cursor, (unsigned)kReplayBatch);
            b = __shfl_sync(kFullMask, b, 0);
            if (b >= (unsigned)n) { exhausted = true; w_next = w_end = n; }
            else { w_next = (int)b; w_end = min((int)b + kReplayBatch, n); }
        }
        const unsigned m_idle = __ballot_sync(kFullMask, state == R_IDLE);
        if (m_step == 0u && exhausted && w_next >= w_end) break;
        const int avail = w_end - w_next;
        const int rank = __popc(m_idle & ((1u << lane) - 1u));
        if (state == R_IDLE && rank < avail) {
            const uint4* rec = emu.cont + (size_t)(w_next + rank) * 5;
            const uint4 a = rec[0], b = rec[1], c = rec[2], d = rec[3], e = rec[4];
            r.i = (int)a.x; r.ix = a.y & 0x3ff; r.iy = (a.y >> 10) & 0x3ff; r.iz = a.y >> 20;
            r.gpos = a.z & kGuard; r.inter = a.z & 1u; r.nh = (a.z >> 1) & 0xf; r.seen = a.w; r.passed = false;
            r.tmx = __uint_as_float(b.x); r.tmy = __uint_as_float(b.y); r.tmz = __uint_as_float(b.z); r.t_star = __uint_as_float(b.w);
            r.dx = __uint_as_float(c.x); r.dy = __uint_as_float(c.y); r.dz = __uint_as_float(c.z); r.w_t = __uint_as_float(c.w);
            r.w_tri = (int)d.x; r.best_k = (int)d.y; r.k = (int)d.z; r.cx = d.w & 0x3ff; r.cy = (d.w >> 10) & 0x3ff; r.cz = d.w >> 20;
            r.steps = (int)e.z;
            const float4 h = hit[r.i];
            replayLoadHits(sc, emu, r.i, r.nh, __float_as_int(h.y), r.t_star, r.ulo, r.uhi, s_lo, s_hi, s_ts, s_ids, kReplayBlock);
            state = R_STEP;
        }
        w_next += min(__popc(m_idle), avail);
    }
    if (COUNT) {
#pragma unroll
        for (int d = 16; d > 0; d >>= 1) steps_total += __shfl_xor_sync(kFullMask, steps_total, d);
        if (lane == 0) atomicAdd(&st->count_cells, steps_total);
    }
}

template <bool UV>
__global__ void __launch_bounds__(kTraceBlock, 4)
k_emu_full(SceneDev sc, const float4* __restrict__ O, const float4* __restrict__ D, float4* __restrict__ hit, float2* __restrict__ uv,
           FrameState* st, int round, EmuBuf emu)
{
    uint4* __restrict__ big = emu.big + (size_t)(blockIdx.x * blockDim.x + threadIdx.x) * kBigHits;
    const int n = (int)st->n_replay[round];
    if (blockIdx.x == 0 && threadIdx.x == 0) st->rays_reemulated += (unsigned long long)n;
    unsigned int* cursor = &st->fetch_replay[round];
    const int lane = threadIdx.x & 31;
    const int GX = sc.gx, GY = sc.gy, GZ = sc.gz;
    if (n == 0 || sc.tlas_root < 0) return;

    int sp = 0;
    __shared__ int s_stack[kEmuStack * kTraceBlock];
    int l_stack[kBvhStack - kEmuStack];
    auto push = [&](int v) { if (sp < kEmuStack) s_stack[sp * kTraceBlock + threadIdx.x] = v; else l_stack[sp - kEmuStack] = v; ++sp; };
    auto pop = [&]() { --sp; return sp < kEmuStack ? s_stack[sp * kTraceBlock + threadIdx.x] : l_stack[sp - kEmuStack]; };
    __shared__ int s_ids[kFullHits * kTraceBlock];
    __shared__ float s_ts[kFullHits * kTraceBlock];
    __shared__ unsigned s_lo[kFullHits * kTraceBlock], s_hi[kFullHits * kTraceBlock];
    int nh = 0;
    float c_t = kFloatMax;
    bool overflow = false;

    int node = kDone, i = -1;
    V3 bo = v3(0, 0, 0), bd = v3(0, 0, 0), winv = v3(0, 0, 0);
    unsigned near_off = 0u, wnear_off = 0u;
    V3 ro = v3(0, 0, 0), rd = v3(0, 0, 1), rinv = v3(0, 0, 0);
    float tmin = 0.0f, tmax = 0.0f;
    float g_dist = kFloatMax, g_t = 0.0f;
    int g_model = -1, g_tri = -1;
    int w_next = 0, w_end = 0;
    bool exhausted = false;
    const int vote_tri = sc.vote_tri, vote_inst = sc.vote_inst, vote_refill = sc.vote_refill;

    for (;;) {
        if (node >= 0) {
            int key[4], lnk[4];
            nodeChildren(reinterpret_cast<const char*>(&sc.nodes[node]), ro, rinv, near_off, tmin, tmax, key, lnk);
            if (key[3] != 0x7f800000) push(lnk[3]);
            if (key[2] != 0x7f800000) push(lnk[2]);
            if (key[1] != 0x7f800000) push(lnk[1]);
            if (key[0] != 0x7f800000) node = lnk[0]; else node = pop();
        }
        const unsigned code = ~(unsigned)node;
        const unsigned state = min(code >> 29, 4u);
        const bool live = state != 3u || i >= 0 || !exhausted;
        const unsigned sum = __reduce_add_sync(kFull, live ? 1u << (6u * state) : 0u);
        if (sum == 0u) break;
        const int n_tri = sum & 63u, n_enter = (sum >> 6) & 63u, n_exit = (sum >> 12) & 63u, n_done = (sum >> 18) & 63u, n_inner = (sum >> 24) & 63u;
        const bool s_tri = state == 0u, s_enter = state == 1u, s_exit = state == 2u, s_done = state == 3u;

        if (s_tri && n_tri >= min(vote_tri, n_inner)) {
            const int k = (int)(code >> 3);
            const F8 ta = ldg8(&sc.bvh_tris[k]), tb = ldg8(reinterpret_cast<const char*>(&sc.bvh_tris[k]) + 32);
            const V3 v0 = v3(ta.v[0], ta.v[1], ta.v[2]), v0v1 = v3(ta.v[3], ta.v[4], ta.v[5]), v0v2 = v3(ta.v[6], ta.v[7], tb.v[0]);
            const V3 pvec = xcross(rd, v0v2);
            const float det = xdot(v0v1, pvec);
            const float invDet = xdiv(1.0f, det);
            const V3 tvec = xsub(ro, v0);
            const float u = xmul(xdot(tvec, pvec), invDet);
            const V3 qvec = xcross(tvec, v0v1);
            const float v = xmul(xdot(rd, qvec), invDet);
            const float t = xmul(xdot(v0v2, qvec), invDet);
            const bool reject = (xabs(xsub(det, 0.0f)) < kEpsilon) | (u < (0.0f - kEpsilon)) | (u > (1.0f + kEpsilon)) |
                                (v < (0.0f - kEpsilon)) | (xadd(u, v) > (1.0f + kEpsilon)) | (t < (0.0f - kEpsilon));
            if (!reject) {
                if (nh < kFullHits + kBigHits) {
                    const int id = __float_as_int(tb.v[1]);
                    const int2 bx = __ldg(&sc.tri_box[id]);
                    if (nh < kFullHits) {
                        const int slot = nh * kTraceBlock + threadIdx.x;
                        s_ids[slot] = id; s_ts[slot] = t; s_lo[slot] = (unsigned)bx.x; s_hi[slot] = (unsigned)bx.y;
                    } else big[nh - kFullHits] = make_uint4((unsigned)id, __float_as_uint(t), (unsigned)bx.x, (unsigned)bx.y);
                }
                ++nh;
                if (t < c_t) c_t = t;
            }
            if (code & 7u) node = (int)~(code + 7u); else node = pop();
        }
        if (s_enter && n_enter >= min(vote_inst, n_inner)) {
            const int im = (int)(code & kIndexMask);
            const InstanceTrace* __restrict__ inst = &sc.inst[im];
            const float4 w0 = ldg4(&inst->w2m[0]), w1 = ldg4(&inst->w2m[1]), w2 = ldg4(&inst->w2m[2]);
            ro = xmat4(w0, w1, w2, bo, 1.0f);
            rd = xnormalize(xmat4(w0, w1, w2, bd, 0.0f));
            rinv = v3(safeInv(rd.x), safeInv(rd.y), safeInv(rd.z));
            near_off = nearOffsets(rd);
            tmin = -(kEpsilon + 1e-4f); tmax = 3.0e38f;
            nh = 0; c_t = kFloatMax;
            push((int)~(kExitBit | (unsigned)im));
            node = __float_as_int(__ldg(&inst->grid.z));
        }
        if (s_exit && n_exit >= min(vote_inst, n_inner)) {
            const int im = (int)(code & kIndexMask);
            if (nh > kFullHits + kBigHits) overflow = true;
            else if (nh > kFullHits) {
                Replay r;
                r.i = i; r.nh = nh; r.t_star = c_t; r.w_tri = -1; r.w_t = kFloatMax; r.steps = 0;
                if (replayEnter(&sc.inst[im], ro, rd, GX, GY, GZ, r)) {
                    const bool px = r.gpos & (1u << 9), py = r.gpos & (1u << 19), pz = r.gpos & (1u << 29);
                    for (;;) {
                        const unsigned v = (unsigned)r.ix | ((unsigned)r.iy << 10) | ((unsigned)r.iz << 20);
                        bool any = false;
#pragma unroll 1
                        for (int j = 0; j < nh; ++j) {
                            unsigned lj, hj; float tj; int idj; bool was_seen;
                            if (j < kFullHits) {
                                const int slot = j * kTraceBlock + threadIdx.x;
                                lj = s_lo[slot]; hj = s_hi[slot]; tj = s_ts[slot]; idj = s_ids[slot]; was_seen = (r.seen >> j) & 1u;
                            } else {
                                const uint4 e = big[j - kFullHits];
                                idj = (int)e.x; tj = __uint_as_float(e.y); lj = e.z & 0x7fffffffu; hj = e.w; was_seen = e.z >> 31;
                            }
                            const unsigned d1 = (v | kGuard) - lj, d2 = (hj | kGuard) - v;
                            if ((d1 & d2 & kGuard) != kGuard) continue;
                            any = true;
                            if (was_seen) continue;
                            if (j < kFullHits) r.seen |= 1u << j; else big[j - kFullHits].z = lj | 0x80000000u;
                            if (r.w_t > tj || (r.w_t == tj && r.best_k == r.k && idj < r.w_tri)) { r.w_t = tj; r.w_tri = idj; r.best_k = r.k; }
                        }
                        if (r.w_t == r.t_star) break;
                        if (any) { r.cx = r.ix; r.cy = r.iy; r.cz = r.iz; r.inter = true; }
                        if (r.inter && (abs(r.cx - r.ix) > 2 || abs(r.cy - r.iy) > 2 || abs(r.cz - r.iz) > 2)) break;
                        const bool sx = r.tmx < r.tmy && r.tmx < r.tmz, sy = !sx && r.tmy < r.tmz;
                        r.ix += sx ? (px ? 1 : -1) : 0; r.iy += sy ? (py ? 1 : -1) : 0; r.iz += (sx || sy) ? 0 : (pz ? 1 : -1);
                        const float tsel = sx ? r.tmx : sy ? r.tmy : r.tmz;
                        const int isel = sx ? r.ix : sy ? r.iy : r.iz, lim = sx ? (px ? GX : -1) : sy ? (py ? GY : -1) : (pz ? GZ : -1);
                        if (isel == lim || tsel >= kFloatMax) break;
                        r.tmx = sx ? xadd(r.tmx, r.dx) : r.tmx; r.tmy = sy ? xadd(r.tmy, r.dy) : r.tmy; r.tmz = (sx || sy) ? r.tmz : xadd(r.tmz, r.dz);
                        ++r.k;
                    }
                    if (r.w_tri >= 0) {
                        const float dn = exactHitDistance(sc, bo, bd, im, r.w_t);
                        if (g_dist > dn || (g_dist == dn && g_model >= 0 && im < g_model)) { g_dist = dn; g_model = im; g_tri = r.w_tri; g_t = r.w_t; }
                    }
                }
            }
            else if (nh > 0) {
                Replay r;
                r.i = i; r.nh = nh; r.t_star = c_t; r.w_tri = -1; r.w_t = kFloatMax; r.steps = 0;
                if (replayEnter(&sc.inst[im], ro, rd, GX, GY, GZ, r)) {
                    r.ulo = 0x1ffu | (0x1ffu << 10) | (0x1ffu << 20); r.uhi = 0u;
#pragma unroll 1
                    for (int j = 0; j < nh; ++j) {
                        const unsigned lj = s_lo[j * kTraceBlock + threadIdx.x], hj = s_hi[j * kTraceBlock + threadIdx.x];
                        if ((((hj | kGuard) - lj) & kGuard) == kGuard) {
                            r.ulo = min(r.ulo & 0x1ffu, lj & 0x1ffu) | min(r.ulo & (0x1ffu << 10), lj & (0x1ffu << 10)) | min(r.ulo & (0x1ffu << 20), lj & (0x1ffu << 20));
                            r.uhi = max(r.uhi & 0x1ffu, hj & 0x1ffu) | max(r.uhi & (0x1ffu << 10), hj & (0x1ffu << 10)) | max(r.uhi & (0x1ffu << 20), hj & (0x1ffu << 20));
                        }
                    }
#pragma unroll 1
                    while (!replayStep(r, GX, GY, GZ, s_lo, s_hi, s_ts, s_ids, kTraceBlock)) { }
                    if (r.w_tri >= 0) {
                        const float dn = exactHitDistance(sc, bo, bd, im, r.w_t);
                        if (g_dist > dn || (g_dist == dn && g_model >= 0 && im < g_model)) { g_dist = dn; g_model = im; g_tri = r.w_tri; g_t = r.w_t; }
                    }
                }
            }
            nh = 0; c_t = kFloatMax;
            ro = bo; rinv = winv; near_off = wnear_off;
            tmin = sc.tmin_world; tmax = 3.0e38f;
            node = pop();
        }
        if (n_done > 0 && n_done >= min(vote_refill, n_inner)) {
            const unsigned m_done = __ballot_sync(kFull, s_done && live);
            if (s_done && i >= 0) {
                if (overflow) emu.list2[atomicAdd(&st->n_walk[round], 1u)] = i;
                else {
                    const bool found = g_dist < kFloatMax;
                    hit[i] = make_float4(found ? g_dist : kFloatMax, __int_as_float(found ? g_tri : -1), __int_as_float(found ? g_model : -1), found ? g_t : 0.0f);
                    if (UV && uv) {
                        float2 w = make_float2(0.0f, 0.0f);
                        if (found) {
                            const InstanceTrace* __restrict__ inst = &sc.inst[g_model];
                            const float4 w0 = ldg4(&inst->w2m[0]), w1 = ldg4(&inst->w2m[1]), w2 = ldg4(&inst->w2m[2]);
                            const V3 mo = xmat4(w0, w1, w2, bo, 1.0f), md = xnormalize(xmat4(w0, w1, w2, bd, 0.0f));
                            const float4 a = ldg4(&sc.tris[g_tri].v0), b = ldg4(&sc.tris[g_tri].e1), c = ldg4(&sc.tris[g_tri].e2);
                            const V3 pvec = xcross(md, v3(c));
                            const float invDet = xdiv(1.0f, xdot(v3(b), pvec));
                            const V3 tvec = xsub(mo, v3(a));
                            w = make_float2(xmul(xdot(tvec, pvec), invDet), xmul(xdot(md, xcross(tvec, v3(b))), invDet));
                        }
                        uv[i] = w;
                    }
                }
                i = -1;
            }
            if (w_next >= w_end && !exhausted) {
                unsigned b = 0;
                if (lane == 0) b = atomicAdd(cursor, (unsigned)kFullBatch);
                b = __shfl_sync(kFull, b, 0);
                if (b >= (unsigned)n) { exhausted = true; w_next = w_end = n; }
                else { w_next = (int)b; w_end = min((int)b + kFullBatch, n); }
            }
            const int avail = w_end - w_next;
            const int rank = __popc(m_done & ((1u << lane) - 1u));
            if (s_done && live && rank < avail) {
                i = __ldg(&emu.list[w_next + rank]);
                const float4 o4 = O[i], d4 = D[i];
                bo = v3(o4); bd = v3(d4);
                const float il = rsqrtf(bd.x * bd.x + bd.y * bd.y + bd.z * bd.z);
                winv = v3(safeInv(bd.x * il), safeInv(bd.y * il), safeInv(bd.z * il));
                wnear_off = nearOffsets(bd);
                ro = bo; rinv = winv; near_off = wnear_off;
                tmin = sc.tmin_world; tmax = 3.0e38f;
                g_dist = kFloatMax; g_model = -1; g_tri = -1; g_t = 0.0f;
                nh = 0; c_t = kFloatMax; overflow = false;
                sp = 0; push(kDone);
                node = sc.tlas_root;
            }
            w_next += min(__popc(m_done), avail);
        }
    }
}

void launchTraceEmu(const SceneDev& sc, const float4* O, const float4* D, float4* hit, float2* uv, int4* counts, bool count_totals,
                    FrameState* st, int round, int n_fixed, int grid, int grid_replay, int grid_full, cudaStream_t stream, unsigned long long* stamp, const EmuBuf& emu)
{
    const bool count = counts || count_totals;
    const int grid_setup = grid_replay * 2;
    if (count) k_trace_emu<true><<<grid, kTraceBlock, 0, stream>>>(sc, O, D, hit, counts, st, round, n_fixed, stamp, emu);
    else k_trace_emu<false><<<grid, kTraceBlock, 0, stream>>>(sc, O, D, hit, counts, st, round, n_fixed, stamp, emu);
    if (count) {
        k_emu_setup<true, true><<<grid_setup, kSetupBlock, 0, stream>>>(sc, O, D, hit, uv, counts, st, round, n_fixed, emu);
        k_emu_tail<true, true><<<grid_replay, kReplayBlock, 0, stream>>>(sc, O, D, hit, uv, counts, st, round, emu);
    } else if (uv) {
        k_emu_setup<true, false><<<grid_setup, kSetupBlock, 0, stream>>>(sc, O, D, hit, uv, counts, st, round, n_fixed, emu);
        k_emu_tail<true, false><<<grid_replay, kReplayBlock, 0, stream>>>(sc, O, D, hit, uv, counts, st, round, emu);
    } else {
        k_emu_setup<false, false><<<grid_setup, kSetupBlock, 0, stream>>>(sc, O, D, hit, uv, counts, st, round, n_fixed, emu);
        k_emu_tail<false, false><<<grid_replay, kReplayBlock, 0, stream>>>(sc, O, D, hit, uv, counts, st, round, emu);
    }
    if (uv) k_emu_full<true><<<grid_full, kTraceBlock, 0, stream>>>(sc, O, D, hit, uv, st, round, emu);
    else k_emu_full<false><<<grid_full, kTraceBlock, 0, stream>>>(sc, O, D, hit, uv, st, round, emu);
}

int traceEmuOccupancy()
{
    int nb = 0;
    cudaOccupancyMaxActiveBlocksPerMultiprocessor(&nb, k_trace_emu<false>, kTraceBlock, 0);
    return nb;
}

}
```

Measured before the change: 2616.

## Compress BVH nodes to 64-byte quantised format for traversal

Adds a 64-byte BVH node format with per-axis power-of-two exponents and 8-bit quantised child plane offsets, encoded on the device after the BVH is built. Traversal kernels now read two 32-byte sectors per node instead of a 128-byte line, and decode the bytes with byte_perm plus a paired f32x2 add. Conservative rounding keeps the boxes enclosing the originals, and nodes that cannot be quantised fall back to an escape flag that visits every child. The aim is to cut node memory traffic and cache footprint, at the cost of extra decode ALU work and looser boxes that can cause more node visits.

```diff
diff --git a/pathtracerap_b200/csrc/api.cu b/pathtracerap_b200/csrc/api.cu
--- a/pathtracerap_b200/csrc/api.cu
+++ b/pathtracerap_b200/csrc/api.cu
@@ -69,7 +69,7 @@
     std::vector<PtapMesh> h_meshes;
     std::vector<PtapModel> h_models;
     std::vector<InstanceTrace> h_inst;
-    InstanceTrace* d_inst = nullptr; TriRec* d_tris = nullptr; BvhNode* d_nodes = nullptr; size_t nodes_cap = 0; LeafTri* d_btris = nullptr; int* d_btid = nullptr;
+    InstanceTrace* d_inst = nullptr; TriRec* d_tris = nullptr; BvhNode* d_nodes = nullptr; BvhNode64* d_nodes64 = nullptr; size_t nodes_cap = 0; LeafTri* d_btris = nullptr; int* d_btid = nullptr;
     bool have_scene = false, have_grid = false, have_bvh = false, have_frame = false;
     int bvh_kind = -1;
     int accel = PTAP_ACCEL_GRID_COMPAT;
@@ -393,6 +393,8 @@
     if (nnodes + tlas.size() > ctx->nodes_cap) return fail(ctx, PTAP_E_NOMEM, "BVH node storage exhausted");
     CK(cudaMemcpyAsync(ctx->d_inst, ctx->h_inst.data(), nm * sizeof(InstanceTrace), cudaMemcpyHostToDevice, ctx->stream));
     if (!tlas.empty()) CK(cudaMemcpyAsync(ctx->d_nodes + nnodes, tlas.data(), tlas.size() * sizeof(BvhNode), cudaMemcpyHostToDevice, ctx->stream));
+    launchEncodeNodes64(ctx->d_nodes, nnodes + (int)tlas.size(), ctx->d_nodes64, ctx->stream);
+    CK(cudaGetLastError());
     CK(cudaStreamSynchronize(ctx->stream));
     if (tlas_bytes) *tlas_bytes = nm * sizeof(InstanceTrace) + tlas.size() * sizeof(BvhNode);
     ctx->sc.tlas_root = tlas_root;
@@ -681,6 +683,7 @@
     const size_t nodes_cap = (size_t)std::max(nt, 1) * 2 + (size_t)nm * 2 + 2;
     size_t need = Arena::need(nm, sizeof(InstanceTrace)) + Arena::need(nm, sizeof(InstanceShade)) +
                   Arena::need(nt, sizeof(TriRec)) + Arena::need(nt, sizeof(LeafTri)) + Arena::need(nt, sizeof(float4)) + Arena::need(nt, sizeof(int)) + Arena::need(nodes_cap, sizeof(BvhNode)) +
+                  Arena::need(nodes_cap, sizeof(BvhNode64)) +
                   (grid ? Arena::need(v->nvoxels, sizeof(int2)) + Arena::need(v->nrefs, sizeof(int)) : 0) + 4096;
     if (need > ctx->scene_arena.cap) CK(ctx->scene_arena.reserve(need)); else ctx->scene_arena.used = 0;
     Arena& A = ctx->scene_arena;
@@ -691,9 +694,10 @@
     float4* d_normals = A.alloc<float4>(nt);
     int* d_btid = A.alloc<int>(nt);
     BvhNode* d_nodes = A.alloc<BvhNode>(nodes_cap);
+    BvhNode64* d_nodes64 = A.alloc<BvhNode64>(nodes_cap);
     int2* d_cells = grid ? A.alloc<int2>(v->nvoxels) : nullptr;
     int* d_refs = grid ? A.alloc<int>(v->nrefs) : nullptr;
-    if (!d_inst || !d_shade || !d_tris || !d_normals || !d_btris || !d_btid || !d_nodes || (grid && (!d_cells || !d_refs))) return fail(ctx, PTAP_E_NOMEM, "scene arena exhausted");
+    if (!d_inst || !d_shade || !d_tris || !d_normals || !d_btris || !d_btid || !d_nodes || !d_nodes64 || (grid && (!d_cells || !d_refs))) return fail(ctx, PTAP_E_NOMEM, "scene arena exhausted");
     CK(cudaMemcpyAsync(d_inst, inst.data(), nm * sizeof(InstanceTrace), cudaMemcpyHostToDevice, ctx->stream));
     CK(cudaMemcpyAsync(d_shade, shade.data(), nm * sizeof(InstanceShade), cudaMemcpyHostToDevice, ctx->stream));
     CK(cudaMemcpyAsync(d_tris, recs, (size_t)nt * sizeof(TriRec), cudaMemcpyHostToDevice, ctx->stream));
@@ -706,7 +710,7 @@
     size_t bytes = nm * (sizeof(InstanceTrace) + sizeof(InstanceShade)) + (size_t)nt * sizeof(TriRec) +
                    (grid ? cells.size() * sizeof(int2) + (size_t)v->nrefs * sizeof(int) : 0);
     ctx->h_inst = inst;
-    ctx->d_inst = d_inst; ctx->d_nodes = d_nodes; ctx->nodes_cap = nodes_cap; ctx->d_btris = d_btris; ctx->d_btid = d_btid;
+    ctx->d_inst = d_inst; ctx->d_nodes = d_nodes; ctx->d_nodes64 = d_nodes64; ctx->nodes_cap = nodes_cap; ctx->d_btris = d_btris; ctx->d_btid = d_btid;
     ctx->have_bvh = false; ctx->bvh_kind = -1;
     lap("enqueue scene copies");
     if (v->bvh_nodes && v->n_bvh_nodes > 0 && v->bvh_tri_id && v->bvh_mesh_root) {
@@ -721,7 +725,7 @@
     lap("wait for the device");
     ctx->stats.scene_bytes = (int64_t)bytes;
     ctx->sc.inst = d_inst; ctx->sc.shade = d_shade; ctx->sc.tris = d_tris; ctx->sc.normals = d_normals;
-    ctx->sc.cells = d_cells; ctx->sc.refs = d_refs; ctx->sc.nodes = d_nodes; ctx->sc.bvh_tris = d_btris; ctx->sc.bvh_tri_id = d_btid;
+    ctx->sc.cells = d_cells; ctx->sc.refs = d_refs; ctx->sc.nodes = d_nodes64; ctx->sc.bvh_tris = d_btris; ctx->sc.bvh_tri_id = d_btid;
     ctx->sc.nmodels = nm; ctx->sc.gx = v->grid_dim[0]; ctx->sc.gy = v->grid_dim[1]; ctx->sc.gz = v->grid_dim[2];
     ctx->have_scene = true; ctx->have_grid = grid; ctx->cache_valid = false;
     ctx->accel = grid ? PTAP_ACCEL_GRID_COMPAT : PTAP_ACCEL_BVH;
diff --git a/pathtracerap_b200/csrc/bvh_device.cu b/pathtracerap_b200/csrc/bvh_device.cu
--- a/pathtracerap_b200/csrc/bvh_device.cu
+++ b/pathtracerap_b200/csrc/bvh_device.cu
@@ -227,6 +227,55 @@
     for (int k = 0; k < 4; ++k) nd.link[k] = leafLink(0, n, leaf_base);
     encodeNodeDevice(nd, &b, 1);
     out[0] = nd;
+}
+
+
+__device__ bool quantiseAxis(const BvhNode& nd, int a, unsigned used, unsigned& lq, unsigned& uq, int& e)
+{
+    const float span = ldexpf(255.0f, kNodeExpMax);
+    float top = 0.0f;
+    bool ok = true;
+    for (int c = 0; c < 4; ++c) {
+        if (!(used >> c & 1u)) continue;
+        const float lo = nd.planes[a][0][c], hi = nd.planes[a][1][c];
+        ok = ok && lo >= 0.0f && lo <= span && hi <= span;
+        top = fmaxf(top, fmaxf(lo, hi));
+    }
+    if (!ok) return false;
+    e = top > 0.0f ? max(kNodeExpMin, ilogbf(top) - 8) : kNodeExpMin;
+    while (top > ldexpf(255.0f, e)) ++e;
+    const float inv_step = ldexpf(1.0f, -e);
+    lq = uq = 0u;
+    for (int c = 0; c < 4; ++c) {
+        if (!(used >> c & 1u)) continue;
+        const unsigned l = (unsigned)floorf(__fmul_rd(nd.planes[a][0][c], inv_step));
+        const unsigned u = (unsigned)ceilf(fmaxf(__fmul_ru(nd.planes[a][1][c], inv_step), 0.0f));
+        lq |= l << (8 * c); uq |= u << (8 * c);
+    }
+    return true;
+}
+
+__global__ void k_encode_nodes64(const BvhNode* __restrict__ in, int n, BvhNode64* __restrict__ out)
+{
+    const int i = blockIdx.x * blockDim.x + threadIdx.x;
+    if (i >= n) return;
+    const BvhNode nd = in[i];
+    BvhNode64 o;
+    o.px = nd.px; o.py = nd.py; o.pz = nd.pz;
+    unsigned used = 0u;
+    for (int c = 0; c < 4; ++c) {
+        o.link[c] = nd.link[c];
+        if (nd.planes[0][0][c] <= nd.planes[0][1][c]) used |= 1u << c;
+    }
+    int e[3] = {0, 0, 0};
+    bool ok = isfinite(nd.px) && isfinite(nd.py) && isfinite(nd.pz);
+    for (int a = 0; a < 3; ++a) ok = ok && quantiseAxis(nd, a, used, o.q[a][0], o.q[a][1], e[a]);
+    if (!ok) {
+        for (int a = 0; a < 3; ++a) { e[a] = 0; o.q[a][0] = o.q[a][1] = 0u; }
+    }
+    o.meta = (unsigned)(e[0] + 127) | (unsigned)(e[1] + 127) << 9 | used << kNodeUsedShift | (ok ? 0u : kNodeEscape) | (unsigned)(e[2] + 127) << 23;
+    o.pad[0] = o.pad[1] = 0u;
+    out[i] = o;
 }
 
 
@@ -354,6 +403,11 @@
     return r;
 }
 
+}
+
+void launchEncodeNodes64(const BvhNode* nodes, int n, BvhNode64* out, cudaStream_t stream)
+{
+    if (n > 0) k_encode_nodes64<<<(n + 255) / 256, 256, 0, stream>>>(nodes, n, out);
 }
 
 size_t deviceBvhScratchBytes(int ntris)
diff --git a/pathtracerap_b200/csrc/bvh_traverse.cuh b/pathtracerap_b200/csrc/bvh_traverse.cuh
--- a/pathtracerap_b200/csrc/bvh_traverse.cuh
+++ b/pathtracerap_b200/csrc/bvh_traverse.cuh
@@ -14,13 +14,6 @@
     return *reinterpret_cast<float2*>(&rd);
 }
 
-__device__ __forceinline__ uint4 ldg4u(const void* p)
-{
-    uint4 r;
-    asm("ld.global.nc.v4.u32 {%0,%1,%2,%3}, [%4];" : "=r"(r.x), "=r"(r.y), "=r"(r.z), "=r"(r.w) : "l"(p));
-    return r;
-}
-
 __device__ __forceinline__ int childKey(float nx, float ny, float nz, float fx, float fy, float fz, float tmin, float tmax)
 {
     const float tn = fmaxf(fmaxf(fmaxf(nx, ny), nz), tmin);
@@ -29,10 +22,9 @@
     return h ? __float_as_int(fmaxf(tn, 0.0f)) : 0x7f800000;
 }
 
-__device__ __forceinline__ unsigned nearOffsets(const V3& d)
+__device__ __forceinline__ unsigned dirSigns(const V3& d)
 {
-    const unsigned sx = __float_as_uint(d.x) >> 31, sy = __float_as_uint(d.y) >> 31, sz = __float_as_uint(d.z) >> 31;
-    return (32u + (sx << 4)) | ((64u + (sy << 4)) << 8) | ((96u + (sz << 4)) << 16);
+    return (__float_as_uint(d.x) >> 31) | (__float_as_uint(d.y) >> 31 << 1) | (__float_as_uint(d.z) >> 31 << 2);
 }
 
 __device__ __forceinline__ float safeInv(float d)
@@ -46,32 +38,55 @@
     return g_dist < kFloatMax ? g_dist * prune + cb + 1e-3f : 3.0e38f;
 }
 
-__device__ __forceinline__ void nodeChildren(const char* __restrict__ np, const V3& ro, const V3& rinv, unsigned near_off, float tmin, float tmax, int key[4], int lnk[4])
+__device__ __forceinline__ float2 add2(float2 a, float2 b)
 {
-    const F8 hd = ldg8(np);
-    const unsigned nox = near_off & 0xffu, noy = (near_off >> 8) & 0xffu, noz = near_off >> 16;
-    const uint4 NX = ldg4u(np + nox), FX = ldg4u(np + (nox ^ 16u));
-    const uint4 NY = ldg4u(np + noy), FY = ldg4u(np + (noy ^ 16u));
-    const uint4 NZ = ldg4u(np + noz), FZ = ldg4u(np + (noz ^ 16u));
+    unsigned long long ra = *reinterpret_cast<unsigned long long*>(&a), rb = *reinterpret_cast<unsigned long long*>(&b), rd;
+    asm("add.rn.f32x2 %0, %1, %2;" : "=l"(rd) : "l"(ra), "l"(rb));
+    return *reinterpret_cast<float2*>(&rd);
+}
+
+__device__ __forceinline__ void planeBytes(unsigned w, float2& a, float2& b)
+{
+    const float2 m = make_float2(-8388608.0f, -8388608.0f);
+    a = add2(make_float2(__uint_as_float(__byte_perm(w, 0x4B000000u, 0x7440u)), __uint_as_float(__byte_perm(w, 0x4B000000u, 0x7441u))), m);
+    b = add2(make_float2(__uint_as_float(__byte_perm(w, 0x4B000000u, 0x7442u)), __uint_as_float(__byte_perm(w, 0x4B000000u, 0x7443u))), m);
+}
+
+template <bool SORT>
+__device__ __forceinline__ void nodeChildren(const BvhNode64* __restrict__ nd, const V3& ro, const V3& rinv, unsigned signs, float tmin, float tmax, int key[4], int lnk[4])
+{
+    const F8 hd = ldg8(nd), qd = ldg8(reinterpret_cast<const char*>(nd) + 32);
+    const unsigned meta = __float_as_uint(hd.v[3]);
     const float cx = (hd.v[0] - ro.x) * rinv.x, cy = (hd.v[1] - ro.y) * rinv.y, cz = (hd.v[2] - ro.z) * rinv.z;
-    const float2 ix = make_float2(rinv.x, rinv.x), iy = make_float2(rinv.y, rinv.y), iz = make_float2(rinv.z, rinv.z);
+    const float sx = rinv.x * __uint_as_float(meta << 23), sy = rinv.y * __uint_as_float((meta << 14) & 0x7f800000u), sz = rinv.z * __uint_as_float(meta & 0x7f800000u);
+    const unsigned lx = __float_as_uint(qd.v[0]), ux = __float_as_uint(qd.v[1]), ly = __float_as_uint(qd.v[2]), uy = __float_as_uint(qd.v[3]);
+    const unsigned lz = __float_as_uint(qd.v[4]), uz = __float_as_uint(qd.v[5]);
+    const bool mx = signs & 1u, my = signs & 2u, mz = signs & 4u;
+    const float2 ix = make_float2(sx, sx), iy = make_float2(sy, sy), iz = make_float2(sz, sz);
     const float2 ccx = make_float2(cx, cx), ccy = make_float2(cy, cy), ccz = make_float2(cz, cz);
-    const float2 nxa = fma2(make_float2(__uint_as_float(NX.x), __uint_as_float(NX.y)), ix, ccx), nxb = fma2(make_float2(__uint_as_float(NX.z), __uint_as_float(NX.w)), ix, ccx);
-    const float2 nya = fma2(make_float2(__uint_as_float(NY.x), __uint_as_float(NY.y)), iy, ccy), nyb = fma2(make_float2(__uint_as_float(NY.z), __uint_as_float(NY.w)), iy, ccy);
-    const float2 nza = fma2(make_float2(__uint_as_float(NZ.x), __uint_as_float(NZ.y)), iz, ccz), nzb = fma2(make_float2(__uint_as_float(NZ.z), __uint_as_float(NZ.w)), iz, ccz);
-    const float2 fxa = fma2(make_float2(__uint_as_float(FX.x), __uint_as_float(FX.y)), ix, ccx), fxb = fma2(make_float2(__uint_as_float(FX.z), __uint_as_float(FX.w)), ix, ccx);
-    const float2 fya = fma2(make_float2(__uint_as_float(FY.x), __uint_as_float(FY.y)), iy, ccy), fyb = fma2(make_float2(__uint_as_float(FY.z), __uint_as_float(FY.w)), iy, ccy);
-    const float2 fza = fma2(make_float2(__uint_as_float(FZ.x), __uint_as_float(FZ.y)), iz, ccz), fzb = fma2(make_float2(__uint_as_float(FZ.z), __uint_as_float(FZ.w)), iz, ccz);
+    float2 a, b;
+    planeBytes(mx ? ux : lx, a, b); const float2 nxa = fma2(a, ix, ccx), nxb = fma2(b, ix, ccx);
+    planeBytes(my ? uy : ly, a, b); const float2 nya = fma2(a, iy, ccy), nyb = fma2(b, iy, ccy);
+    planeBytes(mz ? uz : lz, a, b); const float2 nza = fma2(a, iz, ccz), nzb = fma2(b, iz, ccz);
+    planeBytes(mx ? lx : ux, a, b); const float2 fxa = fma2(a, ix, ccx), fxb = fma2(b, ix, ccx);
+    planeBytes(my ? ly : uy, a, b); const float2 fya = fma2(a, iy, ccy), fyb = fma2(b, iy, ccy);
+    planeBytes(mz ? lz : uz, a, b); const float2 fza = fma2(a, iz, ccz), fzb = fma2(b, iz, ccz);
     key[0] = childKey(nxa.x, nya.x, nza.x, fxa.x, fya.x, fza.x, tmin, tmax);
     key[1] = childKey(nxa.y, nya.y, nza.y, fxa.y, fya.y, fza.y, tmin, tmax);
     key[2] = childKey(nxb.x, nyb.x, nzb.x, fxb.x, fyb.x, fzb.x, tmin, tmax);
     key[3] = childKey(nxb.y, nyb.y, nzb.y, fxb.y, fyb.y, fzb.y, tmin, tmax);
+    const bool escape = meta & kNodeEscape;
 #pragma unroll
-    for (int c = 0; c < 4; ++c) lnk[c] = __float_as_int(hd.v[4 + c]);
+    for (int c = 0; c < 4; ++c) {
+        key[c] = !(meta >> (kNodeUsedShift + c) & 1u) ? 0x7f800000 : escape ? 0 : key[c];
+        lnk[c] = __float_as_int(hd.v[4 + c]);
+    }
+    if (SORT) {
 #define PTAP_CSWAP(a, b) { const bool sw = key[b] < key[a]; const int ka = sw ? key[b] : key[a], kb = sw ? key[a] : key[b]; \
                            const int la = sw ? lnk[b] : lnk[a], lb = sw ? lnk[a] : lnk[b]; key[a] = ka; key[b] = kb; lnk[a] = la; lnk[b] = lb; }
-    PTAP_CSWAP(0, 1) PTAP_CSWAP(2, 3) PTAP_CSWAP(0, 2) PTAP_CSWAP(1, 3) PTAP_CSWAP(1, 2)
+        PTAP_CSWAP(0, 1) PTAP_CSWAP(2, 3) PTAP_CSWAP(0, 2) PTAP_CSWAP(1, 3) PTAP_CSWAP(1, 2)
 #undef PTAP_CSWAP
+    }
 }
 
 }
diff --git a/pathtracerap_b200/csrc/device_types.h b/pathtracerap_b200/csrc/device_types.h
--- a/pathtracerap_b200/csrc/device_types.h
+++ b/pathtracerap_b200/csrc/device_types.h
@@ -55,6 +55,17 @@
 };
 static_assert(sizeof(BvhNode) == 128, "BvhNode must be one 128-byte line");
 
+constexpr int kNodeExpMin = -100, kNodeExpMax = 27;
+constexpr unsigned kNodeUsedShift = 17, kNodeEscape = 1u << 21;
+struct __align__(64) BvhNode64 {
+    float px, py, pz;
+    unsigned meta;
+    int link[4];
+    unsigned q[3][2];
+    unsigned pad[2];
+};
+static_assert(sizeof(BvhNode64) == 64, "BvhNode64 must be two 32-byte sectors");
+
 struct FrameState {
     int n_active[kMaxDepth + 2];
     unsigned int ticket[kMaxDepth + 2];
@@ -83,7 +94,7 @@
     const int2* cells;
     const int* refs;
     const int2* tri_box;
-    const BvhNode* nodes;
+    const BvhNode64* nodes;
     const LeafTri* bvh_tris;
     const int* bvh_tri_id;
     int nmodels;
diff --git a/pathtracerap_b200/csrc/kernels.cuh b/pathtracerap_b200/csrc/kernels.cuh
--- a/pathtracerap_b200/csrc/kernels.cuh
+++ b/pathtracerap_b200/csrc/kernels.cuh
@@ -56,6 +56,7 @@
 int buildMeshBvhDevice(const TriRec* d_tris, int t0, int t1, const float* bb_min, const float* bb_max, int node_base, BvhNode* out_nodes, int leaf_base,
                        LeafTri* btris, int* btid, char* scratch, size_t scratch_bytes, cudaStream_t stream, int* nnodes, int* depth,
                        std::string* why);
+void launchEncodeNodes64(const BvhNode* nodes, int n, BvhNode64* out, cudaStream_t stream);
 
 int gridDeviceCount(const float* d_pos, int t0, int n, const float bb_min[3], const float width[3], const int gd[3], int* d_count, int* d_offset,
                     void* d_tmp, size_t tmp_bytes, cudaStream_t stream, long long* npairs);
diff --git a/pathtracerap_b200/csrc/trace_bvh.cu b/pathtracerap_b200/csrc/trace_bvh.cu
--- a/pathtracerap_b200/csrc/trace_bvh.cu
+++ b/pathtracerap_b200/csrc/trace_bvh.cu
@@ -8,9 +8,6 @@
 
 #ifndef PTAP_TRACE_MIN_CTAS
 #define PTAP_TRACE_MIN_CTAS 8
-#endif
-#ifndef PTAP_NODE_LDG256
-#define PTAP_NODE_LDG256 0
 #endif
 #ifndef PTAP_COLD_SMEM
 #define PTAP_COLD_SMEM 0
@@ -93,14 +90,14 @@
 #define C_BO v3(CF(0), CF(1), CF(2))
 #define C_BD v3(CF(3), CF(4), CF(5))
 #define C_WINV v3(CF(6), CF(7), CF(8))
-#define C_WNEAR CF(9)
+#define C_WSIGNS CF(9)
 #define g_dist CF(10)
 #define g_t CF(11)
 #define g_model_f CF(12)
 #define g_tri_f CF(13)
 #define g_u CF(14)
 #define g_v CF(15)
-    unsigned near_off = 0u;
+    unsigned signs = 0u;
     V3 ro = v3(0, 0, 0), rd = v3(0, 0, 1), rinv = v3(0, 0, 0);
     float tmin = 0.0f, tmax = 0.0f;
     int best_tri = -1; float best_u = 0.0f, best_v = 0.0f;
@@ -113,54 +110,9 @@
 #pragma unroll
         for (int rep = 0; rep < kNodeSteps; ++rep) {
             if (node >= 0) {
-                const char* __restrict__ np = reinterpret_cast<const char*>(&sc.nodes[node]);
-                const F8 hd = ldg8(np);
-#if PTAP_NODE_LDG256
-                const F8 px8 = ldg8(np + 32), py8 = ldg8(np + 64), pz8 = ldg8(np + 96);
+                int key[4], lnk[4];
+                nodeChildren<!ANY>(&sc.nodes[node], ro, rinv, signs, tmin, tmax, key, lnk);
                 if (COUNT) cnt.x++;
-                const float cx = (hd.v[0] - ro.x) * rinv.x, cy = (hd.v[1] - ro.y) * rinv.y, cz = (hd.v[2] - ro.z) * rinv.z;
-                const float2 ix = make_float2(rinv.x, rinv.x), iy = make_float2(rinv.y, rinv.y), iz = make_float2(rinv.z, rinv.z);
-                const float2 ccx = make_float2(cx, cx), ccy = make_float2(cy, cy), ccz = make_float2(cz, cz);
-                const float2 lxa = fma2(make_float2(px8.v[0], px8.v[1]), ix, ccx), lxb = fma2(make_float2(px8.v[2], px8.v[3]), ix, ccx), hxa = fma2(make_float2(px8.v[4], px8.v[5]), ix, ccx), hxb = fma2(make_float2(px8.v[6], px8.v[7]), ix, ccx);
-                const float2 lya = fma2(make_float2(py8.v[0], py8.v[1]), iy, ccy), lyb = fma2(make_float2(py8.v[2], py8.v[3]), iy, ccy), hya = fma2(make_float2(py8.v[4], py8.v[5]), iy, ccy), hyb = fma2(make_float2(py8.v[6], py8.v[7]), iy, ccy);
-                const float2 lza = fma2(make_float2(pz8.v[0], pz8.v[1]), iz, ccz), lzb = fma2(make_float2(pz8.v[2], pz8.v[3]), iz, ccz), hza = fma2(make_float2(pz8.v[4], pz8.v[5]), iz, ccz), hzb = fma2(make_float2(pz8.v[6], pz8.v[7]), iz, ccz);
-#define PTAP_MM(l, h, c) fminf(l.c, h.c), fmaxf(l.c, h.c)
-                const float2 nxa = make_float2(fminf(lxa.x, hxa.x), fminf(lxa.y, hxa.y)), fxa = make_float2(fmaxf(lxa.x, hxa.x), fmaxf(lxa.y, hxa.y));
-                const float2 nxb = make_float2(fminf(lxb.x, hxb.x), fminf(lxb.y, hxb.y)), fxb = make_float2(fmaxf(lxb.x, hxb.x), fmaxf(lxb.y, hxb.y));
-                const float2 nya = make_float2(fminf(lya.x, hya.x), fminf(lya.y, hya.y)), fya = make_float2(fmaxf(lya.x, hya.x), fmaxf(lya.y, hya.y));
-                const float2 nyb = make_float2(fminf(lyb.x, hyb.x), fminf(lyb.y, hyb.y)), fyb = make_float2(fmaxf(lyb.x, hyb.x), fmaxf(lyb.y, hyb.y));
-                const float2 nza = make_float2(fminf(lza.x, hza.x), fminf(lza.y, hza.y)), fza = make_float2(fmaxf(lza.x, hza.x), fmaxf(lza.y, hza.y));
-                const float2 nzb = make_float2(fminf(lzb.x, hzb.x), fminf(lzb.y, hzb.y)), fzb = make_float2(fmaxf(lzb.x, hzb.x), fmaxf(lzb.y, hzb.y));
-#undef PTAP_MM
-#else
-                const unsigned nox = near_off & 0xffu, noy = (near_off >> 8) & 0xffu, noz = near_off >> 16;
-                const uint4 NX = ldg4u(np + nox), FX = ldg4u(np + (nox ^ 16u));
-                const uint4 NY = ldg4u(np + noy), FY = ldg4u(np + (noy ^ 16u));
-                const uint4 NZ = ldg4u(np + noz), FZ = ldg4u(np + (noz ^ 16u));
-                if (COUNT) cnt.x++;
-                const float cx = (hd.v[0] - ro.x) * rinv.x, cy = (hd.v[1] - ro.y) * rinv.y, cz = (hd.v[2] - ro.z) * rinv.z;
-                const float2 ix = make_float2(rinv.x, rinv.x), iy = make_float2(rinv.y, rinv.y), iz = make_float2(rinv.z, rinv.z);
-                const float2 ccx = make_float2(cx, cx), ccy = make_float2(cy, cy), ccz = make_float2(cz, cz);
-                const float2 nxa = fma2(make_float2(__uint_as_float(NX.x), __uint_as_float(NX.y)), ix, ccx), nxb = fma2(make_float2(__uint_as_float(NX.z), __uint_as_float(NX.w)), ix, ccx);
-                const float2 nya = fma2(make_float2(__uint_as_float(NY.x), __uint_as_float(NY.y)), iy, ccy), nyb = fma2(make_float2(__uint_as_float(NY.z), __uint_as_float(NY.w)), iy, ccy);
-                const float2 nza = fma2(make_float2(__uint_as_float(NZ.x), __uint_as_float(NZ.y)), iz, ccz), nzb = fma2(make_float2(__uint_as_float(NZ.z), __uint_as_float(NZ.w)), iz, ccz);
-                const float2 fxa = fma2(make_float2(__uint_as_float(FX.x), __uint_as_float(FX.y)), ix, ccx), fxb = fma2(make_float2(__uint_as_float(FX.z), __uint_as_float(FX.w)), ix, ccx);
-                const float2 fya = fma2(make_float2(__uint_as_float(FY.x), __uint_as_float(FY.y)), iy, ccy), fyb = fma2(make_float2(__uint_as_float(FY.z), __uint_as_float(FY.w)), iy, ccy);
-                const float2 fza = fma2(make_float2(__uint_as_float(FZ.x), __uint_as_float(FZ.y)), iz, ccz), fzb = fma2(make_float2(__uint_as_float(FZ.z), __uint_as_float(FZ.w)), iz, ccz);
-#endif
-                int key[4], lnk[4];
-                key[0] = childKey(nxa.x, nya.x, nza.x, fxa.x, fya.x, fza.x, tmin, tmax);
-                key[1] = childKey(nxa.y, nya.y, nza.y, fxa.y, fya.y, fza.y, tmin, tmax);
-                key[2] = childKey(nxb.x, nyb.x, nzb.x, fxb.x, fyb.x, fzb.x, tmin, tmax);
-                key[3] = childKey(nxb.y, nyb.y, nzb.y, fxb.y, fyb.y, fzb.y, tmin, tmax);
-#pragma unroll
-                for (int c = 0; c < 4; ++c) lnk[c] = __float_as_int(hd.v[4 + c]);
-                if (!ANY) {
-#define PTAP_CSWAP(a, b) { const bool sw = key[b] < key[a]; const int ka = sw ? key[b] : key[a], kb = sw ? key[a] : key[b]; \
-                           const int la = sw ? lnk[b] : lnk[a], lb = sw ? lnk[a] : lnk[b]; key[a] = ka; key[b] = kb; lnk[a] = la; lnk[b] = lb; }
-                    PTAP_CSWAP(0, 1) PTAP_CSWAP(2, 3) PTAP_CSWAP(0, 2) PTAP_CSWAP(1, 3) PTAP_CSWAP(1, 2)
-#undef PTAP_CSWAP
-                }
                 if (key[3] != 0x7f800000) push(lnk[3]);
                 if (key[2] != 0x7f800000) push(lnk[2]);
                 if (key[1] != 0x7f800000) push(lnk[1]);
@@ -199,7 +151,7 @@
             const float mlen = xsqrt(xdot(dm, dm));
             rd = xscale(dm, xdiv(1.0f, mlen));
             rinv = v3(safeInv(rd.x), safeInv(rd.y), safeInv(rd.z));
-            near_off = nearOffsets(rd);
+            signs = dirSigns(rd);
             const float wil = rsqrtf(bd.x * bd.x + bd.y * bd.y + bd.z * bd.z);
             tmin = -(kEpsilon + 1e-4f);
             tmax = kFloatMax; best_tri = -1;
@@ -238,7 +190,7 @@
                     if (UV) { g_u = best_u; g_v = best_v; }
                 }
             }
-            ro = bo; rinv = C_WINV; near_off = __float_as_uint(C_WNEAR);
+            ro = bo; rinv = C_WINV; signs = __float_as_uint(C_WSIGNS);
             tmin = sc.tmin_world; tmax = worldBound(g_dist, sc.prune, cb);
             node = pop();
         }
@@ -271,10 +223,10 @@
                 const V3 bo = v3(o4), bd = v3(d4);
                 const float il = rsqrtf(bd.x * bd.x + bd.y * bd.y + bd.z * bd.z);
                 const V3 winv = v3(safeInv(bd.x * il), safeInv(bd.y * il), safeInv(bd.z * il));
-                const unsigned wnear_off = nearOffsets(bd);
+                const unsigned wsigns = dirSigns(bd);
                 CF(0) = bo.x; CF(1) = bo.y; CF(2) = bo.z; CF(3) = bd.x; CF(4) = bd.y; CF(5) = bd.z;
-                CF(6) = winv.x; CF(7) = winv.y; CF(8) = winv.z; C_WNEAR = __uint_as_float(wnear_off);
-                ro = bo; rinv = winv; near_off = wnear_off;
+                CF(6) = winv.x; CF(7) = winv.y; CF(8) = winv.z; C_WSIGNS = __uint_as_float(wsigns);
+                ro = bo; rinv = winv; signs = wsigns;
                 tmin = sc.tmin_world; tmax = 3.0e38f;
                 g_dist = kFloatMax; g_model_f = __int_as_float(-1); g_tri_f = __int_as_float(-1); g_t = 0.0f; g_u = 0.0f; g_v = 0.0f;
                 best_tri = -1;
@@ -303,7 +255,7 @@
 #undef C_BO
 #undef C_BD
 #undef C_WINV
-#undef C_WNEAR
+#undef C_WSIGNS
 #undef g_dist
 #undef g_t
 #undef g_model_f
diff --git a/pathtracerap_b200/csrc/trace_emu.cu b/pathtracerap_b200/csrc/trace_emu.cu
--- a/pathtracerap_b200/csrc/trace_emu.cu
+++ b/pathtracerap_b200/csrc/trace_emu.cu
@@ -69,7 +69,7 @@
     int node = kDone, i = -1;
     V3 bo = v3(0, 0, 0), bd = v3(0, 0, 0);
     V3 winv = v3(0, 0, 0);
-    unsigned near_off = 0u, wnear_off = 0u;
+    unsigned signs = 0u, wsigns = 0u;
     V3 ro = v3(0, 0, 0), rd = v3(0, 0, 1), rinv = v3(0, 0, 0);
     float tmin = 0.0f, tmax = 0.0f;
     float g_dist = kFloatMax, g_t = 0.0f;
@@ -81,7 +81,7 @@
     for (;;) {
         if (node >= 0) {
             int key[4], lnk[4];
-            nodeChildren(reinterpret_cast<const char*>(&sc.nodes[node]), ro, rinv, near_off, tmin, tmax, key, lnk);
+            nodeChildren<true>(&sc.nodes[node], ro, rinv, signs, tmin, tmax, key, lnk);
             if (COUNT) cnt.x++;
             if (key[3] != 0x7f800000) push(lnk[3]);
             if (key[2] != 0x7f800000) push(lnk[2]);
@@ -131,7 +131,7 @@
             const float mlen = xsqrt(xdot(dm, dm));
             rd = xscale(dm, xdiv(1.0f, mlen));
             rinv = v3(safeInv(rd.x), safeInv(rd.y), safeInv(rd.z));
-            near_off = nearOffsets(rd);
+            signs = dirSigns(rd);
             const float wil = rsqrtf(bd.x * bd.x + bd.y * bd.y + bd.z * bd.z);
             tmin = -(kEpsilon + 1e-4f);
             tmax = 3.0e38f;
@@ -168,7 +168,7 @@
                 }
             }
             nh = 0; c_t = kFloatMax; c_tri = -1;
-            ro = bo; rinv = winv; near_off = wnear_off;
+            ro = bo; rinv = winv; signs = wsigns;
             tmin = sc.tmin_world; tmax = worldBound(g_dist, sc.prune, cb);
             node = pop();
         }
@@ -203,8 +203,8 @@
                 bo = v3(o4); bd = v3(d4);
                 const float il = rsqrtf(bd.x * bd.x + bd.y * bd.y + bd.z * bd.z);
                 winv = v3(safeInv(bd.x * il), safeInv(bd.y * il), safeInv(bd.z * il));
-                wnear_off = nearOffsets(bd);
-                ro = bo; rinv = winv; near_off = wnear_off;
+                wsigns = dirSigns(bd);
+                ro = bo; rinv = winv; signs = wsigns;
                 tmin = sc.tmin_world; tmax = 3.0e38f;
                 g_dist = kFloatMax; g_model = -1; g_tri = -1; g_t = 0.0f;
                 nh = 0; nh_best = 0; c_t = kFloatMax; c_tri = -1; n_amb = 0; best_amb = false;
@@ -505,7 +505,7 @@
 
     int node = kDone, i = -1;
     V3 bo = v3(0, 0, 0), bd = v3(0, 0, 0), winv = v3(0, 0, 0);
-    unsigned near_off = 0u, wnear_off = 0u;
+    unsigned signs = 0u, wsigns = 0u;
     V3 ro = v3(0, 0, 0), rd = v3(0, 0, 1), rinv = v3(0, 0, 0);
     float tmin = 0.0f, tmax = 0.0f;
     float g_dist = kFloatMax, g_t = 0.0f;
@@ -517,7 +517,7 @@
     for (;;) {
         if (node >= 0) {
             int key[4], lnk[4];
-            nodeChildren(reinterpret_cast<const char*>(&sc.nodes[node]), ro, rinv, near_off, tmin, tmax, key, lnk);
+            nodeChildren<true>(&sc.nodes[node], ro, rinv, signs, tmin, tmax, key, lnk);
             if (key[3] != 0x7f800000) push(lnk[3]);
             if (key[2] != 0x7f800000) push(lnk[2]);
             if (key[1] != 0x7f800000) push(lnk[1]);
@@ -566,7 +566,7 @@
             ro = xmat4(w0, w1, w2, bo, 1.0f);
             rd = xnormalize(xmat4(w0, w1, w2, bd, 0.0f));
             rinv = v3(safeInv(rd.x), safeInv(rd.y), safeInv(rd.z));
-            near_off = nearOffsets(rd);
+            signs = dirSigns(rd);
             tmin = -(kEpsilon + 1e-4f); tmax = 3.0e38f;
             nh = 0; c_t = kFloatMax;
             push((int)~(kExitBit | (unsigned)im));
@@ -639,7 +639,7 @@
                 }
             }
             nh = 0; c_t = kFloatMax;
-            ro = bo; rinv = winv; near_off = wnear_off;
+            ro = bo; rinv = winv; signs = wsigns;
             tmin = sc.tmin_world; tmax = 3.0e38f;
             node = pop();
         }
@@ -682,8 +682,8 @@
                 bo = v3(o4); bd = v3(d4);
                 const float il = rsqrtf(bd.x * bd.x + bd.y * bd.y + bd.z * bd.z);
                 winv = v3(safeInv(bd.x * il), safeInv(bd.y * il), safeInv(bd.z * il));
-                wnear_off = nearOffsets(bd);
-                ro = bo; rinv = winv; near_off = wnear_off;
+                wsigns = dirSigns(bd);
+                ro = bo; rinv = winv; signs = wsigns;
                 tmin = sc.tmin_world; tmax = 3.0e38f;
                 g_dist = kFloatMax; g_model = -1; g_tri = -1; g_t = 0.0f;
                 nh = 0; c_t = kFloatMax; overflow = false;
```

Result: slower. 2256 (median of 6 runs) (-13.7%).
